# ESCOMP/POP2-CESM

Hardware: AMD Instinct MI355X
Metric: simulated_years_per_day (higher is better)
Workload: dtype f64; 1 GPU; tx0.1v3; nt=2, steps_per_day=300, step_calls_per_day=319, distribution=equal-block-counts, blocks_local=1, hmix=del4, hmix_tracer=del4, vmix=kpp, partial_bottom_cells=False, ns_boundary=closed, grid_input=False, tadvect=centered, solver=pcg, preconditioner=diagonal, transport=none, kpp_surface_buoyancy=on-demand down to the boundary-layer depth

## Files before the change

include/pop_amd.h:

```cpp
#ifndef POP_AMD_H
#define POP_AMD_H

#ifdef __cplusplus
extern "C" {
#endif

#define POP_CONFIG_VERSION 7
typedef struct pop_config {
  int struct_version;
  int nx_global, ny_global, km, nt;
  int block_size_x, block_size_y;
  int ew_boundary;
  int ns_boundary;
  int hmix_momentum;
  int hmix_tracer;
  int lvariable_hmix;
  int vmix_choice;
  int tadvect;
  int solver_choice;
  int max_iterations;
  int convergence_check_freq;
  int tmix_opt;
  int time_mix_freq;
  int steps_per_day;
// ... 33 lines not shown
  double kappa_depth_1, kappa_depth_2, kappa_depth_scale;
  int aniso_alignment;
  int lvariable_hmix_aniso;
  int lsmag_aniso;
  int vconst_5;
  double visc_para, visc_perp;
  double c_para, c_perp;
  double u_para, u_perp;
  double vconst_1;
  double vconst_2;
  double vconst_3;
  double vconst_4;
  double vconst_6;
  double vconst_7;
  double smag_lat;
  double smag_lat_fact;
  double smag_lat_gauss;
  int lsubmesoscale_mixing;
  int luse_const_horiz_len_scale;
  int submeso_diag;
  double efficiency_factor;
  double time_scale_constant;
  double hor_length_scale;
} pop_config;

typedef struct pop_ctx pop_ctx;

#define POP_CREATE_HOST_ONLY 1
#define POP_CREATE_PLAN_ONLY 2

#define POP_TUNING_UNSET (-2147483647 - 1)
typedef struct pop_tuning {
  int struct_bytes;
  int land_skip;
  int land_full_steps;
  int xcd_remap;
  int red_band;
  int lds_order;
  int momentum_lds;
  int tracer_lds;
  int generic_thomas;
  int reg_thomas_t;
  int thomas_pair;
  int tracer_fwd;
  int vdc_shared;
  int side_stream;
  int del4_side;
  int del4_tile;
  int d2t_fuse, d2u_fuse;
  int vmixu_defer;
  int vmixu_inline;
  int btrop_inline;
  int kpp_ahead;
  int kpp_col;
  int kpp_lazy;
  int kpp_ushear_hint;
  int kpp_ushear_margin;
  int kpp_side_stream;
  int kpp_interior_generic;
  int kpp_src_full;
  int solver_unfused;
  int solver_nograph;
  int solver_presum;
  int solver_distributed;
  int solver_overlap_off;
  int fpcg_b2;
  int pcsi_step2;
  int halo_separate;
  int halo_overlap_off;
  int rccl_overlap;
  int evp_wave;
  int fpcg_a_pair;
  int kpp_sparse;
  int pbc_generic_thomas;
  int pbc_generic_kpp;
  int gm_sf_stored;
  int state3d_levels;
  int pcg_persist;
  int gm_flux_tile;
  int pcsi_two_step;
  int block_sums_relay;
  int aniso_side;
  int submeso_all_levels;
} pop_tuning;
void pop_tuning_init(pop_tuning *t);
int pop_get_tuning(const pop_ctx *ctx, pop_tuning *resolved);

int pop_create(const pop_config *cfg, int rank, int nranks, int flags, pop_ctx **out);
typedef struct pop_grid_input {
  const double *ULAT, *ULON, *HTN, *HTE, *HUS, *HUW, *ANGLE;
  const int *KMT;
  const double *DZBC;
} pop_grid_input;
int pop_create_with_grid(const pop_config *cfg, const pop_grid_input *grid, int rank, int nranks, int flags, pop_ctx **out);
int pop_create_tuned(const pop_config *cfg, const pop_grid_input *grid, const pop_tuning *tuning, int rank, int nranks, int flags, pop_ctx **out);
int pop_read_grid_files(const char *horiz_grid_file, const char *topography_file, int nx_global, int ny_global,
                        double *seven_records , int *kmt );
int pop_destroy(pop_ctx *ctx);
const char *pop_last_error(const pop_ctx *ctx);

#define POP_MAX_TIDAL_MIN_REGIONS 9
typedef struct pop_tidal_nml {
  int struct_bytes;
  int ltidal_mixing;
  int tidal_mixing_method;
  int ltidal_max;
  int ltidal_stabc;
  int lccsm_control_compatible;
  int ltidal_min_regions;
  int num_tidal_min_regions;
  int tidal_diag;
  double tidal_local_mixing_fraction;
  double tidal_mixing_efficiency;
  double vertical_decay_scale;
  double tidal_mix_max;
  double tidal_min_values[POP_MAX_TIDAL_MIN_REGIONS];
  double tidal_TLATmin_regions[POP_MAX_TIDAL_MIN_REGIONS];
  double tidal_TLATmax_regions[POP_MAX_TIDAL_MIN_REGIONS];
  double tidal_TLONmin_regions[POP_MAX_TIDAL_MIN_REGIONS];
  double tidal_TLONmax_regions[POP_MAX_TIDAL_MIN_REGIONS];
  int tidal_min_regions_klevels[POP_MAX_TIDAL_MIN_REGIONS];
} pop_tidal_nml;
void pop_tidal_nml_init(pop_tidal_nml *nml);
int pop_init_tidal_mixing(pop_ctx *ctx, const pop_tidal_nml *nml, const double *energy_flux, long long count);

typedef struct pop_kpp_bckgrnd_nml {
  int struct_bytes;
  int lhoriz_varying_bckgrnd;
  int larctic_bckgrnd_vdc;
  double bckgrnd_vdc_eq;
  double bckgrnd_vdc_psim;
  double bckgrnd_vdc_ban;
} pop_kpp_bckgrnd_nml;
void pop_kpp_bckgrnd_nml_init(pop_kpp_bckgrnd_nml *nml);
int pop_init_kpp_bckgrnd(pop_ctx *ctx, const pop_kpp_bckgrnd_nml *nml);

int pop_init_iage(pop_ctx *ctx, int n);

typedef struct pop_ice_nml {
  int struct_bytes;
  int ice_freq_opt;
  int licecesm2;
  int kmxice;
  int lactive_ice;
  int lfw_as_salt_flx;
  int tfreeze_option;
  double sea_ice_salinity;
  double ocn_ref_salinity;
  double latent_heat_fusion;
  double cp_sw;
  double rho_sw;
  double rho_fw;
} pop_ice_nml;
void pop_ice_nml_init(pop_ice_nml *nml);
int pop_init_ice(pop_ctx *ctx, const pop_ice_nml *nml);
int pop_ice_formation(pop_ctx *ctx, int tl);
int pop_ice_flx_to_coupler(pop_ctx *ctx);
int pop_ice_export_reset(pop_ctx *ctx);
int pop_tfreez_host(pop_ctx *ctx, const double *S, double *TFRZ, long long count);

int pop_get_dim(const pop_ctx *ctx, const char *name);
double pop_get_scalar(const pop_ctx *ctx, const char *name);
int pop_get_block(const pop_ctx *ctx, int block_id, int *out8, int *i_glob, int *j_glob);
int pop_local_block_ids(const pop_ctx *ctx, int *ids );

int pop_get_field(pop_ctx *ctx, const char *name, int tl, int n, double *host, long long count);
// ... 134 lines not shown
```

pop2-cesm_amd/csrc/forms.hpp:

```cpp
#pragma once
#include <algorithm>
#include "pop_internal.hpp"

namespace pop {

enum { VMIXU_INLINE = 0, VMIXU_SIDE = 1, VMIXU_DEFERRED = 2 };
enum { KPP_BUOY_MARCH = 0, KPP_BUOY_FUSED_LDS, KPP_BUOY_LDS, KPP_BUOY_PLAIN };
enum { KPP_INTERIOR_FUSED = 0, KPP_INTERIOR_REG, KPP_INTERIOR_GENERIC };
#define POP_FORMS(X)                                                                                                                 \
                                                                   \
  X(int, xcd_remap) X(int, red_band) X(int, lds_order)                                                                              \
     \
  X(bool, land_skip) X(int, land_full_steps)                                                                                        \
     \
  X(int, momentum_lds_rows) X(int, tracer_lds_rows) X(bool, gm_lds) X(bool, kpp_src_full) X(bool, tracer_fwd)                       \
                                                                                               \
  X(bool, reg_thomas_u) X(bool, reg_thomas_t) X(bool, thomas_pair) X(int, impvmixu_waves)                                           \
                                                                                                     \
  X(bool, vdc_shared) X(bool, side_stream) X(bool, del4_side) X(bool, mom_side) X(bool, aniso_side)                                 \
                                                                                                             \
  X(int, del4_tile_rows) X(bool, d2t_fuse) X(bool, d2u_fuse)                                                                        \
             \
  X(int, vmixu) X(bool, btrop_inline)                                                                                               \
                                                                            \
  X(bool, kpp_ahead) X(int, kpp_col) X(bool, kpp_lazy) X(bool, kpp_lazy20) X(bool, kpp_march) X(bool, kpp_pbc_generic)              \
  X(bool, kpp_shear_col) X(int, kpp_buoy) X(int, kpp_buoy_kr) X(bool, kpp_buoy_sfc) X(bool, kpp_depth_lazy) X(int, kpp_depth_kr)    \
  X(int, kpp_interior) X(bool, kpp_sparse) X(bool, kpp_side) X(bool, kpp_wuk) X(int, kpp_wuk_margin)                                \
                                                                                                            \
  X(int, state3d_levels) X(bool, gm_sf_stored) X(bool, submeso_all_levels)                                                          \
          \
  X(int, path) X(bool, fused_ok) X(bool, evp_fused_ok) X(bool, replicated) X(int, evp_wave) X(bool, graph) X(bool, overlap)         \
  X(bool, presum_forced) X(bool, fpcg_b2) X(bool, fpcg_a_pair) X(int, block_sums_relay) X(int, persist)                             \
                       \
  X(bool, pcsi_two_cell) X(bool, pcsi_two_step) X(bool, pcsi_two_step_dist)                                                         \
                                                                                           \
  X(bool, halo_separate) X(bool, halo_overlap) X(int, rccl_overlap)
struct Forms {
#define X(type, name) type name = 0;
  POP_FORMS(X)
#undef X
};
inline int forms_get(const Forms &f, const std::string &name) {
#define X(type, member) if (name == #member) return (int)f.member;
  POP_FORMS(X)
#undef X
  return -1;
}

constexpr double KPP_EPSSFC = 0.1;
inline std::vector<int> kpp_kref(const HostModel &h) {
  std::vector<int> kref(h.km + 3, 1);
  for (int k = 1; k <= h.km; ++k) {
    const double surfthick = KPP_EPSSFC * h.zt[k];
    kref[k] = k;
    for (int kt = 1; kt <= k; ++kt) if (h.zw[kt] >= surfthick) { kref[k] = kt; break; }
  }
  return kref;
}
inline int max_blocks_per_rank(const HostModel &h) {
  std::vector<int> per(h.nranks, 0);
  for (int o : h.block_owner) if (o >= 0 && o < h.nranks) per[o]++;
  return per.empty() ? 0 : *std::max_element(per.begin(), per.end());
}
inline std::vector<int> local_srcmap(const HostModel &h) {
  std::vector<int> sm(h.n2 * h.nblocks);
  for (size_t p = 0; p < sm.size(); ++p) sm[p] = (int)p;
  for (size_t i = 0; i < h.halo.copy_dst.size(); ++i) sm[h.halo.copy_dst[i]] = h.halo.copy_src[i];
  for (int d : h.halo.fill_dst) sm[d] = -1;
  if (h.c.ns_boundary == 2) {
    const TripolePlan &T = h.halo.tripole[0];
    for (size_t e = 0; e < T.dst.size(); ++e) sm[T.dst[e]] = T.a[e];
  }
  return sm;
}
inline bool pcsi_fold_local(const HostModel &h, const std::vector<int> &srcmap, std::vector<int> &jfold) {
  bool local = true;
  jfold.assign(h.nblocks, h.nyb);
  if (h.c.ns_boundary != 2) return true;
  for (int lb = 0; lb < h.nblocks; ++lb) {
    const BlockInfo &B = h.all_blocks[h.local_ids[lb] - 1];
    if (!(B.j_glob[B.je] < 0)) continue;
    jfold[lb] = B.je;
    for (int j = B.je; j < h.nyb; ++j) for (int i = 0; i < h.nxb; ++i) {
      const int cell = lb * (int)h.n2 + j * h.nxb + i;
      if (srcmap[cell] == cell) local = false;
    }
  }
  return local;
}
inline int chunks_per_block(long long n2, int red_band) {
  const int nc = (int)((n2 + 255) / 256);
  return red_band ? 8 * ((nc + 7) / 8) : nc;
}
inline bool presum_by_size(long long nchunk, long long nblocks) { return nchunk * nblocks > 2048; }
inline bool two_cell_shape(int nxb, bool presummed) { return presummed && (nxb & 1) == 0; }

inline bool bandwidth_bound(const HostModel &h) { return (long long)h.n2 * h.nblocks > (1LL << 19); }
inline bool register_levels(const HostModel &h) { return h.km == 60 || h.km == 62; }

inline int resolve_forms(const HostModel &h, Forms &f, std::string &err) {
  const pop_config &c = h.c;
  const pop_tuning &t = h.tun;
  const bool big = bandwidth_bound(h), reg_km = register_levels(h), evp = use_evp(c), tripole = c.ns_boundary == 2;
  const bool single = h.halo.peers.empty();
  auto rule_or = [](int v, bool rule) { return (tun_set(v) && v >= 0) ? v != 0 : rule; };
  if (tun_set(t.xcd_remap) && t.xcd_remap != 0 && t.xcd_remap != 1) { err = "pop_create: pop_tuning.xcd_remap is " + std::to_string(t.xcd_remap) + ": 0 linear or 1 XCD bands"; return 1; }
  if (tun_set(t.evp_wave) && t.evp_wave != 0 && t.evp_wave != 3) { err = "pop_create: pop_tuning.evp_wave is " + std::to_string(t.evp_wave) + ": 0 one thread per sub-block or 3 wavefronts"; return 1; }

  f.xcd_remap = tun_or(t.xcd_remap, big ? 0 : 1);
  f.red_band = tun_or(t.red_band, 1);
  f.lds_order = tun_or(t.lds_order, 1);
  f.land_skip = !tun_off(t.land_skip);
  f.land_full_steps = tun_or(t.land_full_steps, 4);

  f.momentum_lds_rows = tun_or(t.momentum_lds, 4);
  f.tracer_lds_rows = tun_or(t.tracer_lds, 4);
  f.gm_lds = !tun_off(t.gm_flux_tile);
  f.kpp_src_full = tun_on(t.kpp_src_full);

  const bool pbc_generic = c.partial_bottom_cells && tun_on(t.pbc_generic_thomas);
  const bool want_u = !tun_on(t.generic_thomas) && !pbc_generic;
  const bool want_t = (tun_set(t.reg_thomas_t) ? t.reg_thomas_t != 0 : !tun_on(t.generic_thomas)) && !pbc_generic;
  f.reg_thomas_u = want_u && reg_km;
  f.reg_thomas_t = want_t && reg_km;
  f.thomas_pair = f.reg_thomas_t && rule_or(t.thomas_pair, big);
  f.impvmixu_waves = (!c.partial_bottom_cells && !big) ? 2 : 1;
  f.tracer_fwd = c.tadvect == 1 && c.hmix_tracer != 3 && (f.tracer_lds_rows == 4 || f.tracer_lds_rows == 8) && c.lpressure_avg &&
                 (tun_set(t.tracer_fwd) ? t.tracer_fwd != 0 : !want_t);

  f.vdc_shared = c.vmix_choice == 3 && !c.ldbl_diff && !tun_off(t.vdc_shared);
  f.side_stream = !tun_off(t.side_stream);
  f.del4_side = f.side_stream && (c.hmix_tracer == 4 || c.hmix_momentum == 4) && !tun_off(t.del4_side);
  f.aniso_side = f.side_stream && c.hmix_momentum == 3 && !tun_off(t.aniso_side);
  f.mom_side = c.hmix_momentum == 3 ? f.aniso_side : f.del4_side;

  f.del4_tile_rows = big ? 4 : 0;
  if (tun_set(t.del4_tile)) f.del4_tile_rows = (t.del4_tile == 2 || t.del4_tile == 4 || t.del4_tile == 8 || t.del4_tile == 16) ? t.del4_tile : 0;
  const bool fuse = f.del4_side && !tripole && rule_or(t.d2t_fuse, big);
  f.d2t_fuse = fuse && c.hmix_tracer == 4 && c.tadvect == 1;
  f.d2u_fuse = fuse && c.hmix_momentum == 4 && !tun_off(t.d2u_fuse);

  f.btrop_inline = !f.side_stream || tripole || tun_on(t.btrop_inline);
  const bool off_stream = f.side_stream && f.reg_thomas_u && !tun_on(t.vmixu_inline);
  f.vmixu = (off_stream && !f.btrop_inline && rule_or(t.vmixu_defer, big)) ? VMIXU_DEFERRED : off_stream ? VMIXU_SIDE : VMIXU_INLINE;

  f.evp_wave = tun_or(t.evp_wave, 3);
  f.graph = !tun_on(t.solver_nograph);
  f.overlap = !tun_on(t.solver_overlap_off);
  f.presum_forced = tun_on(t.solver_presum);
  f.fpcg_b2 = !tun_off(t.fpcg_b2);
  f.fpcg_a_pair = !tun_off(t.fpcg_a_pair);
  f.block_sums_relay = tun_or(t.block_sums_relay, 1);
  f.persist = !tun_set(t.pcg_persist) ? 1 : (t.pcg_persist == 0 || t.pcg_persist == 2 || t.pcg_persist == 4 || t.pcg_persist == 8) ? t.pcg_persist : 1;
  const bool unfused = tun_on(t.solver_unfused);
  f.fused_ok = single && h.nblocks <= 8 && !unfused;
  if (evp) {
    f.evp_fused_ok = f.fused_ok && c.solver_choice == 3;
    f.fused_ok = false;
  }
  f.replicated = !single && c.solver_choice == 1 && !evp && h.nblocks_tot <= 8 && (long long)h.n2 * h.nblocks_tot <= (4LL << 20) &&
                 !tun_on(t.solver_distributed);
  const bool spread = h.nranks > 1 && !unfused, few = max_blocks_per_rank(h) <= 16;
  if (c.solver_choice == 2) f.path = (f.fused_ok && !evp) ? 2 : (spread && few && !evp) ? 3 : 1;
  else if (c.solver_choice == 3) f.path = evp ? (f.evp_fused_ok ? 2 : 1) : f.fused_ok ? 2 : spread ? 3 : 1;
  else f.path = evp ? 1 : f.replicated ? 4 : f.fused_ok ? 2 : (spread && few) ? 3 : 1;
  const int nchunk = chunks_per_block((long long)h.n2, f.red_band);
  const bool two_cell_rule = two_cell_shape(h.nxb, presum_by_size(nchunk, h.nblocks));
  f.pcsi_two_cell = tun_set(t.pcsi_step2) ? two_cell_shape(h.nxb, t.pcsi_step2 != 0) : two_cell_rule;
  if (!evp && (tun_set(t.pcsi_two_step) ? t.pcsi_two_step != 0 : two_cell_rule)) {
    std::vector<int> jfold;
    const bool fold_ok = !tripole || pcsi_fold_local(h, local_srcmap(h), jfold);
    f.pcsi_two_step = fold_ok && single;
    f.pcsi_two_step_dist = fold_ok && !single;
  }

  if (c.vmix_choice == 3) {
    const bool resident_solve = (c.solver_choice == 1 || c.solver_choice == 3) && !evp && f.persist != 0 && h.nranks == 1 && h.nblocks <= 8 &&
                                h.n2 * h.nblocks <= 250u * 8u * 256u;
    f.kpp_ahead = f.side_stream && (tun_set(t.kpp_ahead) ? t.kpp_ahead != 0 : (big || resident_solve));
    const std::vector<int> kref = kpp_kref(h);
    const int max_kref = *std::max_element(kref.begin(), kref.end());
    f.kpp_col = (max_kref <= 24) ? tun_or(t.kpp_col, big ? 31 : 1) : 0;
    const bool fused_bi = (f.kpp_col & 8) && max_kref <= 20 && h.km <= 64, lds = (f.kpp_col & 4) && max_kref <= 28;
    f.kpp_lazy = (fused_bi || !lds) && max_kref <= 28 && !c.lcheckekmo && c.kpp_ml_diagnostics != 1 && !tun_off(t.kpp_lazy);
    f.kpp_lazy20 = f.kpp_lazy && max_kref <= 20;
    f.kpp_march = f.kpp_lazy && fused_bi && (f.kpp_col & 16) && c.num_v_smooth_Ri == 1 && !c.ldbl_diff && h.km >= 3;
    f.kpp_pbc_generic = c.partial_bottom_cells && !(f.kpp_march && f.kpp_lazy20 && (f.kpp_col & 1) && !tun_on(t.pbc_generic_kpp));
    const bool gen = f.kpp_pbc_generic;
    f.kpp_shear_col = !gen && (f.kpp_col & 1);
    f.kpp_buoy = gen ? KPP_BUOY_PLAIN : f.kpp_march ? KPP_BUOY_MARCH : fused_bi ? KPP_BUOY_FUSED_LDS : lds ? KPP_BUOY_LDS : KPP_BUOY_PLAIN;
    f.kpp_buoy_kr = max_kref <= 20 ? 20 : 28;
    f.kpp_buoy_sfc = gen || !f.kpp_lazy;
    f.kpp_depth_lazy = !gen && f.kpp_lazy;
    f.kpp_depth_kr = (f.kpp_depth_lazy && !f.kpp_lazy20) ? 28 : 20;
    f.kpp_interior = gen ? KPP_INTERIOR_GENERIC : fused_bi ? KPP_INTERIOR_FUSED : (!tun_on(t.kpp_interior_generic) && reg_km) ? KPP_INTERIOR_REG : KPP_INTERIOR_GENERIC;
    f.kpp_sparse = !gen && f.kpp_march && h.km <= 64 && !tun_off(t.kpp_sparse);
    f.kpp_side = !tun_off(t.kpp_side_stream) && !gen;
    f.kpp_wuk = f.kpp_depth_lazy && (f.kpp_col & 1) && !tun_off(t.kpp_ushear_hint);
    f.kpp_wuk_margin = tun_or(t.kpp_ushear_margin, 3);
  }

  f.state3d_levels = tun_or(t.state3d_levels, 4);
  f.gm_sf_stored = !tun_off(t.gm_sf_stored);
  f.submeso_all_levels = tun_on(t.submeso_all_levels);

  f.halo_separate = tun_on(t.halo_separate);
  f.halo_overlap = !tun_on(t.halo_overlap_off);
  f.rccl_overlap = tun_or(t.rccl_overlap, 1);
  return 0;
}

}
```

pop2-cesm_amd/csrc/kernels_bckgrnd.hpp:

```cpp
#pragma once

namespace pop {

struct BckDev {
  const double *VDC = nullptr, *VVC = nullptr, *VVC_PR = nullptr;
};

struct BckRaw { double visc, vd1, vd2; };
__global__ void __launch_bounds__(POP_COL_THREADS)
k_kpp_bckgrnd(DevGrid g, BckDev bd, int vdc_same, double *__restrict__ VISC, double *__restrict__ VDC1, double *__restrict__ VDC2) {
  Col c;
  if (!col_setup(g, c, false)) return;
  const int km = g.km;
  const long long n2 = g.n2;
  const int kmt = g.KMT[c.q2];
  if (kmt < 2) return;
  const double bvdc = bd.VDC[c.q2], bvvc = bd.VVC[c.q2];
  const long long vb = ((long long)c.b * (km + 2)) * n2 + c.p2;
  auto load = [&](int k) {
    BckRaw r;
    r.visc = VISC[c.base3 + (long long)(k - 1) * n2]; r.vd1 = VDC1[vb + (long long)k * n2];
    r.vd2 = vdc_same ? 0.0 : VDC2[vb + (long long)k * n2];
    return r;
  };
  BckRaw cu = load(1);
#pragma unroll 1
  for (int k = 1; k < kmt; ++k) {
    const BckRaw nx = load(k + 1 < kmt ? k + 1 : k);
    VISC[c.base3 + (long long)(k - 1) * n2] = cu.visc + bvvc;
    VDC1[vb + (long long)k * n2] = cu.vd1 + bvdc;
    if (!vdc_same) VDC2[vb + (long long)k * n2] = cu.vd2 + bvdc;
    cu = nx;
  }
}

}
```

pop2-cesm_amd/csrc/kernels_common.hpp:

```cpp
#pragma once
#include "device_types.hpp"
#include "forms.hpp"
#include <type_traits>

namespace pop {

template <class F> inline void with_flags(F &&f) { f(); }
template <class F, class... Bs> inline void with_flags(F &&f, bool b, Bs... bs) {
  if (b) with_flags([&](auto... c) { f(std::true_type{}, c...); }, bs...);
  else with_flags([&](auto... c) { f(std::false_type{}, c...); }, bs...);
}
template <int... Vs, class F> inline bool with_value(int v, F &&f) {
  return ((v == Vs ? (f(std::integral_constant<int, Vs>{}), true) : false) || ...);
}

#define POP_COL_THREADS 64
#ifndef POP_TRC_WAVES
#define POP_TRC_WAVES 2
#endif
#ifndef POP_MOM_WAVES
#define POP_MOM_WAVES 2
#endif

__device__ __forceinline__ double pbc_dz(const DevGrid &g, int k, int kbot, double dzbot) {
  return (k < 1 || k > g.km) ? 0.0 : ((k == kbot) ? dzbot : g.dz[k]);
}

__device__ __forceinline__ int blk_ie(const DevGrid &g, int b) { return g.ieb ? g.ieb[b] : g.ie; }
__device__ __forceinline__ int blk_je(const DevGrid &g, int b) { return g.jeb ? g.jeb[b] : g.je; }

struct Col {
  int i, j, b, p2;
  long long q2;
  long long base3;
};
__host__ __device__ inline int lds_grid_x(int lds_order, int ntx, int nty) {
  const int nt = ntx * nty;
  return lds_order ? 256 * ((nt + 255) / 256) : nt;
}
__host__ __device__ inline int lds_slot_of(int a) {
  const int r = a >> 5, t = a & 31;
  return (((r >> 3) << 5) + t) * 8 + (r & 7);
}
__host__ __device__ inline bool lds_tile_from_gi(int gi, int ntx, int nty, int &ti, int &tj);
__host__ __device__ inline bool lds_tile_of(int lds_order, int bx, int ntx, int nty, int &ti, int &tj) {
  if (!lds_order) { ti = bx % ntx; tj = bx / ntx; return tj < nty; }
  const int e = bx & 7, s = bx >> 3;
  const int gi = ((s >> 5) * 8 + e) * 32 + (s & 31);
  return lds_tile_from_gi(gi, ntx, nty, ti, tj);
}
__host__ __device__ inline bool lds_tile_from_gi(int gi, int ntx, int nty, int &ti, int &tj) {
  constexpr int PW = 4, PH = 8;
  if (gi >= ntx * nty) return false;
  const int row_tiles = PH * ntx, full_rows = nty / PH;
  int Pj, r, h;
  if (gi >= full_rows * row_tiles) { Pj = full_rows; r = gi - full_rows * row_tiles; h = nty - full_rows * PH; }
  else { Pj = gi / row_tiles; r = gi % row_tiles; h = PH; }
  const int patch_tiles = h * PW, nfullp = ntx / PW;
  int Pi, w, rr;
  if (r < nfullp * patch_tiles) { Pi = r / patch_tiles; w = PW; rr = r % patch_tiles; }
  else { Pi = nfullp; w = ntx - nfullp * PW; rr = r - nfullp * patch_tiles; }
  ti = Pi * PW + rr % w; tj = Pj * PH + rr / w;
  return true;
}
__device__ __forceinline__ bool lds_tile(int lds_order, int ntx, int nty, int &ti, int &tj) {
  return lds_tile_of(lds_order, (int)blockIdx.x, ntx, nty, ti, tj);
}
template <int R>
__device__ __forceinline__ bool lds_tile_active(const DevGrid &g, int b, int ntx, int nty, int &ti, int &tj, bool &listed) {
  const int *L = (R == 8) ? g.lds_act8 : g.lds_act4;
  const int nL = (R == 8) ? g.lds_n8 : g.lds_n4;
  listed = g.skip && L != nullptr;
  if (!listed) return lds_tile(g.lds_order, ntx, nty, ti, tj);
  const int e = L[(long long)b * nL + blockIdx.x];
  if (e < 0) return false;
  ti = e & 0xffff; tj = e >> 16;
  return true;
}
template <int R>
__host__ inline int lds_launch_x(const DevGrid &g, int ntx, int nty) {
  const int *L = (R == 8) ? g.lds_act8 : g.lds_act4;
  if (g.skip && L) return (R == 8) ? g.lds_n8 : g.lds_n4;
  return lds_grid_x(g.lds_order, ntx, nty);
}
__device__ __forceinline__ int ocean_cells(const DevGrid &g, int b, int p0, int p1) {
  const int *S = g.opre + (long long)b * (g.n2 + 1);
  return S[p1] - S[p0];
}
__device__ __forceinline__ bool land_tile(const DevGrid &g, int b, int i0, int w, int j0, int h) {
  if (!g.skip) return false;
  int i1 = i0 + w, j1 = j0 + h;
  if (i0 < 0) i0 = 0;
  if (j0 < 0) j0 = 0;
  if (i1 > g.nxb) i1 = g.nxb;
  if (j1 > g.nyb) j1 = g.nyb;
  if (i0 >= i1) return false;
  int n = 0;
  for (int j = j0; j < j1; ++j) n += ocean_cells(g, b, j * g.nxb + i0, j * g.nxb + i1);
  return n == 0;
}
__device__ __forceinline__ bool land_run(const DevGrid &g, int b, long long p0, int n) {
  if (!g.skip || p0 >= g.n2) return false;
  const int p1 = (p0 + n < g.n2) ? (int)(p0 + n) : g.n2;
  return ocean_cells(g, b, (int)p0, p1) == 0;
}
__host__ __device__ inline int col_grid_x(int n2, int threads) { const int nt = (n2 + threads - 1) / threads; return 8 * ((nt + 7) / 8); }
__host__ inline int col_grid(const DevGrid &g, int threads) { return col_grid_x(g.n2, threads); }
__device__ __forceinline__ bool col_setup(const DevGrid &g, Col &c, bool interior_only) {
  c.b = blockIdx.y;
  const int tile = g.xcd_remap ? (blockIdx.x & 7) * (gridDim.x >> 3) + (blockIdx.x >> 3) : blockIdx.x;
  c.p2 = tile * blockDim.x + threadIdx.x;
  if (c.p2 >= g.n2) return false;
  if (land_run(g, c.b, (long long)tile * blockDim.x, blockDim.x)) return false;
  c.i = c.p2 % g.nxb;
  c.j = c.p2 / g.nxb;
  if (interior_only && (c.i + 1 < g.ib || c.i + 1 > blk_ie(g, c.b) || c.j + 1 < g.jb || c.j + 1 > blk_je(g, c.b))) return false;
  c.q2 = (long long)c.b * g.n2 + c.p2;
  c.base3 = (long long)c.b * g.n3 + c.p2;
  return true;
}
__device__ __forceinline__ bool patch_cell(const DevGrid &g, int tile, int b, int &p2) {
  if (!tile) {
    p2 = blockIdx.x * blockDim.x + threadIdx.x;
    if (p2 >= g.n2) return false;
    return !land_run(g, b, (long long)blockIdx.x * blockDim.x, blockDim.x);
  }
  const int tiles_i = (g.nxb + 63) / 64;
  const int ti = blockIdx.x % tiles_i, tj = blockIdx.x / tiles_i;
  const int i = ti * 64 + (threadIdx.x & 63), j = tj * tile + (threadIdx.x >> 6);
  if (land_tile(g, b, ti * 64, 64, tj * tile, tile)) return false;
  if (i >= g.nxb || j >= g.nyb) return false;
  p2 = j * g.nxb + i;
  return true;
}
__host__ inline unsigned patch_grid_x(const DevGrid &g, int tile) {
  return tile ? (unsigned)(((g.nxb + 63) / 64) * ((g.nyb + tile - 1) / tile)) : (unsigned)((g.n2 + 255) / 256);
}
__host__ inline int red_grid_x(const DevGrid &g) {
  return g.red_act ? g.red_nact : chunks_per_block(g.n2, g.red_band);
}
__device__ __forceinline__ int red_chunk(const DevGrid &g) {
  if (g.red_act) return g.red_act[(long long)blockIdx.y * g.red_nact + blockIdx.x];
  return g.red_band ? (blockIdx.x & 7) * (gridDim.x >> 3) + (blockIdx.x >> 3) : blockIdx.x;
}
__device__ __forceinline__ int red_cell(const DevGrid &g) {
  const long long p2 = (long long)red_chunk(g) * blockDim.x + threadIdx.x;
  return p2 < g.n2 ? (int)p2 : g.n2;
}

__device__ __forceinline__ bool red_land(const DevGrid &g, bool deep = false) {
  if (!g.skip || (blockIdx.x == 0 && blockIdx.y == 0)) return false;
  if (g.red_act)
    return (int)((blockIdx.x & 7) * (g.red_nact >> 3) + (blockIdx.x >> 3)) >= g.red_cnt[blockIdx.y];
  const long long p0 = (long long)red_chunk(g) * 256;
  if (!land_run(g, blockIdx.y, p0, 256)) return false;
  const long long p1 = (p0 + 255 < g.n2) ? p0 + 255 : g.n2 - 1;
  const int j0 = (int)(p0 / g.nxb), j1 = (int)(p1 / g.nxb);
  const int i0 = (j0 == j1) ? (int)(p0 % g.nxb) : 0, i1 = (j0 == j1) ? (int)(p1 % g.nxb) : g.nxb - 1;
  if (deep && !(i0 >= g.ib - 1 + NGHOST && i1 <= blk_ie(g, blockIdx.y) - 1 - NGHOST && j0 >= g.jb - 1 + NGHOST && j1 <= blk_je(g, blockIdx.y) - 1 - NGHOST)) return false;
  return true;
}
template <int NF>
__device__ __forceinline__ bool red_land_out(const DevGrid &g, double *__restrict__ partial, int nchunk, bool deep = false) {
  if (!red_land(g, deep)) return false;
  if (threadIdx.x == 0) {
    const long long slot = (long long)blockIdx.y * nchunk + red_chunk(g);
#pragma unroll
    for (int f = 0; f < NF; ++f) partial[NF * slot + f] = 0.0;
  }
  return true;
}

struct MwjfP {
  double n0, n2, ns1t0, d0, d1, d3;
};
__device__ __forceinline__ MwjfP mwjf_level(double pbar) {
  const double p = 10.0 * pbar;
  MwjfP c;
  c.n0 = (9.99843699e+2 * 0.001) + p * ((1.04004591e-2 * 0.001) + p * (-3.24041825e-8 * 0.001));
  c.n2 = (-5.45928211e-2 * 0.001) + p * ((1.03970529e-7 * 0.001) + p * (-1.23869360e-11 * 0.001));
  c.ns1t0 = (2.96938239e+0 * 0.001) + p * (5.18761880e-6 * 0.001);
  c.d0 = 1.0e+0 + p * 5.30848875e-6;
  c.d1 = 7.28606739e-3 + (p * p * p) * -1.27934137e-17;
  c.d3 = 3.68390573e-7 + (p * p) * -3.03175128e-16;
  return c;
}
struct MwjfTS { double TQ, SQ, SQR; };
__device__ __forceinline__ MwjfTS mwjf_prep(double TK, double SK) {
  MwjfTS r;
  r.TQ = fmin(TK, 999.0); r.TQ = fmax(r.TQ, -2.0);
  double SQ = fmin(SK, 0.999); SQ = fmax(SQ, 0.0);
  r.SQ = 1000.0 * SQ;
  r.SQR = sqrt(r.SQ);
  return r;
}
__device__ __forceinline__ double mwjf_eval(const MwjfP &c, const MwjfTS &x) {
  const double n1 = 7.35212840e+0 * 0.001, n3 = 3.98476704e-4 * 0.001;
  const double ns1t1 = -7.23268813e-3 * 0.001, ns2t0 = 2.12382341e-3 * 0.001;
  const double d2 = -4.60835542e-5, d4 = 1.80809186e-10, ds1t0 = 2.14691708e-3, ds1t1 = -9.27062484e-6;
  const double ds1t3 = -1.78343643e-10, dsqt0 = 4.76534122e-6, dsqt2 = 1.63410736e-9;
  const double TQ = x.TQ, SQ = x.SQ, SQR = x.SQR;
  const double W1 = c.n0 + TQ * (n1 + TQ * (c.n2 + n3 * TQ)) + SQ * (c.ns1t0 + ns1t1 * TQ + ns2t0 * SQ);
  const double W2 = c.d0 + TQ * (c.d1 + TQ * (d2 + TQ * (c.d3 + d4 * TQ))) +
                    SQ * (ds1t0 + TQ * (ds1t1 + TQ * TQ * ds1t3) + SQR * (dsqt0 + TQ * TQ * dsqt2));
  const double DEN = 1.0 / W2;
  return W1 * DEN;
}
struct MwjfTS2 { double TQ, SQ, A2; };
__device__ __forceinline__ MwjfTS2 mwjf_prep2(double TK, double SK) {
  const double ds1t0 = 2.14691708e-3, ds1t1 = -9.27062484e-6, ds1t3 = -1.78343643e-10, dsqt0 = 4.76534122e-6, dsqt2 = 1.63410736e-9;
  MwjfTS2 r;
  r.TQ = fmin(TK, 999.0); r.TQ = fmax(r.TQ, -2.0);
  double SQ = fmin(SK, 0.999); SQ = fmax(SQ, 0.0);
  r.SQ = 1000.0 * SQ;
  const double SQR = sqrt(r.SQ), TQ = r.TQ;
  r.A2 = r.SQ * (ds1t0 + TQ * (ds1t1 + TQ * TQ * ds1t3) + SQR * (dsqt0 + TQ * TQ * dsqt2));
  return r;
}
// ... 37 lines not shown
```

pop2-cesm_amd/csrc/kernels_kpp.hpp:

```cpp
#pragma once

namespace pop {

struct KppDev {
  CArr zgrid, hwide, bckgrnd_vdc, bckgrnd_vvc;
  CArrI kref;
  CArr eosP;
  unsigned long long *CONVB;
  int src_clear_all;
  double *HBLT0, *USTAR, *BFSFC;
  int *KBL0, *KBL;
  double Vtc, cg, rich_mix;
  int lrich, ldbl_diff, nsmooth;
  int *WUK;
  int wu_margin;
  int vdc_same;

  int lshort_wave, sw_type, jerlov, lcheckekmo;
  const double *FCORT, *SHF_QSW;
  const double *Tr, *ztr;
  const int *CHLI;
  int ksol;
  double *BO, *BOSOL;
  double *SRCX = nullptr;
// ... 229 lines not shown
  double (*dst)[POP_COL_THREADS] = shtop;
  for (int pass = 0; pass + 1 < kp.nsmooth; ++pass) {
#pragma unroll 1
    for (int k = 1 + gy; k <= km; k += NG) {
      const double cur = src ? src[k - 1][tx] : w0(k);
      double v = cur;
      if (kmt >= 3) {
        const double w1 = 0.25 * ((k > 1) ? (src ? src[k - 2][tx] : w0(k - 1)) : cur);
        const double nxt = (k < km) ? (src ? src[k][tx] : w0(k + 1)) : cur;
        v = w1 + 0.5 * cur + 0.25 * nxt;
      }
      dst[k - 1][tx] = v;
    }
    __syncthreads();
    src = dst; dst = (dst == shtop) ? shri : shtop;
  }
  if (!live) return;
  const long long vb = ((long long)b * (km + 2)) * n2 + p2;
#pragma unroll 1
  for (int k = 1 + gy; k <= km; k += NG) {
    const long long o = base3 + (long long)(k - 1) * n2;
    const double cur = src ? src[k - 1][tx] : w0(k);
    double riw = cur;
    if (kp.nsmooth >= 1 && kmt >= 3) {
      const double w1 = 0.25 * ((k > 1) ? (src ? src[k - 2][tx] : w0(k - 1)) : cur);
      const double nxt = (k < km) ? (src ? src[k][tx] : w0(k + 1)) : cur;
      riw = w1 + 0.5 * cur + 0.25 * nxt;
    }
    double fri = fmax(riw, 0.0) / KPP_RIINFTY;
    fri = fmin(fri, 1.0);
    double visc, vd1 = 0.0, vd2 = 0.0;
    if (kp.lrich) {
      const double f = 1.0 - fri * fri;
      const double f3 = (f * f) * f;
      visc = kp.bckgrnd_vvc[k] + kp.rich_mix * f3;
      if (k < km) { vd2 = kp.bckgrnd_vdc[k] + kp.rich_mix * f3; vd1 = vd2; }
    } else {
      visc = kp.bckgrnd_vvc[k];
      if (k < km) { vd2 = kp.bckgrnd_vdc[k]; vd1 = vd2; }
    }
    if (k >= kmt) { visc = 0.0; vd1 = 0.0; vd2 = 0.0; }
    if (kp.ldbl_diff) {
      const double t_k = T[o], s_k = S[o];
      double ta_u = 0.0, sb_u = 0.0;
      { const MwjfP Pk = mwjf_level(g.pressz[k]); (void)mwjf_rho<true>(Pk, tmask(t_k), s_k, &ta_u, &sb_u); }
      double alphadt = 0.0, betads = 0.0, ta_n = 0.0, sb_n = 0.0, t_n = 0.0, s_n = 0.0;
      if (k < km) {
        t_n = T[o + n2]; s_n = S[o + n2];
        const MwjfP Pn = mwjf_level(g.pressz[k + 1]);
        (void)mwjf_rho<true>(Pn, tmask(t_n), s_n, &ta_n, &sb_n);
        alphadt = -0.5 * (ta_u + ta_n) * (t_k - t_n);
        betads = 0.5 * (sb_u + sb_n) * (s_k - s_n);
      }
      if (alphadt > betads && betads > 0.0) {
        const double rrho = fmin(alphadt / betads, KPP_RRHO0);
        const double f = 1.0 - (rrho - 1.0) / (KPP_RRHO0 - 1.0);
        const double diffdd = KPP_DSFMAX * ((f * f) * f);
        vd1 = vd1 + 0.7 * diffdd; vd2 = vd2 + diffdd;
      }
      double rrho = 0.0, diffdd = 0.0, prandtl = 0.0;
      if (alphadt < 0.0 && betads < 0.0 && alphadt > betads) {
        rrho = alphadt / betads;
        diffdd = 1.5e-2 * 0.909 * exp(4.6 * exp(-0.54 * (1.0 / rrho - 1.0)));
        prandtl = 0.15 * rrho;
      }
      if (rrho > 0.5) prandtl = (1.85 - 0.85 / rrho) * rrho;
      vd1 = vd1 + diffdd; vd2 = vd2 + prandtl * diffdd;
    }
    VISC[o] = visc;
    VDC1[vb + (long long)k * n2] = vd1;
    if (!kp.vdc_same) VDC2[vb + (long long)k * n2] = vd2;
  }
}

__global__ void k_kpp_level_table(DevGrid g, double *__restrict__ tab) {
  const int k = threadIdx.x;
  if (k < 1 || k > g.km) return;
  const MwjfP P = mwjf_level(g.pressz[k]);
  double *t = tab + 6 * k;
  t[0] = P.n0; t[1] = P.n2; t[2] = P.ns1t0; t[3] = P.d0; t[4] = P.d1; t[5] = P.d3;
}
struct KppRaw { double t, s, u[4], v[4]; };
template <bool PBC = false>
__global__ void __launch_bounds__(POP_COL_THREADS)
k_kpp_buoy_interior_march(DevGrid g, KppDev kp, const double *__restrict__ T, const double *__restrict__ S,
                          const double *__restrict__ U, const double *__restrict__ V, double *__restrict__ DBLOC,
                          double *__restrict__ VISC, double *__restrict__ VDC1, double *__restrict__ VDC2) {
  Col c;
  if (!col_setup(g, c, false)) return;
  const int km = g.km, nxb = g.nxb;
  const long long n2 = g.n2;
  const int kmt = g.KMT[c.q2];
  const bool edge = (c.i == 0 || c.j == 0);
  const long long off4[4] = {0, edge ? 0 : -(long long)nxb, edge ? 0 : -1, edge ? 0 : -1 - (long long)nxb};
  const long long vb = ((long long)c.b * (km + 2)) * n2 + c.p2;
  int kmu4[4] = {0, 0, 0, 0}; double dzub4[4] = {0.0, 0.0, 0.0, 0.0}; const double dzbc = PBC ? g.DZBC[c.q2] : 0.0;
  if (PBC) {
#pragma unroll
    for (int t = 0; t < 4; ++t) { kmu4[t] = g.KMU[c.q2 + off4[t]]; dzub4[t] = g.DZUB[c.q2 + off4[t]]; }
  }
  auto dzq = [&](int k, int kbot, double dzbot) { return (k < 1 || k > km) ? 0.0 : ((k == kbot) ? dzbot : g.dz.u(k)); };
  auto load = [&](int k) {
    KppRaw r;
    const long long o = c.base3 + (long long)(k - 1) * n2;
    r.t = T[o]; r.s = S[o];
#pragma unroll
    for (int t = 0; t < 4; ++t) { r.u[t] = U[o + off4[t]]; r.v[t] = V[o + off4[t]]; }
    return r;
  };
  auto emit = [&](int k, double wprev, double cur, double wnext) {
    double riw = cur;
    if (kmt >= 3) {
      const double w1 = 0.25 * ((k > 1) ? wprev : cur);
      const double nxt = (k < km) ? wnext : cur;
      riw = w1 + 0.5 * cur + 0.25 * nxt;
    }
    double fri = fmax(riw, 0.0) / KPP_RIINFTY;
    fri = fmin(fri, 1.0);
    double visc, vd1 = 0.0, vd2 = 0.0;
    if (kp.lrich) {
      const double f = 1.0 - fri * fri;
      const double f3 = (f * f) * f;
      visc = kp.bckgrnd_vvc[k] + kp.rich_mix * f3;
      if (k < km) { vd2 = kp.bckgrnd_vdc[k] + kp.rich_mix * f3; vd1 = vd2; }
    } else {
      visc = kp.bckgrnd_vvc[k];
      if (k < km) { vd2 = kp.bckgrnd_vdc[k]; vd1 = vd2; }
    }
    if (k >= kmt) { visc = 0.0; vd1 = 0.0; vd2 = 0.0; }
    VISC[c.base3 + (long long)(k - 1) * n2] = visc;
    VDC1[vb + (long long)k * n2] = vd1;
    if (!kp.vdc_same) VDC2[vb + (long long)k * n2] = vd2;
  };
  KppRaw up = load(1), A = load(2 <= km ? 2 : km), B;
  MwjfTS2 xkm = mwjf_prep2(tmask(up.t), up.s);
  double wpp = 0.0, wp = 0.0, carry = 0.0;
  unsigned long long convb = 0ull;
  auto level = [&](int k, const KppRaw &cu, KppRaw &nx) {
    nx = load(k + 1 <= km ? k + 1 : km);
    const MwjfTS2 xk = mwjf_prep2(tmask(cu.t), cu.s);
    MwjfP P;
    { const int e = 6 * k; P.n0 = kp.eosP[e]; P.n2 = kp.eosP[e + 1]; P.ns1t0 = kp.eosP[e + 2]; P.d0 = kp.eosP[e + 3]; P.d1 = kp.eosP[e + 4]; P.d3 = kp.eosP[e + 5]; }
    const double rhokm = mwjf_eval2(P, xkm);
    const double rhok = mwjf_eval2(P, xk);
    double dbl = 0.0;
    if (rhok != 0.0) dbl = GRAV * (1.0 - rhokm / rhok);
    if (k - 1 >= kmt) dbl = 0.0;
    DBLOC[c.base3 + (long long)(k - 2) * n2] = dbl;
    if (!(dbl > 0.0)) convb |= 1ull << (k - 2);
    double sh4[4];
#pragma unroll
    for (int t = 0; t < 4; ++t) {
      const double du = up.u[t] - cu.u[t], dv = up.v[t] - cu.v[t];
      sh4[t] = du * du + dv * dv;
      if (PBC) { const double h = 0.5 * (dzq(k - 1, kmu4[t], dzub4[t]) + dzq(k, kmu4[t], dzub4[t])); sh4[t] = sh4[t] / (h * h); }
    }
    double vsh = 0.25 * sh4[0] + 0.25 * sh4[1] + 0.25 * sh4[2] + 0.25 * sh4[3];
    if (edge) vsh = 0.0;
    double ri = dbl * (kp.zgrid[k - 1] - kp.zgrid[k]) / (vsh + KPP_EPS);
    if (PBC) { const double h = 0.5 * (dzq(k - 1, kmt, dzbc) + dzq(k, kmt, dzbc)); ri = dbl / (vsh + KPP_EPS / (h * h)) / h; }
    const int m = k - 1;
    const double w = (m <= kmt) ? ri : carry;
    if (m == kmt) carry = ri;
    if (m >= 2) emit(m - 1, wpp, wp, w);
    wpp = wp; wp = w;
#pragma unroll
    for (int t = 0; t < 4; ++t) { up.u[t] = cu.u[t]; up.v[t] = cu.v[t]; }
    xkm = xk;
  };
  int k = 2;
#pragma unroll 1
  for (; k + 1 <= km; k += 2) { level(k, A, B); level(k + 1, B, A); }
  if (k <= km) level(k, A, B);
  DBLOC[c.base3 + (long long)(km - 1) * n2] = 0.0;
  if (kp.CONVB) kp.CONVB[c.q2] = convb;
  {
    double ri = 0.0 * (kp.zgrid[km] - kp.zgrid[km + 1]) / (0.0 + KPP_EPS);
    if (PBC) { const double h = 0.5 * dzq(km, kmt, dzbc); ri = 0.0 / (0.0 + KPP_EPS / (h * h)) / h; }
    const double w = (km <= kmt) ? ri : carry;
    emit(km - 1, wpp, wp, w);
    emit(km, wp, w, w);
  }
}

template <int KR, bool PBC = false>
__global__ void __launch_bounds__(POP_COL_THREADS)
k_kpp_ushear_col(DevGrid g, KppDev kp, const double *__restrict__ U, const double *__restrict__ V, double *__restrict__ WU) {
  static_assert(POP_COL_THREADS == 64, "k_kpp_ushear_col: one wavefront per workgroup");
  __shared__ int s_cap;
  if (kp.WUK && threadIdx.x == 0) s_cap = 0;
  Col c;
  if (!col_setup(g, c, false)) return;
  const int km = g.km;
  const long long n2 = g.n2;
  int kcap = km, krcap = KR;
  if (kp.WUK) {
    int h = kp.KBL[c.q2];
    if (c.i + 1 < g.nxb) h = max(h, kp.KBL[c.q2 + 1]);
    if (c.j + 1 < g.nyb) { h = max(h, kp.KBL[c.q2 + g.nxb]); if (c.i + 1 < g.nxb) h = max(h, kp.KBL[c.q2 + g.nxb + 1]); }
    __syncthreads();
    atomicMax(&s_cap, h);
    __syncthreads();
    kcap = min(km, max(2, s_cap + kp.wu_margin));
    kp.WUK[c.q2] = kcap;
    krcap = kp.kref[kcap];
  }
  const int kmu_c = PBC ? g.KMU[c.q2] : 0; const double dzub_c = PBC ? g.DZUB[c.q2] : 0.0;
  double ur[KR + 1], vr[KR + 1];
#pragma unroll
  for (int t = 1; t <= KR; ++t) {
    ur[t] = 0.0; vr[t] = 0.0;
    if (t <= krcap) {
      const int kk = (t <= km) ? t : km;
      const long long o = c.base3 + (long long)(kk - 1) * n2;
      ur[t] = U[o]; vr[t] = V[o];
    }
  }
  for (int kl = 2; kl <= kcap; ++kl) {
    const long long o = c.base3 + (long long)(kl - 1) * n2;
    const double ukl = U[o], vkl = V[o];
    const double surfthick = KPP_EPSSFC * g.zt[kl];
    const int kref = kp.kref[kl];
    double uref, vref;
    if (kref > 1) {
      double uk = ur[1], vk = vr[1];
#pragma unroll
      for (int t = 2; t <= KR; ++t) if (t == kref) { uk = ur[t]; vk = vr[t]; }
      uref = uk * (surfthick - g.zw[kref - 1]);
      vref = vk * (surfthick - g.zw[kref - 1]);
#pragma unroll
      for (int kt = 1; kt <= KR - 1; ++kt)
        if (kt <= kref - 1) { uref = uref + g.dz[kt] * ur[kt]; vref = vref + g.dz[kt] * vr[kt]; }
      uref = uref / surfthick; vref = vref / surfthick;
    } else { uref = ur[1]; vref = vr[1]; }
    const double du = uref - ukl, dv = vref - vkl;
    if (PBC) {
      const double h = -kp.zgrid[kl - 1] + 0.5 * (pbc_dz(g, kl, kmu_c, dzub_c) + pbc_dz(g, kl - 1, kmu_c, dzub_c) - pbc_dz(g, 1, kmu_c, dzub_c));
      WU[o] = (du * du + dv * dv) / (h * h);
    } else WU[o] = du * du + dv * dv;
  }
}

template <bool PBC = false>
__global__ void __launch_bounds__(POP_COL_THREADS)
k_kpp_interior(DevGrid g, KppDev kp, const double *__restrict__ T, const double *__restrict__ S,
               const double *__restrict__ U, const double *__restrict__ V, const double *__restrict__ DBLOC,
               double *__restrict__ RIW, double *__restrict__ VISC, double *__restrict__ VDC1, double *__restrict__ VDC2) {
  Col c;
  if (!col_setup(g, c, false)) return;
  const int km = g.km, nxb = g.nxb;
  const long long n2 = g.n2;
  const int kmt = g.KMT[c.q2];
  const bool edge = (c.i == 0 || c.j == 0);
  int kmu4[4] = {0, 0, 0, 0}; double dzub4[4] = {0, 0, 0, 0}; const double dzbc = PBC ? g.DZBC[c.q2] : 0.0;
  if (PBC && !edge) {
    const long long off[4] = {0, -nxb, -1, -1 - nxb};
#pragma unroll
    for (int t = 0; t < 4; ++t) { kmu4[t] = g.KMU[c.q2 + off[t]]; dzub4[t] = g.DZUB[c.q2 + off[t]]; }
  }
  double prev = 0.0;
  for (int k = 1; k <= km; ++k) {
    const long long o = c.base3 + (long long)(k - 1) * n2;
    double vsh = 0.0;
    if (k < km && !edge) {
      auto sh = [&](long long q, int t) {
        const double du = U[q] - U[q + n2], dv = V[q] - V[q + n2];
        if (PBC) { const double h = 0.5 * (pbc_dz(g, k, kmu4[t], dzub4[t]) + pbc_dz(g, k + 1, kmu4[t], dzub4[t])); return (du * du + dv * dv) / (h * h); }
        return du * du + dv * dv;
      };
      vsh = 0.25 * sh(o, 0) + 0.25 * sh(o - nxb, 1) + 0.25 * sh(o - 1, 2) + 0.25 * sh(o - 1 - nxb, 3);
    }
    double ri = DBLOC[o] * (kp.zgrid[k] - kp.zgrid[k + 1]) / (vsh + KPP_EPS);
    if (PBC) {
      const double h = (k < km) ? 0.5 * (pbc_dz(g, k, kmt, dzbc) + pbc_dz(g, k + 1, kmt, dzbc)) : 0.5 * pbc_dz(g, k, kmt, dzbc);
      ri = DBLOC[o] / (vsh + KPP_EPS / (h * h)) / h;
    }
    const double w0 = (k <= kmt) ? ri : prev;
    RIW[o] = w0;
    prev = w0;
  }
  for (int n = 0; n < kp.nsmooth; ++n) {
    double w1 = 0.25 * RIW[c.base3];
    if (kmt >= 3) {
      double cur = RIW[c.base3];
      for (int k = 1; k <= km; ++k) {
        const long long o = c.base3 + (long long)(k - 1) * n2;
        const double nxt = (k < km) ? RIW[o + n2] : cur;
        RIW[o] = w1 + 0.5 * cur + 0.25 * nxt;
        w1 = 0.25 * cur;
        cur = nxt;
      }
    }
  }
  const long long vb = ((long long)c.b * (km + 2)) * n2 + c.p2;
  double ta_u = 0.0, sb_u = 0.0, t_k = T[c.base3], s_k = S[c.base3];
  if (kp.ldbl_diff) { const MwjfP P = mwjf_level(g.pressz[1]); (void)mwjf_rho<true>(P, tmask(t_k), s_k, &ta_u, &sb_u); }
  for (int k = 1; k <= km; ++k) {
    const long long o = c.base3 + (long long)(k - 1) * n2;
    double fri = fmax(RIW[o], 0.0) / KPP_RIINFTY;
    fri = fmin(fri, 1.0);
    double visc, vd1 = 0.0, vd2 = 0.0;
    if (kp.lrich) {
      const double f = 1.0 - fri * fri;
      const double f3 = (f * f) * f;
      visc = kp.bckgrnd_vvc[k] + kp.rich_mix * f3;
      if (k < km) { vd2 = kp.bckgrnd_vdc[k] + kp.rich_mix * f3; vd1 = vd2; }
    } else {
      visc = kp.bckgrnd_vvc[k];
      if (k < km) { vd2 = kp.bckgrnd_vdc[k]; vd1 = vd2; }
    }
    if (k >= kmt) { visc = 0.0; vd1 = 0.0; vd2 = 0.0; }
    if (kp.ldbl_diff) {
      double alphadt = 0.0, betads = 0.0, ta_n = 0.0, sb_n = 0.0, t_n = 0.0, s_n = 0.0;
      if (k < km) {
        t_n = T[o + n2]; s_n = S[o + n2];
        const MwjfP P = mwjf_level(g.pressz[k + 1]);
        (void)mwjf_rho<true>(P, tmask(t_n), s_n, &ta_n, &sb_n);
        alphadt = -0.5 * (ta_u + ta_n) * (t_k - t_n);
        betads = 0.5 * (sb_u + sb_n) * (s_k - s_n);
      }
      if (alphadt > betads && betads > 0.0) {
        const double rrho = fmin(alphadt / betads, KPP_RRHO0);
        const double f = 1.0 - (rrho - 1.0) / (KPP_RRHO0 - 1.0);
// ... 117 lines not shown
    VISC[o] = visc;
    VDC1[vb + (long long)k * n2] = vd1;
    if (!kp.vdc_same) VDC2[vb + (long long)k * n2] = vd2;
  }
}

template <bool PBC = false>
__global__ void __launch_bounds__(256)
k_kpp_ushear(DevGrid g, KppDev kp, const double *__restrict__ U, const double *__restrict__ V, double *__restrict__ WU) {
  const int p2 = blockIdx.x * blockDim.x + threadIdx.x;
  const int kl = blockIdx.y + 1, b = blockIdx.z;
  if (p2 >= g.n2 || kl < 2) return;
  const long long n2 = g.n2;
  const long long base3 = (long long)b * g.n3 + p2;
  const long long o = base3 + (long long)(kl - 1) * n2;
  const double surfthick = KPP_EPSSFC * g.zt[kl];
  const int kref = kp.kref[kl];
  double uref, vref;
  if (kref > 1) {
    const long long orf = base3 + (long long)(kref - 1) * n2;
    uref = U[orf] * (surfthick - g.zw[kref - 1]);
    vref = V[orf] * (surfthick - g.zw[kref - 1]);
    int kt = 1;
    for (; kt + 7 <= kref - 1; kt += 8) {
      double uu[8], vv[8];
#pragma unroll
      for (int t = 0; t < 8; ++t) { const long long ot = base3 + (long long)(kt + t - 1) * n2; uu[t] = U[ot]; vv[t] = V[ot]; }
#pragma unroll
      for (int t = 0; t < 8; ++t) { uref = uref + g.dz[kt + t] * uu[t]; vref = vref + g.dz[kt + t] * vv[t]; }
    }
    for (; kt <= kref - 1; ++kt) {
      const long long ot = base3 + (long long)(kt - 1) * n2;
      uref = uref + g.dz[kt] * U[ot];
      vref = vref + g.dz[kt] * V[ot];
    }
    uref = uref / surfthick; vref = vref / surfthick;
  } else { uref = U[base3]; vref = V[base3]; }
  const double du = uref - U[o], dv = vref - V[o];
  if (PBC) {
    const long long q2 = (long long)b * n2 + p2;
    const int kmu = g.KMU[q2]; const double dzub = g.DZUB[q2];
    const double h = -kp.zgrid[kl - 1] + 0.5 * (pbc_dz(g, kl, kmu, dzub) + pbc_dz(g, kl - 1, kmu, dzub) - pbc_dz(g, 1, kmu, dzub));
    WU[o] = (du * du + dv * dv) / (h * h);
  } else
  WU[o] = du * du + dv * dv;
}

template <bool PBC = false>
__device__ __forceinline__ double kpp_ushear_point(const DevGrid &g, const KppDev &kp, const double *__restrict__ U, const double *__restrict__ V,
                                                   long long base3, int kl, long long q2 = 0) {
  const long long n2 = g.n2;
  const long long o = base3 + (long long)(kl - 1) * n2;
  const double surfthick = KPP_EPSSFC * g.zt[kl];
  const int kref = kp.kref[kl];
  double uref, vref;
  if (kref > 1) {
    const long long orf = base3 + (long long)(kref - 1) * n2;
    uref = U[orf] * (surfthick - g.zw[kref - 1]);
    vref = V[orf] * (surfthick - g.zw[kref - 1]);
#pragma unroll 1
    for (int kt = 1; kt <= kref - 1; ++kt) {
      const long long ot = base3 + (long long)(kt - 1) * n2;
      uref = uref + g.dz[kt] * U[ot];
      vref = vref + g.dz[kt] * V[ot];
    }
    uref = uref / surfthick; vref = vref / surfthick;
  } else { uref = U[base3]; vref = V[base3]; }
  const double du = uref - U[o], dv = vref - V[o];
  if (PBC) {
    const int kmu = g.KMU[q2]; const double dzub = g.DZUB[q2];
    const double h = -kp.zgrid[kl - 1] + 0.5 * (pbc_dz(g, kl, kmu, dzub) + pbc_dz(g, kl - 1, kmu, dzub) - pbc_dz(g, 1, kmu, dzub));
    return (du * du + dv * dv) / (h * h);
  }
  return du * du + dv * dv;
}

template <bool LAZY, int KR, bool PBC = false>
__global__ void __launch_bounds__(POP_COL_THREADS)
k_kpp_bldepth(DevGrid g, KppDev kp, const double *__restrict__ T, const double *__restrict__ S,
              const double *__restrict__ STF1, const double *__restrict__ STF2, const double *__restrict__ DBLOC,
              const double *__restrict__ DBSFC, const double *__restrict__ WU, const double *__restrict__ UU, const double *__restrict__ VV) {
  static_assert(POP_COL_THREADS == 64, "the lazy march votes over one 64-lane wave");
  __shared__ double shtop[LAZY ? 3 * KR : 1][POP_COL_THREADS];
  int nprep = 0;
  Col c;
  if (!col_setup(g, c, false)) return;
  const int km = g.km, nxb = g.nxb;
  const long long n2 = g.n2;
  const int kmt = g.KMT[c.q2];
  const bool edge = (c.i == 0 || c.j == 0);
  int wuk[4] = {km, km, km, km};
  if (LAZY && kp.WUK && !edge) { wuk[0] = kp.WUK[c.q2]; wuk[1] = kp.WUK[c.q2 - 1]; wuk[2] = kp.WUK[c.q2 - nxb]; wuk[3] = kp.WUK[c.q2 - 1 - nxb]; }
  const double s1 = g.SMFT1[c.q2], s2 = g.SMFT2[c.q2];
  double ustar = sqrt(sqrt(s1 * s1 + s2 * s2));
  ustar = fmax(ustar, KPP_EPS);
  double talpha, sbeta;
  const MwjfP P1 = mwjf_level(g.pressz[1]);
  const double rho1 = mwjf_rho<true>(P1, tmask(T[c.base3]), S[c.base3], &talpha, &sbeta);
  double bo = 0.0, bosol = 0.0;
  const int chli = (kp.lshort_wave && kp.sw_type == 2) ? kp.CHLI[c.q2] : 0;
  if (rho1 != 0.0) {
    bo = GRAV * (-talpha * STF1[c.q2] - sbeta * STF2[c.q2]) / rho1;
    if (kp.lshort_wave) bosol = -GRAV * talpha * kp.SHF_QSW[c.q2] / rho1;
  }
  int kbl = (kmt > 1) ? kmt : 1;
  double hblt = -kp.zgrid[kbl];
  const double dzbc = PBC ? g.DZBC[c.q2] : 0.0, dzub = PBC ? g.DZUB[c.q2] : 0.0;
  const int kmu_c = PBC ? g.KMU[c.q2] : 0;
  auto zkl_of = [&](int kl) { return (PBC && kl > 1) ? -kp.zgrid[kl - 1] + 0.5 * (pbc_dz(g, kl, kmt, dzbc) + pbc_dz(g, kl - 1, kmt, dzbc)) : -kp.zgrid[kl]; };
  if (PBC) hblt = zkl_of(kbl);
  double rib_upper = 0.0, rib_up = 0.0, z_upper = 0.0, z_up = kp.zgrid[1];
  double bfsfc = bo;
  double hekman = 0.0, hlimit = 0.0, hmon_up = 0.0;
  if (kp.lcheckekmo) {
    hekman = -kp.zgrid[km] + KPP_EPS; hlimit = -kp.zgrid[km] + KPP_EPS;
    double bf = kpp_bfsfc(kp, bo, bosol, -z_up, 1, chli);
    const double st = (bf >= 0.0) ? 1.0 : 0.0;
    bf = bf + st * KPP_EPS;
    const double w = st * KPP_CMONOB * ustar * ustar * ustar / KPP_VONKAR / bf + (st - 1.0) * kp.zgrid[km];
    hmon_up = (w <= -z_up) ? -z_up + KPP_EPS : w;
  }
  for (int kl = 2; kl <= km; ++kl) {
    if (LAZY && __builtin_amdgcn_ballot_w64(kbl == kmt && kl <= kmt) == 0) break;
    const long long o = c.base3 + (long long)(kl - 1) * n2;
    const double surfthick = KPP_EPSSFC * g.zt[kl];
    const double zkl = zkl_of(kl);
    double dbsfc;
    if (LAZY) {
      const int kref = kp.kref[kl];
      for (; nprep < kref; ++nprep) {
        const int kk = (nprep + 1 <= km) ? nprep + 1 : km;
        const long long ot = c.base3 + (long long)(kk - 1) * n2;
        const MwjfTS2 x = mwjf_prep2(tmask(T[ot]), S[ot]);
        shtop[nprep][threadIdx.x] = x.TQ; shtop[KR + nprep][threadIdx.x] = x.SQ; shtop[2 * KR + nprep][threadIdx.x] = x.A2;
      }
      auto top_at = [&](int t) { MwjfTS2 x; x.TQ = shtop[t - 1][threadIdx.x]; x.SQ = shtop[KR + t - 1][threadIdx.x]; x.A2 = shtop[2 * KR + t - 1][threadIdx.x]; return x; };
      const MwjfTS2 xk = mwjf_prep2(tmask(T[o]), S[o]);
      const MwjfP P = mwjf_level(g.pressz[kl]);
      const double rhok = mwjf_eval2(P, xk);
      double rhoavg = mwjf_eval2(P, top_at(kref));
      if (kref != 1) {
        rhoavg = rhoavg * (surfthick - g.zw[kref - 1]);
#pragma unroll 1
        for (int kt = 1; kt <= kref - 1; ++kt) rhoavg = rhoavg + g.dz[kt] * mwjf_eval2(P, top_at(kt));
        rhoavg = rhoavg / surfthick;
      }
      dbsfc = 0.0;
      if (rhok != 0.0) dbsfc = GRAV * (1.0 - rhoavg / rhok);
    } else dbsfc = DBSFC[o];
    double vshear = 0.0;
    if (!edge) {
      if (LAZY && kp.WUK) {
        const double w00 = (kl <= wuk[0]) ? WU[o] : kpp_ushear_point<PBC>(g, kp, UU, VV, c.base3, kl, c.q2);
        const double w10 = (kl <= wuk[1]) ? WU[o - 1] : kpp_ushear_point<PBC>(g, kp, UU, VV, c.base3 - 1, kl, c.q2 - 1);
        const double w01 = (kl <= wuk[2]) ? WU[o - nxb] : kpp_ushear_point<PBC>(g, kp, UU, VV, c.base3 - nxb, kl, c.q2 - nxb);
        const double w11 = (kl <= wuk[3]) ? WU[o - 1 - nxb] : kpp_ushear_point<PBC>(g, kp, UU, VV, c.base3 - 1 - nxb, kl, c.q2 - 1 - nxb);
        vshear = fmax(fmax(w00, w10), fmax(w01, w11));
      } else vshear = fmax(fmax(WU[o], WU[o - 1]), fmax(WU[o - nxb], WU[o - 1 - nxb]));
    }
    bfsfc = kpp_bfsfc(kp, bo, bosol, zkl, 2 * kl - 1, chli);
    const double stable = (bfsfc >= 0.0) ? 1.0 : 0.0;
    bfsfc = bfsfc + stable * KPP_EPS;
    if (kp.lcheckekmo) {
      if (stable > 0.5 && hekman >= -kp.zgrid[km]) hekman = fmax(zkl, KPP_CEKMAN * ustar / (fabs(kp.FCORT[c.q2]) + KPP_EPS));
      const double hmon_dn = stable * KPP_CMONOB * ustar * ustar * ustar / KPP_VONKAR / bfsfc + (stable - 1.0) * kp.zgrid[km];
      if (hmon_dn <= zkl && hmon_up > -z_up) {
        const double w = (hmon_dn - hmon_up) / (z_up + zkl);
        hlimit = (hmon_dn - w * zkl) / (1.0 - w);
      }
      hmon_up = hmon_dn;
    }
    double wm_unused = 0.0, ws;
    kpp_wscale<false>(KPP_EPSSFC, zkl, ustar, bfsfc, wm_unused, ws);
    const double db = DBLOC[o];
    double bfr = sqrt(0.5 * (db + fabs(db) + KPP_EPS2) / (kp.zgrid[kl] - kp.zgrid[kl + 1]));
    if (PBC) bfr = (kl < km) ? sqrt(0.5 * (db + fabs(db) + KPP_EPS2) / (0.5 * (pbc_dz(g, kl, kmt, dzbc) + pbc_dz(g, kl + 1, kmt, dzbc))))
                             : sqrt(0.5 * (db + fabs(db) + KPP_EPS2) / pbc_dz(g, kl, kmt, dzbc));
    const double zref = -surfthick / 2.0;
    double wmm = zkl * ws * bfr * ((kp.Vtc / KPP_RICR) * fmax(2.1 - 200.0 * bfr, KPP_CONCV));
    double wk = (kmt >= kl) ? (zref - kp.zgrid[kl]) * dbsfc : 0.0;
    double rib_dn;
    if (PBC) {
      const double ht = -kp.zgrid[kl - 1] + 0.5 * (pbc_dz(g, kl - 1, kmt, dzbc) + pbc_dz(g, kl, kmt, dzbc) - pbc_dz(g, 1, kmt, dzbc));
      const double hu = -kp.zgrid[kl - 1] + 0.5 * (pbc_dz(g, kl, kmu_c, dzub) + pbc_dz(g, kl - 1, kmu_c, dzub) - pbc_dz(g, 1, kmu_c, dzub));
      wk = (kmt >= kl) ? dbsfc / ht : 0.0;
      wmm = wmm / (ht * ht);
      rib_dn = wk / (vshear + wmm + KPP_EPS / (hu * hu));
    } else rib_dn = wk / (vshear + wmm + KPP_EPS);
    if (kbl == kmt && rib_dn > KPP_RICR) {
      const double slope_up = (rib_upper - rib_up) / (z_up - z_upper);
      const double d = z_up + zkl;
      const double a_co = (rib_dn - rib_up - slope_up * (zkl + z_up)) / (d * d);
      const double b_co = slope_up + 2.0 * a_co * z_up;
      const double c_co = rib_up + z_up * (a_co * z_up + slope_up) - KPP_RICR;
      const double sqrt_arg = b_co * b_co - 4.0 * a_co * c_co;
      if ((fabs(b_co) > KPP_EPS && fabs(a_co) / fabs(b_co) <= KPP_EPS) || sqrt_arg <= 0.0)
        hblt = -z_up + (z_up + zkl) * (KPP_RICR - rib_up) / (rib_dn - rib_up);
      else hblt = (-b_co + sqrt(sqrt_arg)) / (2.0 * a_co);
      kbl = kl;
    }
    rib_upper = rib_up; rib_up = rib_dn;
    z_upper = z_up; z_up = kp.zgrid[kl];
  }
  if (kp.lcheckekmo) {
    if (hekman < hlimit) hlimit = hekman;
    for (int kl = 2; kl <= km; ++kl)
      if (hlimit < hblt && hlimit > -kp.zgrid[kl - 1] && hlimit <= zkl_of(km)) { hblt = hlimit; kbl = kl; }
  }
  if (LAZY && km >= 2) {
    bfsfc = kpp_bfsfc(kp, bo, bosol, -kp.zgrid[km], 2 * km - 1, chli);
    bfsfc = bfsfc + ((bfsfc >= 0.0) ? 1.0 : 0.0) * KPP_EPS;
  }
  kp.HBLT0[c.q2] = hblt;
  kp.KBL0[c.q2] = kbl;
  kp.USTAR[c.q2] = ustar;
  kp.BFSFC[c.q2] = bfsfc;
  if (kp.lshort_wave) { kp.BO[c.q2] = bo; kp.BOSOL[c.q2] = bosol; }
}

struct KppBlRaw { double visc, vd1, vd2, db; };
template <bool PBC = false, bool SAME = false, bool SPARSE = false, bool XS = false>
__global__ void __launch_bounds__(POP_COL_THREADS)
k_kpp_blmix(DevGrid g, StepParams sp, KppDev kp, const double *__restrict__ DBLOC, const double *__restrict__ STF1,
            const double *__restrict__ STF2, double *__restrict__ VISC, double *__restrict__ VDC1, double *__restrict__ VDC2,
            double *__restrict__ SRC1, double *__restrict__ SRC2, double *__restrict__ HBLT_OUT) {
  Col c;
  if (!col_setup(g, c, false)) return;
  const int km = g.km, nxb = g.nxb;
  const long long n2 = g.n2;
  const int kmt = g.KMT[c.q2];
  const CArr zgrid = kp.zgrid, hwide = kp.hwide;
  double w2 = kp.HBLT0[c.q2];
  int kbl = kp.KBL0[c.q2];
  const bool inner = (c.i >= 1 && c.i <= g.nxb - 2 && c.j >= 1 && c.j <= g.nyb - 2);
  if (inner && kmt != 0) {
    double cw = 0.125, ce = 0.125, cn = 0.125, cs = 0.125, cc = 0.5;
    if (g.KMT[c.q2 - 1] == 0) { cc = cc + cw; cw = 0.0; }
    if (g.KMT[c.q2 + 1] == 0) { cc = cc + ce; ce = 0.0; }
    if (g.KMT[c.q2 - nxb] == 0) { cc = cc + cs; cs = 0.0; }
    if (g.KMT[c.q2 + nxb] == 0) { cc = cc + cn; cn = 0.0; }
    w2 = cw * kp.HBLT0[c.q2 - 1] + ce * kp.HBLT0[c.q2 + 1] + cs * kp.HBLT0[c.q2 - nxb] + cn * kp.HBLT0[c.q2 + nxb] + cc * kp.HBLT0[c.q2];
  }
  const double dzbc = PBC ? g.DZBC[c.q2] : 0.0;
  auto dzt_at = [&](int k) { return pbc_dz(g, k, kmt, dzbc); };
  auto ztmp = [&](int k) { return PBC ? -zgrid[k - 1] + 0.5 * (dzt_at(k - 1) + dzt_at(k)) : -zgrid[k]; };
  if (inner && kmt >= 1 && w2 > ztmp(kmt)) w2 = ztmp(kmt);
  const double hblt = fmax(w2, -zgrid[1]);
  if (inner && kmt != 0)
    for (int k = 1; k <= km; ++k)
      if (hblt > -zgrid[k - 1] && hblt <= ztmp(k)) kbl = max(k, 2);
  HBLT_OUT[c.q2] = hblt;
  const int kbl_prev = SPARSE ? kp.KBL[c.q2] : 0;
  kp.KBL[c.q2] = kbl;
  const double ustar = kp.USTAR[c.q2];
  double bfsfc = kp.BFSFC[c.q2];
  if (kp.lshort_wave) bfsfc = kpp_bfsfc(kp, kp.BO[c.q2], kp.BOSOL[c.q2], hblt, 0, kp.sw_type == 2 ? kp.CHLI[c.q2] : 0);
  const double stable = (bfsfc >= 0.0) ? 1.0 : 0.0;
  bfsfc = bfsfc + stable * KPP_EPS;
  double wm, ws;
  kpp_wscale<true>(KPP_EPSSFC, hblt, ustar, bfsfc, wm, ws);
  double casea_x = -zgrid[kbl] - 0.5 * hwide[kbl] - hblt;
  if (PBC) casea_x = (kbl == 1) ? -zgrid[0] - hblt : -zgrid[kbl - 1] + 0.5 * dzt_at(kbl - 1) - hblt;
  const double casea = 0.5 + (casea_x >= 0.0 ? 0.5 : -0.5);
  const int nc = (casea > 0.5) ? 1 : 0;
  const int kn = nc * (kbl - 1) + (1 - nc) * kbl;
  const double u2 = ustar * ustar;
  const double f1 = stable * 5.0 * bfsfc / (u2 * u2 + KPP_EPS);
  const long long vb = ((long long)c.b * (km + 2)) * n2 + c.p2;
  auto visc_at = [&](int k) { return (k >= 1 && k <= km) ? VISC[c.base3 + (long long)(k - 1) * n2] : 0.0; };
  double gat1[3] = {0.0, 0.0, 0.0}, dat1[3] = {0.0, 0.0, 0.0};
  if (kn >= 1 && kn <= km) {
    const int k = kn;
    double dh = 0.5 * hwide[k] - zgrid[k] - hblt;
    double R = 1.0 - dh / hwide[k];
    double hup = hwide[k], hdn = hwide[k + 1];
    if (PBC) {
      const double w1 = (k == 1) ? 0.0 : dzt_at(k - 1);
      hdn = (k == km) ? KPP_EPS : dzt_at(k + 1);
      hup = dzt_at(k);
      dh = -zgrid[k - 1] + dzt_at(k) + 0.5 * w1 - hblt;
      R = 1.0 - dh / dzt_at(k);
    }
    double fm[3], f0[3], fp[3];
    fm[0] = visc_at(k - 1); f0[0] = visc_at(k); fp[0] = visc_at(k + 1);
    fm[2] = VDC1[vb + (long long)(k - 1) * n2]; f0[2] = VDC1[vb + (long long)k * n2]; fp[2] = VDC1[vb + (long long)(k + 1) * n2];
    if (!SAME) { fm[1] = VDC2[vb + (long long)(k - 1) * n2]; f0[1] = VDC2[vb + (long long)k * n2]; fp[1] = VDC2[vb + (long long)(k + 1) * n2]; }
    else { fm[1] = fm[2]; f0[1] = f0[2]; fp[1] = fp[2]; }
#pragma unroll
    for (int q = 0; q < 3; ++q) {
      const double up = (fm[q] - f0[q]) / hup, dn = (f0[q] - fp[q]) / hdn;
      const double Pq = 0.5 * ((1.0 - R) * (up + fabs(up)) + R * (dn + fabs(dn)));
      const double Hq = f0[q] + Pq * dh;
      const double wv = (q == 0) ? wm : ws;
      gat1[q] = Hq / hblt / (wv + KPP_EPS);
      dat1[q] = fmin(-Pq / (wv + KPP_EPS) + f1 * Hq, 0.0);
    }
  }
  auto shape = [&](double sig, double wv, int q) {
    return hblt * wv * sig * (1.0 + sig * ((sig - 2.0) + (3.0 - 2.0 * sig) * gat1[q] + (sig - 1.0) * dat1[q]));
  };
  double dkm1[3];
  {
    const int k = kbl - 1;
    const double sig = -zgrid[k] / hblt;
    double wm1, ws1;
    kpp_wscale<true>(fmin(sig, KPP_EPSSFC), hblt, ustar, bfsfc, wm1, ws1);
    dkm1[0] = shape(sig, wm1, 0); dkm1[1] = shape(sig, ws1, 1); dkm1[2] = shape(sig, ws1, 2);
  }
  const double stf1 = STF1[c.q2], stf2 = STF2[c.q2];
  const int kb1 = (kbl - 1 >= 1) ? kbl - 1 : 1;
// ... 19 lines not shown
        const double dzk = (PBC && k > 1) ? dzt_at(k) : g.dz.u(k);
        SRC1[o] = stf1 / dzk * (0.0 - 0.0); SRC2[o] = stf2 / dzk * (0.0 - 0.0);
        if (XS) kp.SRCX[o] = 0.0 - 0.0;
      }
    }
  } else {
  auto load = [&](int k) {
    KppBlRaw r;
    const long long o = c.base3 + (long long)(k - 1) * n2;
    r.visc = VISC[o]; r.vd1 = VDC1[vb + (long long)k * n2]; r.vd2 = SAME ? 0.0 : VDC2[vb + (long long)k * n2]; r.db = DBLOC[o];
    return r;
  };
  auto level = [&](int k, const KppBlRaw &cu, KppBlRaw &nx) {
    nx = load(k + 1 <= km ? k + 1 : km);
    const long long o = c.base3 + (long long)(k - 1) * n2;
    const double zk = zgrid.u(k), zk1 = zgrid.u(k + 1), dz_k = g.dz.u(k);
    double visc = cu.visc, vd1 = cu.vd1, vd2 = SAME ? cu.vd1 : cu.vd2;
    if (k <= km - 1) {
      const double N2 = PBC ? cu.db / (0.5 * (dzt_at(k) + dzt_at(k + 1))) : cu.db / (zk - zk1);
      const double fcon = (N2 > 0.0) ? 0.0 : 1.0;
      double cvv = 0.0, cvd = 0.0;
      if (k >= kbl) { cvv = sp.convect_visc * fcon; cvd = sp.convect_diff * fcon; }
      if (k < kmt) { visc = visc + cvv; vd1 = vd1 + cvd; vd2 = vd2 + cvd; }
      else { visc = 0.0; vd1 = 0.0; vd2 = 0.0; }
    } else { vd1 = 0.0; vd2 = 0.0; }
    VISC[o] = visc;
    VDC1[vb + (long long)k * n2] = vd1;
    if (!SAME) VDC2[vb + (long long)k * n2] = vd2;
    const double fl1 = vd1 * 0.0, fl2 = vd2 * 0.0;
    const double dzk = (PBC && k > 1) ? dzt_at(k) : dz_k;
    const double p1 = (k == 1) ? -fl1 : 0.0 - fl1, p2 = (k == 1) ? -fl2 : 0.0 - fl2;
    SRC1[o] = stf1 / dzk * p1; SRC2[o] = stf2 / dzk * p2;
    if (XS) kp.SRCX[o] = p2;
  };
  {
    KppBlRaw A = load(1), B;
    int k = 1;
#pragma unroll 1
    for (; k + 1 <= km; k += 2) { level(k, A, B); level(k + 1, B, A); }
    if (k <= km) level(k, A, B);
  }
  }
  double flux1_prev = 0.0, flux2_prev = 0.0;
#pragma unroll 1
  for (int k = 1; k <= kbl && k <= km; ++k) {
    const long long o = c.base3 + (long long)(k - 1) * n2;
    const double dzk = (PBC && k > 1) ? dzt_at(k) : g.dz[k];
    if (k == kbl) {
      if (k > 1) { SRC1[o] = stf1 / dzk * (flux1_prev - 0.0); SRC2[o] = stf2 / dzk * (flux2_prev - 0.0); if (XS) kp.SRCX[o] = flux2_prev - 0.0; }
      else if (SPARSE) { SRC1[o] = stf1 / dzk * (-(0.0)); SRC2[o] = stf2 / dzk * (-(0.0)); if (XS) kp.SRCX[o] = -(0.0); }
      break;
    }
    double sig = (-zgrid[k] + 0.5 * hwide[k]) / hblt;
    if (PBC && k > 1) sig = (-zgrid[k - 1] + 0.5 * dzt_at(k - 1) + dzt_at(k)) / hblt;
    double wmk, wsk;
    kpp_wscale<true>(fmin(sig, KPP_EPSSFC), hblt, ustar, bfsfc, wmk, wsk);
    double b0 = shape(sig, wmk, 0), b1 = shape(sig, wsk, 1), b2 = shape(sig, wsk, 2);
    double ghat = (1.0 - stable) * kp.cg / (wsk * hblt + KPP_EPS);
    if (k == kbl - 1 && k <= km - 1) {
      double dh = (hblt + zgrid[k]) / (zgrid[k] - zgrid[k + 1]);
      if (PBC) {
        const double w1 = (k == 1) ? -0.5 * dzt_at(k) : zgrid[k - 1] - 0.5 * (dzt_at(k - 1) + dzt_at(k));
        dh = (hblt + w1) / (0.5 * (dzt_at(k) + dzt_at(k + 1)));
      }
      const double omd = 1.0 - dh;
      b0 = omd * visc_b + dh * ((omd * omd) * dkm1[0] + (dh * dh) * (casea * visc_b + (1.0 - casea) * b0));
      b1 = omd * vd2_b + dh * ((omd * omd) * dkm1[1] + (dh * dh) * (casea * vd2_b + (1.0 - casea) * b1));
      b2 = omd * vd1_b + dh * ((omd * omd) * dkm1[2] + (dh * dh) * (casea * vd1_b + (1.0 - casea) * b2));
      ghat = (1.0 - casea) * ghat;
    }
    double visc = b0, vd2 = b1, vd1 = b2;
    if (k <= km - 1) {
      if (k < kmt) { visc = visc + 0.0; vd1 = vd1 + 0.0; vd2 = vd2 + 0.0; }
      else { visc = 0.0; vd1 = 0.0; vd2 = 0.0; }
    } else { vd1 = 0.0; vd2 = 0.0; }
    VISC[o] = visc;
    VDC1[vb + (long long)k * n2] = vd1;
    if (!SAME) VDC2[vb + (long long)k * n2] = vd2;
    const double fl1 = vd1 * ghat, fl2 = vd2 * ghat;
    if (k == 1) { SRC1[o] = stf1 / dzk * (-fl1); SRC2[o] = stf2 / dzk * (-fl2); if (XS) kp.SRCX[o] = -fl2; }
    else { SRC1[o] = stf1 / dzk * (flux1_prev - fl1); SRC2[o] = stf2 / dzk * (flux2_prev - fl2); if (XS) kp.SRCX[o] = flux2_prev - fl2; }
    flux1_prev = fl1; flux2_prev = fl2;
  }
}

#define POP_VVC_KC 8
__global__ void __launch_bounds__(POP_COL_THREADS)
k_kpp_hmxl(DevGrid g, KppDev kp, const double *__restrict__ T, const double *__restrict__ S, const double *__restrict__ DBSFC,
           double *__restrict__ HMXL, double *__restrict__ HMXL_DR) {
  Col c;
  if (!col_setup(g, c, false)) return;
  const int km = g.km, kmt = g.KMT[c.q2];
  const long long n2 = g.n2;
  const bool pbc = g.pbc != 0;
  const double dzb = pbc ? g.DZBC[c.q2] : 0.0;
  auto dzt = [&](int k) { return pbc_dz(g, k, kmt, dzb); };
  double ustar = 0.0, hmxl = (kmt == 1) ? g.zt[1] : 0.0;
  for (int k = 2; k <= km && k <= kmt; ++k) {
    const double zk = pbc ? g.zt[k - 1] + 0.5 * (dzt(k - 1) + dzt(k)) : g.zt[k];
    const double q = DBSFC[c.base3 + (long long)(k - 1) * n2] / zk;
    ustar = (q > ustar) ? q : ustar;
    hmxl = zk;
  }
  double gm1 = 0.0, dbm1 = DBSFC[c.base3];
  for (int k = 2; k <= km; ++k) {
    const double db = DBSFC[c.base3 + (long long)(k - 1) * n2];
    const double dzk = pbc ? 0.5 * (dzt(k) + dzt(k - 1)) : (g.zt[k] - g.zt[k - 1]);
    const double v = (ustar > 0.0) ? (db - dbm1) / dzk : 0.0;
    if (v >= ustar && (v - gm1) != 0.0 && ustar > 0.0) {
      const double bf = (v - ustar) / (v - gm1);
      hmxl = pbc ? (g.zt[k - 1] + 0.25 * (dzt(k - 1) + dzt(k))) * (1.0 - bf) + (g.zt[k - 1] - 0.25 * (dzt(k - 2) + dzt(k - 1))) * bf
                 : -0.5 * (kp.zgrid[k] + kp.zgrid[k - 1]) * (1.0 - bf) - 0.5 * (kp.zgrid[k - 1] + kp.zgrid[k - 2]) * bf;
      ustar = 0.0;
    }
    gm1 = v; dbm1 = db;
  }
  HMXL[c.q2] = hmxl;
  const MwjfP P1 = mwjf_level(g.pressz[1]);
  const double rho1 = mwjf_rho<false>(P1, tmask(T[c.base3]), S[c.base3], nullptr, nullptr);
  const double target = rho1 + 3.0e-05;
  double rhok = rho1, hdr = (kmt == 1) ? g.zt[1] : 0.0;
  bool found = (kmt == 1);
  for (int k = 1; k <= km - 1; ++k) {
    const long long o = c.base3 + (long long)k * n2;
    const double rkp1 = mwjf_rho<false>(P1, tmask(T[o]), S[o], nullptr, nullptr);
    if (target > rhok && target <= rkp1 && !found) {
      hdr = g.zt[k] + (target - rhok) * (g.zt[k + 1] - g.zt[k]) / (rkp1 - rhok + KPP_EPS);
      found = true;
    }
    rhok = rkp1;
  }
  HMXL_DR[c.q2] = hdr;
}

__global__ void k_kpp_vvc(DevGrid g, const double *__restrict__ VISC, double *__restrict__ VVC, int patch) {
  int p2;
  const int k0 = blockIdx.y * POP_VVC_KC + 1, b = blockIdx.z;
  if (!patch_cell(g, patch, b, p2)) return;
  const int i = p2 % g.nxb, j = p2 / g.nxb, nxb = g.nxb;
  const long long q2 = (long long)b * g.n2 + p2;
  const bool in = i < g.nxb - 1 && j < g.nyb - 1;
  const int kmu = g.KMU[q2];
  const double au0 = g.AU0[q2], aun = g.AUN[q2], aue = g.AUE[q2], aune = g.AUNE[q2];
  const int k1 = min(k0 + POP_VVC_KC - 1, g.km);
  for (int k = k0; k <= k1; ++k) {
    const long long o = (long long)b * g.n3 + (long long)(k - 1) * g.n2 + p2;
    double v = 0.0;
    if (k <= g.km - 1 && k < kmu && in)
      v = au0 * VISC[o] + aun * VISC[o + nxb] + aue * VISC[o + 1] + aune * VISC[o + nxb + 1];
    VVC[o] = v;
  }
}

inline void launch_kpp_vvc(const DevGrid &g, int vp, hipStream_t st, const double *VISC, double *VVC) {
  hipLaunchKernelGGL(k_kpp_vvc, dim3(patch_grid_x(g, vp), (g.km + POP_VVC_KC - 1) / POP_VVC_KC, g.nblocks), dim3(vp ? 64 * vp : 256), 0, st, g, VISC, VVC, vp);
}

struct KppHost {
  TidalDev tidal;
  bool tidal_on = false;
  BckDev bck;
  bool bck_on = false;
  const double *zero_bck = nullptr;
  KppDev dev;
  int *wuk = nullptr;
  unsigned long long *convb = nullptr;
  hipStream_t side = nullptr;
  hipEvent_t ev_fork = nullptr, ev_join = nullptr, ev_bd = nullptr;
};
inline void kpp_destroy(MixDev &m) {
  KppHost *k = (KppHost *)m.kpp;
  if (k) {
    if (k->ev_fork) hipEventDestroy(k->ev_fork);
    if (k->ev_join) hipEventDestroy(k->ev_join);
    if (k->ev_bd) hipEventDestroy(k->ev_bd);
    if (k->side) hipStreamDestroy(k->side);
  }
  delete k; m.kpp = nullptr;
}

inline int sw_chl_index(const SwTab &T, double chl) {
  chl = std::max(chl, T.chlmin); chl = std::min(chl, T.chlmax);
  int idx = (int)(std::log10(chl / T.chlmin) / T.dlogchl);
  return std::min(std::max(idx, 0), 400);
}
inline int sw_tables_create(HostModel &h, std::vector<void *> &allocs, std::string &err) {
  if (h.sw.swabs) return 0;
  const pop_config &c = h.c;
  const int km = h.km, type = c.sw_absorption_type, jt = c.jerlov_water_type ? c.jerlov_water_type : 3;
  const size_t a2 = h.n2 * h.nblocks;
  void *p;
  auto up = [&](const void *src, size_t bytes, void **dst) -> int {
    if (hipMalloc(dst, bytes) != hipSuccess) return 1;
    allocs.push_back(*dst);
    return hipMemcpy(*dst, src, bytes, hipMemcpyHostToDevice) != hipSuccess ? 1 : 0;
  };
  {
    std::vector<double> sa(km + 1, 0.0);
    sa[0] = 1.0;
    if (type == 1) {
      const double rfac[5] = {0.58, 0.62, 0.67, 0.77, 0.78}, depth1[5] = {0.35, 0.60, 1.00, 1.50, 1.40}, depth2[5] = {23.0, 20.0, 17.0, 14.0, 7.90};
      for (int kk = 1; kk <= km - 1; ++kk) {
        const double dm = -h.zw[kk] * 0.01;
        sa[kk] = (dm < -200.0) ? 0.0 : rfac[jt - 1] * std::exp(dm / depth1[jt - 1]) + (1.0 - rfac[jt - 1]) * std::exp(dm / depth2[jt - 1]);
      }
    }
    if (up(sa.data(), sa.size() * 8, &p)) { err = "sw alloc"; return 1; } h.sw.swabs = (double *)p;
  }
  if (type == 2) {
    static const double cnc[31] = {.001, .005, .01, .02, .03, .05, .10, .15, .20, .25, .30, .35, .40, .45, .50, .60, .70, .80, .90, 1.00, 1.50,
      2.00, 2.50, 3.00, 4.00, 5.00, 6.00, 7.00, 8.00, 9.00, 10.00};
    static const double A1t[31] = {0.4421, 0.4451, 0.4488, 0.4563, 0.4622, 0.4715, 0.4877, 0.4993, 0.5084, 0.5159, 0.5223, 0.5278, 0.5326, 0.5369,
      0.5408, 0.5474, 0.5529, 0.5576, 0.5615, 0.5649, 0.5757, 0.5802, 0.5808, 0.5788, 0.56965, 0.55638, 0.54091, 0.52442, 0.50766, 0.49110, 0.47505};
    static const double A2t[31] = {0.2981, 0.2963, 0.2940, 0.2894, 0.2858, 0.2800, 0.2703, 0.2628, 0.2571, 0.2523, 0.2481, 0.2444, 0.2411, 0.2382,
      0.2356, 0.2309, 0.2269, 0.2235, 0.2206, 0.2181, 0.2106, 0.2089, 0.2113, 0.2167, 0.23357, 0.25504, 0.27829, 0.30274, 0.32698, 0.35056, 0.37303};
    static const double B1t[31] = {0.0287, 0.0301, 0.0319, 0.0355, 0.0384, 0.0434, 0.0532, 0.0612, 0.0681, 0.0743, 0.0800, 0.0853, 0.0902, 0.0949,
      0.0993, 0.1077, 0.1154, 0.1227, 0.1294, 0.1359, 0.1640, 0.1876, 0.2082, 0.2264, 0.25808, 0.28498, 0.30844, 0.32932, 0.34817, 0.36540, 0.38132};
    static const double B2t[31] = {0.3192, 0.3243, 0.3306, 0.3433, 0.3537, 0.3705, 0.4031, 0.4262, 0.4456, 0.4621, 0.4763, 0.4889, 0.4999, 0.5100,
      0.5191, 0.5347, 0.5477, 0.5588, 0.5682, 0.5764, 0.6042, 0.6206, 0.6324, 0.6425, 0.66172, 0.68144, 0.70086, 0.72144, 0.74178, 0.76190, 0.78155};
    const int ksol = 2 * km, nsub = 400;
    std::vector<double> ztr(ksol + 1, 0.0), Tr((size_t)(ksol + 1) * (nsub + 1));
    for (int kk = 1; kk <= km; ++kk) { ztr[2 * kk - 1] = h.zt[kk]; ztr[2 * kk] = h.zw[kk]; }
    h.sw.chlmin = cnc[0]; h.sw.chlmax = cnc[30];
    h.sw.dlogchl = (std::log10(h.sw.chlmax) - std::log10(h.sw.chlmin)) / (double)nsub;
    double logchl = std::log10(h.sw.chlmin) - h.sw.dlogchl;
    for (int n = 0; n <= nsub; ++n) {
      logchl = logchl + h.sw.dlogchl;
      const double amount = std::pow(10.0, logchl);
      int mc = -1;
      for (int q = 0; q < 30; ++q) if (cnc[q] <= amount && amount <= cnc[q + 1]) { mc = q; break; }
      if (mc < 0) mc = (amount < cnc[0]) ? 0 : 29;
      const double w2 = (amount - cnc[mc]) / (cnc[mc + 1] - cnc[mc]), w1 = 1.0 - w2;
      const double A1 = A1t[mc] * w1 + A1t[mc + 1] * w2, A2 = A2t[mc] * w1 + A2t[mc + 1] * w2;
      const double B1 = B1t[mc] * w1 + B1t[mc + 1] * w2, B2 = B2t[mc] * w1 + B2t[mc + 1] * w2;
      double *Trn = Tr.data() + (size_t)n * (ksol + 1);
      Trn[0] = 1.0;
      for (int kk = 1; kk <= ksol; ++kk) {
        double arg = std::min(B1 * ztr[kk] * 0.01, 35.0);
// ... 1 lines not shown
        arg = std::min(B2 * ztr[kk] * 0.01, 35.0);
        Trn[kk] = Trn[kk] + A2 * std::exp(-arg);
      }
    }
    if (up(ztr.data(), ztr.size() * 8, &p)) { err = "sw alloc"; return 1; } h.sw.ztr = (double *)p;
    if (up(Tr.data(), Tr.size() * 8, &p)) { err = "sw alloc"; return 1; } h.sw.Tr = (double *)p;
    h.sw.ksol = ksol;
    std::vector<int> ci(a2, sw_chl_index(h.sw, 0.25));
    if (up(ci.data(), a2 * 4, &p)) { err = "sw alloc"; return 1; } h.sw.CHLI = (int *)p;
  }
  return 0;
}
inline int kpp_create(HostModel &h, const Forms &f, const DevGrid &g, MixDev &m, std::vector<void *> &allocs, std::string &err) {
  const pop_config &c = h.c;
  if (c.lshort_wave && (c.sw_absorption_type < 0 || c.sw_absorption_type > 2)) { err = "KPP: sw_absorption_type: 0 top-layer, 1 jerlov, 2 chlorophyll"; return 1; }
  if (c.jerlov_water_type < 0 || c.jerlov_water_type > 5) { err = "KPP: jerlov_water_type: 1..5 (0 = 3)"; return 1; }
  if (c.num_v_smooth_Ri < 1) { err = "KPP: num_v_smooth_Ri must be >= 1 (the reference leaves FRI unset otherwise)"; return 1; }
  const int km = h.km;
  std::vector<double> zgrid(km + 3, 0.0), hwide(km + 3, 0.0), bvdc(km + 3, 0.0), bvvc(km + 3, 0.0);
  const std::vector<int> kref = kpp_kref(h);
  zgrid[0] = KPP_EPS; hwide[0] = KPP_EPS;
  for (int k = 1; k <= km; ++k) { zgrid[k] = -h.zt[k]; hwide[k] = h.dz[k]; }
  zgrid[km + 1] = -h.zw[km]; hwide[km + 1] = KPP_EPS;
  for (int k = 1; k <= km; ++k) {
    bvdc[k] = c.bckgrnd_vdc1 + c.bckgrnd_vdc2 * std::atan(c.bckgrnd_vdc_linv * (h.zw[k] - c.bckgrnd_vdc_dpth));
    bvvc[k] = c.Prandtl * bvdc[k];
  }
  auto up = [&](const void *src, size_t bytes, void **dst) -> int {
    if (hipMalloc(dst, bytes) != hipSuccess) return 1;
    allocs.push_back(*dst);
    return hipMemcpy(*dst, src, bytes, hipMemcpyHostToDevice) != hipSuccess ? 1 : 0;
  };
  KppHost *K = new KppHost();
  m.kpp = K;
  if (f.kpp_side) {
    if (hipStreamCreateWithFlags(&K->side, hipStreamNonBlocking) != hipSuccess ||
        hipEventCreateWithFlags(&K->ev_fork, hipEventDisableTiming) != hipSuccess ||
        hipEventCreateWithFlags(&K->ev_join, hipEventDisableTiming) != hipSuccess ||
        hipEventCreateWithFlags(&K->ev_bd, hipEventDisableTiming) != hipSuccess) { err = "kpp: side stream"; return 1; }
  }
  KppDev &k = K->dev;
  void *p;
  if (up(zgrid.data(), zgrid.size() * 8, &p)) { err = "kpp alloc"; return 1; } k.zgrid = (double *)p;
  if (up(hwide.data(), hwide.size() * 8, &p)) { err = "kpp alloc"; return 1; } k.hwide = (double *)p;
  if (up(bvdc.data(), bvdc.size() * 8, &p)) { err = "kpp alloc"; return 1; } k.bckgrnd_vdc = (double *)p;
  if (up(bvvc.data(), bvvc.size() * 8, &p)) { err = "kpp alloc"; return 1; } k.bckgrnd_vvc = (double *)p;
  if (up(kref.data(), kref.size() * 4, &p)) { err = "kpp alloc"; return 1; } k.kref = (int *)p;
  {
    std::vector<double> z6(6 * (km + 3), 0.0);
    if (up(z6.data(), z6.size() * 8, &p)) { err = "kpp alloc"; return 1; }
    if (km + 1 <= 1024) hipLaunchKernelGGL(k_kpp_level_table, dim3(1), dim3(km + 1), 0, 0, g, (double *)p);
    if (hipDeviceSynchronize() != hipSuccess) { err = "kpp: level table"; return 1; }
    k.eosP = (double *)p;
  }
  const size_t a2 = h.n2 * h.nblocks;
  std::vector<double> z(a2, 0.0);
  if (up(z.data(), a2 * 8, &p)) { err = "kpp alloc"; return 1; } k.HBLT0 = (double *)p;
  if (up(z.data(), a2 * 8, &p)) { err = "kpp alloc"; return 1; } k.USTAR = (double *)p;
  if (up(z.data(), a2 * 8, &p)) { err = "kpp alloc"; return 1; } k.BFSFC = (double *)p;
  std::vector<int> zi(a2, 0);
  if (up(zi.data(), a2 * 4, &p)) { err = "kpp alloc"; return 1; } k.KBL0 = (int *)p;
  if (up(zi.data(), a2 * 4, &p)) { err = "kpp alloc"; return 1; } k.KBL = (int *)p;
  if (up(zi.data(), a2 * 4, &p)) { err = "kpp alloc"; return 1; } K->wuk = (int *)p;
  { std::vector<unsigned long long> zb(a2, 0ull); if (up(zb.data(), a2 * 8, &p)) { err = "kpp alloc"; return 1; } K->convb = (unsigned long long *)p; }
  k.CONVB = nullptr; k.src_clear_all = 0;
  k.WUK = nullptr; k.wu_margin = 3;
  k.Vtc = std::sqrt(0.2 / KPP_C_S / KPP_EPSSFC) / (KPP_VONKAR * KPP_VONKAR);
  k.cg = KPP_CSTAR * KPP_VONKAR * std::pow(KPP_C_S * KPP_VONKAR * KPP_EPSSFC, 1.0 / 3.0);
  k.rich_mix = c.kpp_rich_mix; k.lrich = c.lrich; k.ldbl_diff = c.ldbl_diff; k.nsmooth = c.num_v_smooth_Ri;
  k.lshort_wave = c.lshort_wave ? 1 : 0; k.sw_type = c.sw_absorption_type; k.jerlov = c.jerlov_water_type ? c.jerlov_water_type : 3; k.lcheckekmo = c.lcheckekmo ? 1 : 0;
  if (k.lshort_wave) {
    if (up(z.data(), a2 * 8, &p)) { err = "kpp alloc"; return 1; } k.BO = (double *)p;
    if (up(z.data(), a2 * 8, &p)) { err = "kpp alloc"; return 1; } k.BOSOL = (double *)p;
  }
  if (k.lshort_wave && k.sw_type == 2) {
    if (sw_tables_create(h, allocs, err)) return 1;
    k.ztr = h.sw.ztr; k.Tr = h.sw.Tr; k.ksol = h.sw.ksol; k.CHLI = h.sw.CHLI;
  }
  return 0;
}

inline const int *mix_kpp_kbl(const MixDev &m) { return m.kpp ? ((const KppHost *)m.kpp)->dev.KBL : nullptr; }

inline int kpp_vmix_coeffs(const HostModel &h, const Forms &f, const DevGrid &g, const StepParams &sp, const MixDev &m, const MixState &s,
                           hipStream_t st, std::string &err) {
  const KppHost &KH = *(const KppHost *)m.kpp;
  KppDev g_kpp = KH.dev;
  g_kpp.SHF_QSW = s.SHF_QSW; g_kpp.FCORT = g.FCORT;
  if (s.KBL) g_kpp.KBL = s.KBL;
  g_kpp.vdc_same = (s.VDC[0] == s.VDC[1]) ? 1 : 0;
  if (KH.tidal_on || KH.bck_on) { g_kpp.bckgrnd_vdc = KH.zero_bck; g_kpp.bckgrnd_vvc = KH.zero_bck; }
  const dim3 GC(col_grid(g, POP_COL_THREADS), g.nblocks), BC(POP_COL_THREADS);
  const dim3 G3((g.n2 + 255) / 256, g.km, g.nblocks);
  double *DBLOC = s.S3a, *DBSFC = s.S3b, *WU = s.S3c, *VISC = s.S3d, *RIW = s.E3;
  const dim3 GL(col_grid_x(g.n2, POP_COL_THREADS), g.nblocks), BL(POP_COL_THREADS, 4);

  struct Sel {
    bool shear_col;
    int buoy;
    int buoy_kr; bool buoy_sfc;
    bool depth_lazy; int depth_kr;
    int interior;
    bool same, sparse;
    bool side, wuk, convb;
  } sel{f.kpp_shear_col, f.kpp_buoy, f.kpp_buoy_kr, f.kpp_buoy_sfc, f.kpp_depth_lazy, f.kpp_depth_kr, f.kpp_interior,
        g_kpp.vdc_same != 0, f.kpp_sparse, f.kpp_side, f.kpp_wuk, f.kpp_sparse};
  g_kpp.WUK = sel.wuk ? KH.wuk : nullptr;
  g_kpp.wu_margin = f.kpp_wuk_margin;
  g_kpp.CONVB = sel.convb ? KH.convb : nullptr;
  g_kpp.src_clear_all = s.src_clear_all;
  g_kpp.SRCX = s.KPP_SRCX;

  const hipStream_t side = sel.side ? KH.side : nullptr, su = side ? side : st;
  if (side) { hipEventRecord(KH.ev_fork, st); hipStreamWaitEvent(side, KH.ev_fork, 0); }
  with_flags([&](auto COL, auto PBC) {
    if constexpr (COL.value) hipLaunchKernelGGL((k_kpp_ushear_col<24, PBC.value>), GC, BC, 0, su, g, g_kpp, s.UMIX, s.VMIX, WU);
    else hipLaunchKernelGGL(k_kpp_ushear<PBC.value>, G3, dim3(256), 0, su, g, g_kpp, s.UMIX, s.VMIX, WU);
  }, sel.shear_col, g.pbc);
  const auto T0 = s.TMIX[0], T1 = s.TMIX[1];
  if (sel.buoy == KPP_BUOY_MARCH) with_flags([&](auto PBC) { hipLaunchKernelGGL(k_kpp_buoy_interior_march<PBC.value>, GC, BC, 0, st, g, g_kpp, T0, T1, s.UMIX, s.VMIX, DBLOC, VISC, s.VDC[0], s.VDC[1]); }, g.pbc);
  else if (sel.buoy == KPP_BUOY_FUSED_LDS) with_flags([&](auto SFC) { hipLaunchKernelGGL((k_kpp_buoy_interior_lds<20, 8, SFC.value>), GL, dim3(POP_COL_THREADS, 8), 0, st, g, g_kpp, T0, T1, s.UMIX, s.VMIX, DBLOC, DBSFC, VISC, s.VDC[0], s.VDC[1]); }, sel.buoy_sfc);
  else if (sel.buoy == KPP_BUOY_LDS) with_value<20, 28>(sel.buoy_kr, [&](auto KR) { hipLaunchKernelGGL((k_kpp_buoydiff_lds<KR.value, 4>), GL, BL, 0, st, g, g_kpp, T0, T1, DBLOC, DBSFC); });
  else with_flags([&](auto SFC) { hipLaunchKernelGGL(k_kpp_buoydiff<SFC.value>, G3, dim3(256), 0, st, g, g_kpp, T0, T1, DBLOC, DBSFC); }, sel.buoy_sfc);
  auto depth = [&](hipStream_t sd) {
    with_flags([&](auto LAZY, auto KR28, auto PBC) {
      if constexpr (!KR28.value || (LAZY.value && !PBC.value))
        hipLaunchKernelGGL((k_kpp_bldepth<LAZY.value, KR28.value ? 28 : 20, PBC.value>), GC, BC, 0, sd, g, g_kpp, T0, T1, s.STF[0], s.STF[1], (const double *)DBLOC, (const double *)DBSFC, (const double *)WU, s.UMIX, s.VMIX);
    }, sel.depth_lazy, sel.depth_kr == 28, g.pbc);
  };
  if (side) {
    hipEventRecord(KH.ev_bd, st); hipStreamWaitEvent(side, KH.ev_bd, 0);
    depth(side);
    hipEventRecord(KH.ev_join, side);
  }
  if (sel.interior == KPP_INTERIOR_REG) with_value<60, 62>(g.km, [&](auto KM) { hipLaunchKernelGGL(k_kpp_interior_reg<KM.value>, GC, BC, 0, st, g, g_kpp, T0, T1, s.UMIX, s.VMIX, (const double *)DBLOC, VISC, s.VDC[0], s.VDC[1]); });
  else if (sel.interior == KPP_INTERIOR_GENERIC) with_flags([&](auto PBC) { hipLaunchKernelGGL(k_kpp_interior<PBC.value>, GC, BC, 0, st, g, g_kpp, T0, T1, s.UMIX, s.VMIX, (const double *)DBLOC, RIW, VISC, s.VDC[0], s.VDC[1]); }, g.pbc);
  if (KH.tidal_on) {
    TidalDev td = KH.tidal;
    if (KH.bck_on) { td.B2 = KH.bck.VDC; td.BPR2 = KH.bck.VVC_PR; }
    with_flags([&](auto PBC, auto HV) { hipLaunchKernelGGL((k_kpp_tidal<PBC.value, HV.value>), GC, BC, 0, st, g, td, (int)g_kpp.vdc_same, (const double *)DBLOC, VISC, s.VDC[0], s.VDC[1]); }, g.pbc, KH.bck_on);
  } else if (KH.bck_on) hipLaunchKernelGGL(k_kpp_bckgrnd, GC, BC, 0, st, g, KH.bck, (int)g_kpp.vdc_same, VISC, s.VDC[0], s.VDC[1]);
  if (side) hipStreamWaitEvent(st, KH.ev_join, 0);
  else depth(st);
  with_flags([&](auto PBC, auto SAME, auto SPARSE, auto XS) {
    hipLaunchKernelGGL((k_kpp_blmix<PBC.value, SAME.value, SPARSE.value, XS.value>), GC, BC, 0, st, g, sp, g_kpp, (const double *)DBLOC, s.STF[0], s.STF[1], VISC, s.VDC[0], s.VDC[1], s.KPP_SRC[0], s.KPP_SRC[1], s.HBLT);
  }, g.pbc, sel.same, sel.sparse, g_kpp.SRCX != nullptr);
  launch_kpp_vvc(g, f.del4_tile_rows, st, (const double *)VISC, s.VVC);
  if (h.c.kpp_ml_diagnostics == 1 && s.HMXL && s.HMXL_DR)
    hipLaunchKernelGGL(k_kpp_hmxl, GC, BC, 0, st, g, g_kpp, T0, T1, (const double *)DBSFC, s.HMXL, s.HMXL_DR);
  if (hipGetLastError() != hipSuccess) { err = "KPP kernel launch failed"; return 1; }
  return 0;
}

}
```

pop2-cesm_amd/csrc/kernels_mix.hpp:

```cpp
#pragma once
#include "kernels_common.hpp"

namespace pop {

struct MixDev {
  const double *bckgrnd_vdc = nullptr, *bckgrnd_vvc = nullptr, *zgrid = nullptr, *hwide = nullptr, *Ricr = nullptr;
  const double *D4AMF = nullptr, *D4AHF = nullptr;
  const double *d4DTN = nullptr, *d4DTS = nullptr, *d4DTE = nullptr, *d4DTW = nullptr;
  const double *d4DUC = nullptr, *d4DUN = nullptr, *d4DUS = nullptr, *d4DUE = nullptr, *d4DUW = nullptr;
  const double *d4DMC = nullptr, *d4DMN = nullptr, *d4DMS = nullptr, *d4DME = nullptr, *d4DMW = nullptr, *d4DUM = nullptr;
  void *kpp = nullptr;
};
struct MixState {
  const double *TMIX[2], *UMIX, *VMIX, *UCUR, *VCUR, *RHOMIX, *STF[2], *SHF_QSW;
  double *VDC[2], *VVC, *KPP_SRC[2], *HBLT, *HMXL, *HMXL_DR;
  int *KBL = nullptr;
  int src_clear_all = 0;
  double *S3a, *S3b, *S3c, *S3d, *E3, *F3;
  double *KPP_SRCX = nullptr;
};

template <bool PBC>
__global__ void k_rich_t(DevGrid g, StepParams sp, MixState s, double *__restrict__ RICH) {
  const int p2 = blockIdx.x * blockDim.x + threadIdx.x;
// ... 16 lines not shown
      auto shear = [&](const double *A, long long d) {
        const int kmu = g.KMU[q2 + d];
        const double dzub = g.DZUB[q2 + d];
        return (A[ok + d] - A[okp + d]) / (0.5 * (pbc_dz(g, k, kmu, dzub) + pbc_dz(g, kp1, kmu, dzub)));
      };
      double ut = 0.0, vt = 0.0;
      if (i >= 1 && j >= 1) {
        ut = 0.25 * shear(s.UMIX, 0) + 0.25 * shear(s.UMIX, -nxb) + 0.25 * shear(s.UMIX, -1) + 0.25 * shear(s.UMIX, -1 - nxb);
        vt = 0.25 * shear(s.VMIX, 0) + 0.25 * shear(s.VMIX, -nxb) + 0.25 * shear(s.VMIX, -1) + 0.25 * shear(s.VMIX, -1 - nxb);
      }
      const double dzb = g.DZBC[q2];
      const double h = 0.5 * (pbc_dz(g, k, kmt, dzb) + pbc_dz(g, kp1, kmt, dzb));
      rich = -sp.grav * (rhok - s.RHOMIX[okp]) / h / (ut * ut + vt * vt + 1.0e-10 / (h * h));
    } else {
      const double du = u2t(s.UMIX, ok) - u2t(s.UMIX, okp), dv = u2t(s.VMIX, ok) - u2t(s.VMIX, okp);
      rich = -sp.grav * g.dzw[k] * (rhok - s.RHOMIX[okp]) / (du * du + dv * dv + 1.0e-10);
    }
    const double f = 1.0 + 5.0 * rich;
    vdc = fmin(critnu, sp.rich_bckgrnd_vdc + (sp.rich_bckgrnd_vvc + sp.rich_mix / (f * f)) / f);
  }
  if (rich < 0.0) vdc = critnu;
  RICH[ok] = rich;
  s.VDC[0][((long long)b * (g.km + 2) + k) * g.n2 + p2] = vdc;
}
__global__ void k_rich_u(DevGrid g, StepParams sp, MixState s, const double *__restrict__ RICH) {
  const int p2 = blockIdx.x * blockDim.x + threadIdx.x;
  const int k = blockIdx.y + 1, b = blockIdx.z;
  if (p2 >= g.n2) return;
  const int i = p2 % g.nxb, j = p2 / g.nxb, nxb = g.nxb;
  const long long q2 = (long long)b * g.n2 + p2, ok = (long long)b * g.n3 + (long long)(k - 1) * g.n2 + p2;
  double richu = 0.0;
  if (i < g.nxb - 1 && j < g.nyb - 1)
    richu = g.AU0[q2] * RICH[ok] + g.AUN[q2] * RICH[ok + nxb] + g.AUE[q2] * RICH[ok + 1] + g.AUNE[q2] * RICH[ok + nxb + 1];
  const double critnu = sp.convect_visc;
  double vvc;
  if (k < g.KMU[q2]) { const double f = 1.0 + 5.0 * richu; vvc = fmin(critnu, sp.rich_bckgrnd_vvc + sp.rich_mix / (f * f)); }
  else { richu = 0.0; vvc = 0.0; }
  if (richu < 0.0) vvc = critnu;
  s.VVC[ok] = vvc;
}

__global__ void k_state_points(DevGrid g, int kk, const double *__restrict__ T, const double *__restrict__ S, double *__restrict__ rho,
                               double *__restrict__ drdt, double *__restrict__ drds, long long n) {
  const long long p = (long long)blockIdx.x * blockDim.x + threadIdx.x;
  if (p >= n) return;
  const MwjfP P = mwjf_level(g.pressz[kk]);
  double a, b;
  rho[p] = mwjf_rho<true>(P, T[p], S[p], &a, &b);
  if (drdt) drdt[p] = a;
  if (drds) drds[p] = b;
}
inline int mix_state_host(const HostModel &h, const DevGrid &g, int kk, const double *T, const double *S, double *rho, double *drdt,
                          double *drds, long long n, hipStream_t st, std::string &err) {
  if (kk < 1 || kk > h.km) { err = "state: kk out of range"; return 1; }
  double *d = nullptr;
  if (hipMalloc((void **)&d, sizeof(double) * 5 * n) != hipSuccess) { err = "state: hipMalloc failed"; return 1; }
  hipMemcpyAsync(d, T, sizeof(double) * n, hipMemcpyHostToDevice, st);
  hipMemcpyAsync(d + n, S, sizeof(double) * n, hipMemcpyHostToDevice, st);
  hipLaunchKernelGGL(k_state_points, dim3((unsigned)((n + 255) / 256)), dim3(256), 0, st, g, kk, d, d + n, d + 2 * n, d + 3 * n, d + 4 * n, n);
  hipMemcpyAsync(rho, d + 2 * n, sizeof(double) * n, hipMemcpyDeviceToHost, st);
  if (drdt) hipMemcpyAsync(drdt, d + 3 * n, sizeof(double) * n, hipMemcpyDeviceToHost, st);
  if (drds) hipMemcpyAsync(drds, d + 4 * n, sizeof(double) * n, hipMemcpyDeviceToHost, st);
  const hipError_t e = hipStreamSynchronize(st);
  hipFree(d);
  if (e != hipSuccess) { err = std::string("state: ") + hipGetErrorString(e); return 1; }
  return 0;
}

}

#include "kernels_del4.hpp"
#include "kernels_tidal.hpp"
#include "kernels_bckgrnd.hpp"
#include "kernels_kpp.hpp"

namespace pop {

inline int mix_create(HostModel &h, const Forms &f, const DevGrid &g, MixDev &m, std::vector<void *> &allocs, std::string &err) {
  if ((h.c.hmix_momentum == 4 || h.c.hmix_tracer == 4) && del4_create(h, g, m, allocs, err)) return 1;
  if (h.c.vmix_choice == 3 && kpp_create(h, f, g, m, allocs, err)) return 1;
  return 0;
}
inline int mix_vmix_coeffs(const HostModel &h, const Forms &f, const DevGrid &g, const StepParams &sp, const MixDev &m, const MixState &s,
                           hipStream_t st, std::string &err) {
  const dim3 G3((g.n2 + 255) / 256, g.km, g.nblocks);
  if (h.c.vmix_choice == 2) {
    with_flags([&](auto PBC) { hipLaunchKernelGGL(k_rich_t<PBC.value>, G3, dim3(256), 0, st, g, sp, s, s.S3c); }, g.pbc);
    hipLaunchKernelGGL(k_rich_u, G3, dim3(256), 0, st, g, sp, s, (const double *)s.S3c);
    return 0;
  }
  if (h.c.vmix_choice == 3) return kpp_vmix_coeffs(h, f, g, sp, m, s, st, err);
  err = "unknown vmix_choice";
  return 1;
}

}
```

pop2-cesm_amd/csrc/kernels_passive.hpp:

```cpp
#pragma once
#include "kernels_common.hpp"

namespace pop {

struct KppSrcPassiveArgs { const double *STF[2]; double *SRC[2]; };
template <bool PBC = false>
__global__ void __launch_bounds__(256)
k_kpp_src_passive(DevGrid g, const double *__restrict__ X, KppSrcPassiveArgs a, int np) {
  const int p2 = blockIdx.x * blockDim.x + threadIdx.x;
  const int k = blockIdx.y + 1, b = blockIdx.z / np, n = blockIdx.z % np;
  if (p2 >= g.n2) return;
  const long long q2 = (long long)b * g.n2 + p2, o = (long long)b * g.n3 + (long long)(k - 1) * g.n2 + p2;
  const double dzk = (PBC && k > 1) ? pbc_dz(g, k, g.KMT[q2], g.DZBC[q2]) : g.dz[k];
  a.SRC[n][o] = a.STF[n][q2] / dzk * X[o];
}

struct AvgPassiveArgs { double *TO[2], *TC[2]; const double *TN[2]; const double *PO, *PC, *PN; double dz1, grav; };
__global__ void __launch_bounds__(256)
k_avg_passive(DevGrid g, AvgPassiveArgs a, int np) {
  const int p2 = blockIdx.x * blockDim.x + threadIdx.x;
  const int k = blockIdx.y + 1, b = blockIdx.z / np, n = blockIdx.z % np;
  if (p2 >= g.n2) return;
  const long long q = (long long)b * g.n2 + p2, o = (long long)b * g.n3 + (long long)(k - 1) * g.n2 + p2;
  const double to = a.TO[n][o], tc = a.TC[n][o], tn = a.TN[n][o];
  if (k >= 2) {
    a.TO[n][o] = 0.5 * (to + tc);
    a.TC[n][o] = 0.5 * (tc + tn);
    return;
  }
  const double po = a.PO[q], pc = a.PC[q], pn = a.PN[q];
  const double pfo = 0.5 * (po + pc), pfc = 0.5 * (pc + pn);
  double t = 0.5 * ((a.dz1 + po / a.grav) * to + (a.dz1 + pc / a.grav) * tc);
  t = t / (a.dz1 + pfo / a.grav);
  const double mn = fmin(to, tc), mx = fmax(to, tc);
  if (t < mn) t = mn;
  if (t > mx) t = mx;
  a.TO[n][o] = t;
  double t2 = 0.5 * ((a.dz1 + pc / a.grav) * tc + (a.dz1 + pn / a.grav) * tn);
  t2 = t2 / (a.dz1 + pfc / a.grav);
  const double mn2 = fmin(tc, tn), mx2 = fmax(tc, tn);
  if (t2 < mn2) t2 = mn2;
  if (t2 > mx2) t2 = mx2;
  a.TC[n][o] = t2;
}

__global__ void k_rf_surface_div(DevGrid g, RfParams p, const double *__restrict__ PC, const double *__restrict__ PN,
                                 double *__restrict__ TC, double *__restrict__ TN) {
  const long long q2 = (long long)blockIdx.x * blockDim.x + threadIdx.x;
  if (q2 >= (long long)g.n2 * g.nblocks) return;
  const long long b = q2 / g.n2, q = b * g.n3 + (q2 - b * g.n2);
  if (p.nonzero_new) TN[q] = TN[q] / (p.dz1 + PN[q2] / p.grav);
  TC[q] = TC[q] / (p.dz1 + PC[q2] / p.grav);
}

}
```

pop2-cesm_amd/csrc/kernels_tidal.hpp:

```cpp
#pragma once

namespace pop {

struct TidalDev {
  const double *COEF = nullptr;
  const int *BOX = nullptr;
  CArr zgrid, bvdc, bvvc_pr;
  const double *B2 = nullptr, *BPR2 = nullptr;
  CArr minval;
  CArrI klev;
  double mix_max = 0.0, prandtl = 0.0;
  int lmax = 0, stabc = 0;
  double *DIFF = nullptr, *N2 = nullptr, *KV = nullptr, *KVM = nullptr;
};

struct TidalRaw { double db, co, visc, vd1, vd2; };
template <bool PBC = false, bool HV = false>
__global__ void __launch_bounds__(POP_COL_THREADS)
k_kpp_tidal(DevGrid g, TidalDev td, int vdc_same, const double *__restrict__ DBLOC, double *__restrict__ VISC,
            double *__restrict__ VDC1, double *__restrict__ VDC2) {
  Col c;
  if (!col_setup(g, c, false)) return;
  const int km = g.km;
  const long long n2 = g.n2;
  const int kmt = g.KMT[c.q2];
  if (kmt < 2) return;
  const long long vb = ((long long)c.b * (km + 2)) * n2 + c.p2;
  const double dzbc = PBC ? g.DZBC[c.q2] : 0.0;
  double hb = 0.0, hbpr = 0.0;
  if constexpr (HV) { hb = td.B2[c.q2]; hbpr = td.BPR2[c.q2]; }
  double rmin = 0.0; int klo = km + 1;
  if (td.BOX) {
    const int r = td.BOX[c.q2];
    if (r > 0) {
      rmin = td.minval[r];
      const int kl = td.klev[r];
      if (kl == 2) klo = max(3, kmt - 2);
      else if (kl == 6) klo = max(7, kmt - 6);
    }
  }
  auto load = [&](int k) {
    TidalRaw r;
    const long long o = c.base3 + (long long)(k - 1) * n2;
    r.db = DBLOC[o]; r.co = td.COEF[o]; r.visc = VISC[o]; r.vd1 = VDC1[vb + (long long)k * n2];
    r.vd2 = vdc_same ? 0.0 : VDC2[vb + (long long)k * n2];
    return r;
  };
  TidalRaw cu = load(1);
  double prev = 0.0;
#pragma unroll 1
  for (int k = 1; k < kmt; ++k) {
    const TidalRaw nx = load(k + 1 < kmt ? k + 1 : k);
    const long long o = c.base3 + (long long)(k - 1) * n2;
    const double h = PBC ? 0.5 * (pbc_dz(g, k, kmt, dzbc) + pbc_dz(g, k + 1, kmt, dzbc)) : td.zgrid[k] - td.zgrid[k + 1];
    const double N2 = cu.db / h;
    double t = (N2 > 0.0) ? cu.co / N2 : 0.0;
    if (td.lmax) t = fmin(t, td.mix_max);
    if (td.stabc && k > 2 && k >= kmt - 2) t = fmax(t, prev);
    if (k >= klo) t = fmax(t, rmin);
    prev = t;
    const double kv = fmin((HV ? hb : td.bvdc[k]) + t, td.mix_max);
    const double kvm = td.prandtl * fmin((HV ? hbpr : td.bvvc_pr[k]) + t, td.mix_max);
    VISC[o] = cu.visc + kvm;
    VDC1[vb + (long long)k * n2] = cu.vd1 + kv;
    if (!vdc_same) VDC2[vb + (long long)k * n2] = cu.vd2 + kv;
    if (td.DIFF) { td.DIFF[o] = t; td.N2[o] = N2; td.KV[o] = kv; td.KVM[o] = kvm; }
    cu = nx;
  }
}

}
```

pop2-cesm_amd/csrc/pop_amd.hip:

```cpp
#include <hip/hip_runtime.h>
#include <algorithm>
#include <chrono>
#include <unordered_map>
#include "kernels_baroclinic.hpp"
#include "kernels_barotropic.hpp"
#include "kernels_mix.hpp"
#include "kernels_thomas_reg.hpp"
#include "kernels_momentum_lds.hpp"
#include "kernels_aniso.hpp"
#include "kernels_submeso.hpp"
#include "kernels_tracer_lds.hpp"
#include "kernels_rf.hpp"
#include "kernels_pcsi.hpp"
#include "kernels_evp.hpp"
#include "kernels_lwlim.hpp"
#include "kernels_gm.hpp"
#include "kernels_passive.hpp"
#include "kernels_ice.hpp"
#include "kernels_pcg_persist.hpp"
#include "kernels_tavg.hpp"
#include "kernels_diag.hpp"
#include "kernels_moc.hpp"
#include "rccl_transport.hpp"

// ... 72 lines not shown
    if (name == "TIDAL_N2") return ok(td.N2, a3);
    if (name == "KVMIX") return ok(td.KV, a3);
    if (name == "KVMIX_M") return ok(td.KVM, a3);
  }
  if (name == "GM_GTK") return (n == 0 || n == 1) ? ok(c->gm.GTK[n], a3) : (n >= 2 && n < c->h.nt && c->h.c.hmix_tracer == 3) ? ok(c->PW[n], a3) : 1;
  if (name == "HDU") return ok(c->HDU, a3);
  if (name == "HDV") return ok(c->HDV, a3);
  if (name == "F_PARA") return ok(c->FPARA, a3);
  if (name == "F_PERP") return ok(c->FPERP, a3);
  if (name == "QICE") return ok(c->ice.QICE, a2);
  if (name == "AQICE") return ok(c->ice.AQICE, a2);
  if (name == "QFLUX") return ok(c->ice.QFLUX, a2);
  if (name == "FW_FREEZE") return ok(c->ice.FWF, a2);
  if (name == "SMF") return ok(c->d2[n == 0 ? "SMF1" : "SMF2"], a2);
  if (name == "SMFT") return ok(c->d2[n == 0 ? "SMFT1" : "SMFT2"], a2);
  auto it = c->d2.find(name);
  if (it != c->d2.end()) return ok(it->second, a2);
  return 1;
}

int unknown(pop_ctx *c, const char *what, const char *name) { c->err = std::string(what) + name; return 1; }
int field_arg(pop_ctx *c, const char *name, int tl, int n, double **ptr, long long *count) {
  if (!resolve(c, name, tl, n, ptr, count)) return 0;
  for (const char *f : {"TRACER", "STF", "TFW", "KPP_SRC", "GM_GTK", "SUBM_ADV_TEND"})
    if (!strcmp(name, f) && (n < 0 || n >= c->h.nt)) { c->err = std::string(name) + ": tracer index " + std::to_string(n) + " is outside 0 .. nt-1 = " + std::to_string(c->h.nt - 1); return 1; }
  return unknown(c, "unknown field ", name);
}
int mask_arg(pop_ctx *c, const char *name, double **ptr) {
  long long cnt;
  *ptr = nullptr;
  return name && resolve(c, name, 0, 0, ptr, &cnt) ? unknown(c, "unknown mask ", name) : 0;
}
int count_is(pop_ctx *c, long long have, long long want, const char *name) {
  if (have == want) return 0;
  c->err = name ? std::string("count mismatch for ") + name : std::string("count mismatch");
  return 1;
}
template <class V, class T>
int copy_out(pop_ctx *c, const V &v, T *host, long long count, const char *name) {
  if (count_is(c, (long long)v.size(), count, name)) return 1;
  std::copy(v.begin(), v.end(), host);
  return 0;
}
void mark_written(pop_ctx *c, const char *name, int tl) {
  const std::string nm(name);
  if (nm == "KPP_SRC") { c->kpp_src_user = true; c->src_dirty = true; c->src_dirty_alt = true; }
  if (nm == "TRACER") c->tr_ghosts_ok[time_index(c, tl)] = false;
  if (nm == "UVEL" || nm == "VVEL") c->uv_ghosts_ok[time_index(c, tl)] = false;
  for (const char *f : {"TRACER", "UVEL", "VVEL", "RHO", "PSURF", "GRADPX", "GRADPY", "UBTROP", "VBTROP", "PGUESS", "FW_OLD"})
    if (nm == f) c->full_left = c->f.land_full_steps;
}
int loc_kind_ok(pop_ctx *c, int loc, int kind, const char *text) {
  if (loc >= 0 && loc <= 3 && kind >= 0 && kind <= 2) return 0;
  c->err = text;
  return 1;
}
int single_rank_only(pop_ctx *c) {
  if (c->h.nranks == 1) return 0;
  c->err = "host halo update needs all blocks on one rank";
  return 1;
}

}

extern "C" {

int pop_create(const pop_config *cfg, int rank, int nranks, int flags, pop_ctx **out) { return pop_create_tuned(cfg, nullptr, nullptr, rank, nranks, flags, out); }
int pop_create_with_grid(const pop_config *cfg, const pop_grid_input *grid, int rank, int nranks, int flags, pop_ctx **out) {
  return pop_create_tuned(cfg, grid, nullptr, rank, nranks, flags, out);
}

#define POP_TUNING_FIELDS(X)                                                                                                            \
  X(land_skip, "POP_LAND_SKIP") X(land_full_steps, "POP_LAND_FULL_STEPS") X(xcd_remap, "POP_XCD_REMAP")   \
  X(red_band, "POP_RED_BAND") X(lds_order, "POP_LDS_ORDER") X(momentum_lds, "POP_MOMENTUM_LDS") X(tracer_lds, "POP_TRACER_LDS")         \
  X(generic_thomas, "POP_GENERIC_THOMAS") X(reg_thomas_t, "POP_REG_THOMAS_T") X(thomas_pair, "POP_THOMAS_PAIR")                         \
  X(tracer_fwd, "POP_TRACER_FWD") X(vdc_shared, "POP_VDC_SHARED") X(side_stream, "POP_SIDE_STREAM") X(del4_side, "POP_DEL4_SIDE")       \
  X(del4_tile, "POP_DEL4_TILE") X(d2t_fuse, "POP_D2T_FUSE") X(d2u_fuse, "POP_D2U_FUSE") X(vmixu_defer, "POP_VMIXU_DEFER")               \
  X(vmixu_inline, "POP_VMIXU_INLINE") X(btrop_inline, "POP_BTROP_INLINE") X(kpp_ahead, "POP_KPP_AHEAD") X(kpp_col, "POP_KPP_COL")       \
  X(kpp_lazy, "POP_KPP_LAZY") X(kpp_ushear_hint, "POP_KPP_USHEAR_HINT") X(kpp_ushear_margin, "POP_KPP_USHEAR_MARGIN")                   \
  X(kpp_side_stream, "POP_KPP_SIDE_STREAM") X(kpp_interior_generic, "POP_KPP_INTERIOR_GENERIC") \
  X(kpp_src_full, "POP_KPP_SRC_FULL") X(solver_unfused, "POP_SOLVER_UNFUSED") X(solver_nograph, "POP_SOLVER_NOGRAPH")                   \
  X(solver_presum, "POP_SOLVER_PRESUM") X(solver_distributed, "POP_SOLVER_DISTRIBUTED") X(solver_overlap_off, "POP_SOLVER_OVERLAP_OFF") \
  X(fpcg_b2, "POP_FPCG_B2") X(pcsi_step2, "POP_PCSI_STEP2") X(halo_separate, "POP_HALO_SEPARATE")                                       \
  X(halo_overlap_off, "POP_HALO_OVERLAP_OFF") X(rccl_overlap, "POP_RCCL_OVERLAP") X(evp_wave, "POP_EVP_WAVE") X(fpcg_a_pair, "POP_FPCG_A_PAIR") X(kpp_sparse, "POP_KPP_SPARSE") X(pbc_generic_thomas, "POP_PBC_GENERIC_THOMAS") X(pbc_generic_kpp, "POP_PBC_GENERIC_KPP") X(state3d_levels, "POP_STATE3D_LEVELS") X(gm_sf_stored, "POP_GM_SF_STORED") X(pcg_persist, "POP_PCG_PERSIST") X(gm_flux_tile, "POP_GM_FLUX_TILE") X(pcsi_two_step, "POP_PCSI_TWO_STEP") X(block_sums_relay, "POP_BLOCK_SUMS_RELAY") X(aniso_side, "POP_ANISO_SIDE") X(submeso_all_levels, "POP_SUBMESO_ALL_LEVELS")
void pop_tuning_init(pop_tuning *t) {
  if (!t) return;
  t->struct_bytes = (int)sizeof(pop_tuning);
#define X(f, e) t->f = POP_TUNING_UNSET;
  POP_TUNING_FIELDS(X)
#undef X
}
static void tuning_resolve(pop_tuning &t, const pop_tuning *user) {
  pop_tuning_init(&t);
  if (user && user->struct_bytes == (int)sizeof(pop_tuning)) t = *user;
  auto env = [](const char *name, int &v) {
    const char *e = getenv(name);
    if (!e) return;
    char *end = nullptr;
    const long x = strtol(e, &end, 10);
    v = (end == e) ? 1 : (int)x;
  };
#define X(f, e) env(e, t.f);
  POP_TUNING_FIELDS(X)
#undef X
}
int pop_get_tuning(const pop_ctx *c, pop_tuning *resolved) {
  if (!c || !resolved) return 1;
  *resolved = c->h.tun;
  return 0;
}

int pop_read_grid_files(const char *horiz_grid_file, const char *topography_file, int nx_global, int ny_global, double *seven_records, int *kmt) {
  const size_t n = (size_t)nx_global * ny_global;
  auto slurp = [&](const char *path, void *dst, size_t bytes) {
    FILE *f = fopen(path, "rb");
    if (!f) return 1;
    const size_t got = fread(dst, 1, bytes, f);
    fclose(f);
    return got == bytes ? 0 : 1;
  };
  if (horiz_grid_file && seven_records && slurp(horiz_grid_file, seven_records, 7 * n * sizeof(double))) return 1;
  if (topography_file && kmt && slurp(topography_file, kmt, n * sizeof(int))) return 2;
  return 0;
}

int pop_create_tuned(const pop_config *cfg_in, const pop_grid_input *grid, const pop_tuning *tuning, int rank, int nranks, int flags, pop_ctx **out) {
  if (!cfg_in || !out || nranks < 1 || rank < 0 || rank >= nranks) return 1;
  pop_ctx *c = new pop_ctx();
  *out = c;
  if (cfg_in->struct_version == POP_CONFIG_VERSION) c->h.c = *cfg_in;
  else if (cfg_in->struct_version == 6) memcpy(&c->h.c, cfg_in, offsetof(pop_config, lsubmesoscale_mixing));
  else memcpy(&c->h.c, cfg_in, offsetof(pop_config, aniso_alignment));
  const pop_config *cfg = &c->h.c;
  c->h.rank = rank; c->h.nranks = nranks;
  if (cfg->hmix_tracer == 3 && cfg->gm_transition_layer == 1 && cfg->vmix_choice == 3) c->h.c.kpp_ml_diagnostics = 1;
  if (cfg->lsubmesoscale_mixing == 1 && cfg->vmix_choice == 3) c->h.c.kpp_ml_diagnostics = 1;
  if (tuning && tuning->struct_bytes != (int)sizeof(pop_tuning)) { c->err = "pop_create_tuned: pop_tuning.struct_bytes does not match this library (use pop_tuning_init)"; return 1; }
  tuning_resolve(c->h.tun, tuning);
  c->grid_from_input = grid != nullptr;
  if (grid && !(grid->ULAT && grid->ULON && grid->HTN && grid->HTE && grid->HUS && grid->HUW)) { c->err = "pop_create_with_grid: ULAT, ULON, HTN, HTE, HUS, HUW are required"; return 1; }
  c->h.gin = grid;
  {
    auto bad = [&](const std::string &m) { c->err = "pop_create: " + m; return 1; };
    if (cfg->struct_version != POP_CONFIG_VERSION && cfg->struct_version != 6 && cfg->struct_version != 5) return bad("pop_config.struct_version is " + std::to_string(cfg->struct_version) + ", this library reads 5, 6 and " + std::to_string(POP_CONFIG_VERSION) + " (include/pop_amd.h)");
    if (cfg->reserved_i[0] != 0) return bad("pop_config.reserved_i must be 0");
    if (cfg->gm_kappa_bkg_srfbl != 0 && cfg->gm_kappa_bkg_srfbl != 1) return bad("gm_kappa_bkg_srfbl: 0 or 1");
    if (cfg->ah_bkg_bottom < 0.0) return bad("ah_bkg_bottom: >= 0");
    if (cfg->gm_diag_bolus != 0 && cfg->gm_diag_bolus != 1) return bad("gm_diag_bolus: 0 or 1");
    if (cfg->gm_diag_bolus && cfg->hmix_tracer != 3) return bad("gm_diag_bolus needs hmix_tracer = 3");
    if (cfg->gm_transition_layer != 0 && cfg->gm_transition_layer != 1) return bad("gm_transition_layer: 0 or 1");
    if (cfg->gm_transition_layer && cfg->hmix_tracer != 3) return bad("gm_transition_layer needs hmix_tracer = 3");
    if (cfg->hmix_tracer == 3 && cfg->partial_bottom_cells) return bad("hmix_tracer = 3 (Gent-McWilliams) with partial_bottom_cells: the reference refuses the combination (hmix_gm.F90:782-785), so does this library");
    if (cfg->hmix_tracer == 3 && cfg->gm_kappa_type == 2 && cfg->kappa_depth_2 == 0.0) return bad("gm_kappa_type = 2 ('depth') needs kappa_depth_2 /= 0 (hmix_gm.F90:724-730)");
    if (cfg->hmix_tracer == 3 && cfg->gm_kappa_type == 1 && cfg->gm_kappa_freq == 0) return bad("gm_kappa_type = 1 ('bfre') needs gm_kappa_freq = 1 | 2: 'kappa_freq should not be set to never when model fields dependent kappa types are chosen' (hmix_gm.F90:756-780; no N^2 file here)");
    if (cfg->gm_kappa_type < 0 || cfg->gm_kappa_type > 2) return bad("gm_kappa_type: 0 constant, 1 bfre, 2 depth (the other kappa choices of hmix_gm_nml are not built)");
    if (cfg->gm_kappa_freq < 0 || cfg->gm_kappa_freq > 2) return bad("gm_kappa_freq: 0 never, 1 every_time_step, 2 once_a_day");
    if (cfg->gm_kappa_freq == 2 && cfg->tmix_opt == 1) return bad("gm_kappa_freq = once_a_day with time_mix_opt 'avg' (half steps that do not fit the day: the end-of-day test of time_management.F90:3586-3592 on the calendar) is not built: avgfit, robert or none");
    if (cfg->gm_slope_control < 0 || cfg->gm_slope_control > 3) return bad("gm_slope_control: 0 notanh, 1 tanh, 2 clip, 3 Gerd");
    if (cfg->gm_slope_control == 2 && cfg->gm_transition_layer) return bad("gm_slope_control = clip with the transition layer (SLA_SAVE is formed before the slopes are clipped, hmix_gm.F90:1234-1245) is not built");
    if (cfg->ah_bolus < 0.0 || cfg->ah_bkg_srfbl < 0.0 || cfg->slm_r < 0.0 || cfg->slm_b < 0.0) return bad("ah_bolus, ah_bkg_srfbl, slm_r, slm_b: >= 0 (0 = ah, ah, 0.3, 0.3)");
    if (cfg->partial_bottom_cells != 0 && cfg->partial_bottom_cells != 1) return bad("partial_bottom_cells: 0 or 1");
    if (cfg->partial_bottom_cells && grid && grid->DZBC == nullptr && grid->KMT != nullptr) return bad("partial_bottom_cells with a topography record needs pop_grid_input.DZBC (the record of bottom_cell_file)");
    if (cfg->lsw_absorb != 0 && cfg->lsw_absorb != 1) return bad("lsw_absorb: 0 or 1");
    if (cfg->nx_global < 1 || cfg->ny_global < 1 || cfg->km < 2 || cfg->block_size_x < 1 || cfg->block_size_y < 1) return bad("domain / block sizes must be positive (km >= 2)");
    if (cfg->ew_boundary != 0 && cfg->ew_boundary != 1) return bad("ew_boundary: 0 closed, 1 cyclic");
    if (cfg->ns_boundary < 0 || cfg->ns_boundary > 2) return bad("ns_boundary: 0 closed, 1 cyclic, 2 tripole");
    if (cfg->hmix_momentum == 3 && cfg->struct_version < 6) return bad("hmix_momentum = 3 (anis) needs pop_config struct_version 6: the hmix_aniso_nml members (include/pop_amd.h)");
// ... 450 lines not shown
      const size_t nsb = (size_t)E.xnb * E.ynb, S = nsb * h.nblocks;
      constexpr int NC = EVP_LD * EVP_LD, NR = EVP_LE * EVP_LE;
      std::vector<int4> meta(S);
      std::vector<double> cc(S * NC), ne(S * NC), icc(S * NC), ine(S * NC), rinv(S * NR);
      for (int lb = 0; lb < h.nblocks; ++lb) {
        const size_t gb = (size_t)h.local_ids[lb] - 1;
        for (int j = 1; j <= E.ynb; ++j) for (int i = 1; i <= E.xnb; ++i) {
          const size_t sl = lb * nsb + (size_t)(j - 1) * E.xnb + (i - 1), sg = gb * nsb + (size_t)(j - 1) * E.xnb + (i - 1);
          const int is = E.xidx[i], ie = E.xidx[i + 1] + 1, js = E.yidx[j], je = E.yidx[j + 1] + 1;
          int ocean = 0;
          {
            const std::vector<int> &KMT = h.i2.at("KMT");
            for (int cj = js + 1; cj <= je - 1; ++cj) for (int ci = is + 1; ci <= ie - 1; ++ci)
              if (KMT[gb * h.n2 + (size_t)(cj - 1) * h.nxb + (ci - 1)] > 0) ocean = 1;
          }
          meta[sl] = make_int4((int)(lb * h.n2 + (size_t)(js - 1) * h.nxb + (is - 1)), (ie - is + 1) | ((je - js + 1) << 8), E.land[sg], (E.land[sg] && !ocean) ? 1 : 0);
          for (int q = 0; q < NC; ++q) {
            cc[q * S + sl] = E.cc[sg * NC + q]; ne[q * S + sl] = E.ne[sg * NC + q];
            icc[q * S + sl] = E.icc[sg * NC + q]; ine[q * S + sl] = E.ine[sg * NC + q];
          }
          for (int q = 0; q < NR; ++q) rinv[q * S + sl] = E.rinv[sg * NR + q];
        }
      }
      int4 *dm; double *d0, *d1, *d2, *d3, *d4;
      if (dev_upload(c, &dm, meta.data(), S) || dev_upload(c, &d0, cc.data(), cc.size()) || dev_upload(c, &d1, ne.data(), ne.size()) ||
          dev_upload(c, &d2, icc.data(), icc.size()) || dev_upload(c, &d3, ine.data(), ine.size()) || dev_upload(c, &d4, rinv.data(), rinv.size())) return 1;
      c->evp = EvpDev{(long long)S, dm, d0, d1, d2, d3, d4, c->d2["evpC0"], c->d2["btropWgtNE"]};
      c->use_evp = true;
    }
    if (f.pcsi_two_step || f.pcsi_two_step_dist) {
      if (dev_alloc(c, &c->pcsi_raw, a2)) return 1;
      std::vector<int> jfold;
      pcsi_fold_local(h, c->h_srcmap, jfold);
      if (cfg->ns_boundary == 2 && dev_upload(c, &c->pcsi_jfold, jfold.data(), jfold.size())) return 1;
    }
    if (f.replicated) {
      const size_t NG = h.n2 * h.nblocks_tot;
      SolveView &v = c->gv;
      v.g = c->g; v.g.nblocks = h.nblocks_tot;
      double *p;
      if (dev_upload(c, &p, h.f2["btropWgtNE"].data(), NG)) return 1; v.g.WNE = p;
      if (dev_upload(c, &p, h.f2["btropWgtEast"].data(), NG)) return 1; v.g.WEa = p;
      if (dev_upload(c, &p, h.f2["btropWgtNorth"].data(), NG)) return 1; v.g.WNo = p;
      if (dev_upload(c, &p, h.f2["btropXW"].data(), NG)) return 1; v.g.XW = p;
      if (dev_upload(c, &p, h.f2["btropYW"].data(), NG)) return 1; v.g.YW = p;
      if (dev_upload(c, &p, h.f2["centerWgtIndep"].data(), NG)) return 1; v.g.WC0 = p;
      if (dev_upload(c, &p, h.f2["mMask"].data(), NG)) return 1; v.g.mMask = p;
      { std::vector<unsigned char> m8(NG); for (size_t q = 0; q < NG; ++q) m8[q] = h.f2["mMask"][q] != 0.0;
        unsigned char *d8; if (dev_upload(c, &d8, m8.data(), NG)) return 1; v.g.mMask8 = d8; }
      if (dev_upload(c, &c->gTAREA, h.f2["TAREA"].data(), NG)) return 1;
      if (dev_upload(c, &c->gKMT, h.i2["KMT"].data(), NG)) return 1;
      double **vecs[] = {&v.X, &v.R, &v.Z, &v.S0, &v.S1, &v.Q, &v.RHS, &v.C};
      for (auto q : vecs) if (dev_alloc(c, q, NG)) return 1;
      if (dev_alloc(c, &v.partial, (size_t)c->nchunk * h.nblocks_tot * 2 + POP_RELAY_SLACK) || dev_alloc(c, &v.blocksum, (size_t)h.nblocks_tot * 4)) return 1;
      std::vector<int> gsm = global_srcmap(h), gid(h.nblocks_tot);
      for (int b = 0; b < h.nblocks_tot; ++b) gid[b] = b;
      if (dev_upload(c, &v.srcmap, gsm.data(), gsm.size()) || dev_upload(c, &v.gid, gid.data(), gid.size())) return 1;
      v.nchunk = c->nchunk; v.nblocks_tot = h.nblocks_tot;
    }
  }
  if (cfg->vmix_choice == 1) {
    std::vector<double> v((size_t)(h.km + 2) * a2, cfg->const_vdc), w(a3, cfg->const_vvc);
    HIPCHK(c, hipMemcpy(c->VDC[0], v.data(), v.size() * sizeof(double), hipMemcpyHostToDevice));
    HIPCHK(c, hipMemcpy(c->VVC, w.data(), w.size() * sizeof(double), hipMemcpyHostToDevice));
  }
  if (mix_create(c->h, f, c->g, c->mix, c->allocs, c->err)) return 1;
  c->KBL = const_cast<int *>(mix_kpp_kbl(c->mix));
  if (cfg->lsw_absorb != 0 && sw_tables_create(c->h, c->allocs, c->err)) return 1;
  if (c->h.sw.CHLI) {
    std::vector<double> chl((size_t)c->g.n2 * c->g.nblocks, 0.25);
    HIPCHK(c, hipMemcpy(c->CHL, chl.data(), chl.size() * sizeof(double), hipMemcpyHostToDevice));
  }
  if (f.kpp_ahead) {
    for (int n = 0; n < 2; ++n) if (dev_alloc(c, &c->KPPa[n], a3)) return 1;
    if (h.nt > 2 && dev_alloc(c, &c->KPPXa, a3)) return 1;
    if (dev_alloc(c, &c->VDCa[0], (size_t)(h.km + 2) * a2)) return 1;
    if (f.vdc_shared) c->VDCa[1] = c->VDCa[0];
    else if (dev_alloc(c, &c->VDCa[1], (size_t)(h.km + 2) * a2)) return 1;
    if (dev_alloc(c, &c->VVCa, a3) || dev_alloc(c, &c->HBLTa, a2) || dev_alloc(c, &c->KBLa, a2)) return 1;
    if (c->h.c.kpp_ml_diagnostics == 1 && (dev_alloc(c, &c->HMXLa, a2) || dev_alloc(c, &c->HMXL_DRa, a2))) return 1;
    HIPCHK(c, hipStreamCreateWithFlags(&c->ahead, hipStreamNonBlocking));
    HIPCHK(c, hipEventCreateWithFlags(&c->ev_ahead_fork, hipEventDisableTiming));
    HIPCHK(c, hipEventCreateWithFlags(&c->ev_ahead, hipEventDisableTiming));
  }
  c->oldt = 0; c->curt = 1; c->newt = 2; c->mixt = 1;
  for (int t = 0; t < 3; ++t) {
    HIPCHK(c, hipMemcpy(c->TR[0][t], h.f3["TEMP0"].data(), a3 * sizeof(double), hipMemcpyHostToDevice));
    HIPCHK(c, hipMemcpy(c->TR[1][t], h.f3["SALT0"].data(), a3 * sizeof(double), hipMemcpyHostToDevice));
  }
  launch_state3d(c->g, c->TR[0][c->curt], c->TR[1][c->curt], c->RHO[c->curt], c->stream);
  launch_state3d(c->g, c->TR[0][c->oldt], c->TR[1][c->oldt], c->RHO[c->oldt], c->stream);
  HIPCHK(c, hipStreamSynchronize(c->stream));
  h.f3.clear();
  return 0;
}

int pop_destroy(pop_ctx *c) {
  if (c) for (hipEvent_t &e : c->ev_solve) if (e) { hipEventDestroy(e); e = nullptr; }
  if (!c) return 0;
  for (auto &g : c->graphs) hipGraphExecDestroy(g.exec);
  if (c->host_sc) hipHostFree(c->host_sc);
  if (c->host_rr) hipHostFree(c->host_rr);
  if (c->persist_out) hipHostFree(c->persist_out);
  if (c->diag.h_pre || c->diag.h_after || c->diag.h_cfl) {
    if (c->stream) hipStreamSynchronize(c->stream);
    for (double *p : {c->diag.h_pre, c->diag.h_after, c->diag.h_cfl}) if (p) hipHostFree(p);
  }
  if (c->ev_fork) hipEventDestroy(c->ev_fork);
  if (c->ev_d2t) hipEventDestroy(c->ev_d2t);
  if (c->ev_d2u) hipEventDestroy(c->ev_d2u);
  if (c->ev_vmixu) hipEventDestroy(c->ev_vmixu);
  if (c->ahead) { hipStreamSynchronize(c->ahead); hipStreamDestroy(c->ahead); }
  if (c->ev_ahead_fork) hipEventDestroy(c->ev_ahead_fork);
  if (c->ev_ahead) hipEventDestroy(c->ev_ahead);
  if (c->ev_sa) hipEventDestroy(c->ev_sa);
  if (c->ev_sx) hipEventDestroy(c->ev_sx);
  for (auto &e : c->chk_ev) if (e) hipEventDestroy(e);
  if (c->rccl_tr) {
    if (c->stream) hipStreamSynchronize(c->stream);
    if (c->comm_side) hipStreamSynchronize(c->comm_side);
    if (c->rccl_tr->comm2) rccl().CommDestroy(c->rccl_tr->comm2);
    if (c->rccl_tr->comm) rccl().CommDestroy(c->rccl_tr->comm);
    delete c->rccl_tr;
  }
  if (c->comm_side) hipStreamDestroy(c->comm_side);
  if (c->side) { hipStreamSynchronize(c->side); hipStreamDestroy(c->side); }
  kpp_destroy(c->mix);
  for (void *p : c->allocs) hipFree(p);
  if (c->own_stream && c->stream) hipStreamDestroy(c->stream);
  delete c;
  return 0;
}
const char *pop_last_error(const pop_ctx *c) { return c ? c->err.c_str() : "null context"; }

int pop_get_dim(const pop_ctx *c, const char *name) {
  const std::string n(name);
  if (n == "nx_block") return c->h.nxb;
  if (n == "ny_block") return c->h.nyb;
  if (n == "km") return c->h.km;
  if (n == "nt") return c->h.nt;
  if (n == "nblocks") return c->h.nblocks;
  if (n == "nblocks_tot") return c->h.nblocks_tot;
  if (n == "nblocks_x") return c->h.nbx;
  if (n == "nblocks_y") return c->h.nby;
  if (n == "nghost") return NGHOST;
  if (n == "oldtime") return c->oldt;
  if (n == "curtime") return c->curt;
  if (n == "newtime") return c->newt;
  if (n == "leapfrogts") return c->leapfrogts;
  if (n == "land_skip_active") return c->g.skip;
  if (n == "kpp_ahead_used") return c->ahead_swaps;
  if (n == "d2t_fused") return c->f.d2t_fuse;
  if (n == "d2u_fused") return c->f.d2u_fuse;
  if (n == "d2t_last_formed") return c->d2t_last_formed;
  if (n == "d2u_last_formed") return c->d2u_last_formed;
  if (n == "avg_ts") return c->avg_ts;
  if (n == "eod") return c->eod;
  if (n == "eod_last") return c->eod_last;
  if (n == "nsteps_total") return c->nsteps_total;
  if (n == "nsteps_per_interval") return c->h.nsteps_per_interval;
  if (n == "solver_stream_ops") return (int)c->solver_ops;
  if (n == "solver_iterations_enqueued") return (int)c->solver_enq;
  if (n == "rank") return c->h.rank;
  if (n == "nranks") return c->h.nranks;
  if (n == "solver_chunks_per_block") return c->nchunk;
  if (n == "solver_chunks_listed") return c->red_act ? c->red_nact : -1;
  if (n == "solver_chunks_active") return c->red_active_total;
  if (n == "pcg_persist_used") return c->persist_used;
  if (n == "pcg_persist_gave_up") return c->persist_gave_up;
  if (n == "pcsi_two_step") return (c->f.pcsi_two_step || c->f.pcsi_two_step_dist) ? 1 : 0;
  if (n == "pcg_persist_workgroups") return c->persist_nwg;
  if (n == "pcg_persist_chunks_per_workgroup") return c->persist_cp;
  if (n == "solver_path") return c->h.plan_only ? 0 : c->f.path;
  if (n == "thomas_register_tracers") return c->f.reg_thomas_t;
  if (n == "thomas_register_velocity") return c->f.reg_thomas_u;
  if (n == "max_blocks_per_rank") return max_blocks_per_rank(c->h);
  if (n == "ocean_columns_local") return (int)c->h.ocean_cols_local;
  if (n == "ocean_columns_total") return (int)c->h.ocean_cols_total;
  if (n == "lat_aux_region_start") return (c->moc.aux.inited && c->moc.aux.n_reg > 1) ? c->moc.aux.region_start[1] : 0;
  if (n == "moc_stream") return c->moc.requested ? c->moc.stream : 0;
  if (n.compare(0, 5, "form_") == 0 && !c->h.plan_only) return forms_get(c->f, n.substr(5));
  return -1;
}
double pop_get_scalar(const pop_ctx *c, const char *name) {
  const std::string n(name);
  if (n == "dtt") return c->h.dtt;
  if (n == "dtu") return c->h.dtu;
  if (n == "dtp") return c->h.dtp;
  if (n == "residualNorm") return c->h.residualNorm;
  if (n == "convergenceCriterion") return c->h.convergenceCriterion;
  if (n == "rcheck") return c->h.rcheck;
  if (n == "rconst") return c->h.rconst;
  if (n == "uarea_equator") return c->h.uarea_equator;
  if (n == "rmsResidual") return c->rmsResidual;
  if (n == "land_tile_fraction") return c->land_fraction;
  if (n == "PcsiMaxEigs") return c->h.pcsi_max_eig;
  if (n == "PcsiMinEigs") return c->h.pcsi_min_eig;
  if (n == "lanczos_steps") return (double)c->h.pcsi_lanczos_steps;
  if (n == "robert_curtime") return c->h.robert_curtime;
  if (n == "robert_newtime") return c->h.robert_newtime;
  if (n == "rf_volume_2_km") return c->h.rf_volume_2_km;
  if (n == "open_ocean_volume_2_km") return c->h.open_ocean_volume_2_km;
  if (n == "bgtarea_t_1") return c->h.bgtarea_t_1;
  if (n == "persist_iterations") return c->persist_out ? c->persist_out[0] : NAN;
  if (n == "persist_rr") return c->persist_out ? c->persist_out[1] : NAN;
  if (n == "persist_status") return c->persist_out ? c->persist_out[2] : NAN;
  if (n == "persist_checks") return c->persist_out ? c->persist_out[3] : NAN;
  if (n == "tlast_ice") return c->ice.inited ? c->ice.tlast_ice : NAN;
  if (n == "time_weight") return ice_time_weight(c);
  if (n == "cp_over_lhfusion") return c->ice.inited ? c->ice.k.cp_over_lhfusion : NAN;
  if (n == "rf_S1") return c->rf_S[0];
  if (n == "rf_S2") return c->rf_S[1];
  if (n == "rf_S_prev1") return c->rf_S_prev_valid[0] ? c->rf_S_prev[0] : NAN;
  if (n == "rf_S_prev2") return c->rf_S_prev_valid[1] ? c->rf_S_prev[1] : NAN;
  if (n == "solver_ms_total") { solve_collect(const_cast<pop_ctx *>(c)); return c->solver_ms_total; }
  if (n == "solver_iterations_total") { solve_collect(const_cast<pop_ctx *>(c)); return (double)c->solver_iters_total; }
  if (n == "solver_calls_total") { solve_collect(const_cast<pop_ctx *>(c)); return (double)c->solver_calls_total; }
  if (n == "solver_ms_reset") { pop_ctx *m = const_cast<pop_ctx *>(c); solve_collect(m); m->solver_ms_total = 0; m->solver_iters_total = 0; m->solver_calls_total = 0; return 0.0; }
  return NAN;
}
int pop_get_block(const pop_ctx *c, int block_id, int *out8, int *i_glob, int *j_glob) {
  if (block_id < 1 || block_id > c->h.nblocks_tot) return 1;
  const BlockInfo &B = c->h.all_blocks[block_id - 1];
  if (out8) { int v[8] = {B.block_id, B.local_id, B.ib, B.ie, B.jb, B.je, B.iblock, B.jblock}; std::copy(v, v + 8, out8); }
  if (i_glob) std::copy(B.i_glob.begin(), B.i_glob.end(), i_glob);
  if (j_glob) std::copy(B.j_glob.begin(), B.j_glob.end(), j_glob);
  return 0;
}
int pop_local_block_ids(const pop_ctx *c, int *ids) { std::copy(c->h.local_ids.begin(), c->h.local_ids.end(), ids); return 0; }

long long pop_field_count(const pop_ctx *c, const char *name) {
  const std::string n(name);
  const long long a2 = (long long)c->h.n2 * c->h.nblocks, a3 = (long long)c->h.n3 * c->h.nblocks;
  for (const char *s : {"TRACER", "UVEL", "VVEL", "RHO", "KPP_SRC", "VVC", "UISOP", "VISOP", "WISOP", "GM_SF_SLX", "GM_SF_SLY", "HDU", "HDV", "F_PARA", "F_PERP",
// ... 225 lines not shown
  c->eod = (cf.tmix_opt == 2) ? (c->nsteps_this_interval == c->h.nsteps_per_interval) : (c->nsteps_total % cf.steps_per_day == 0);
  if (c->first_step) { c->leapfrogts = 0; c->f_euler_ts = 1; c->first_step = 0; }
  if (cf.tmix_opt == 1 && c->nsteps_total % cf.time_mix_freq == 0) c->avg_ts = 1;
  if (cf.tmix_opt == 2) {
    const int n = c->nsteps_this_interval;
    if (n == 2) c->avg_ts = 1;
    else if (n != 1 && (n + 1) % cf.time_mix_freq != 0 && n % cf.time_mix_freq == 0) c->avg_ts = 1;
  }
  if (c->leapfrogts) { c->mixt = c->oldt; c->beta = 1.0 / 3.0; c->c2dtt = 2.0 * c->h.dt[1]; c->c2dtu = 2.0 * c->h.dtu; c->c2dtp = 2.0 * c->h.dtp; }
  else { c->mixt = c->curt; c->beta = 0.5; c->c2dtt = c->h.dt[1]; c->c2dtu = c->h.dtu; c->c2dtp = c->h.dtp; }
  tavg_set_flag(c);
  c->tavg.in_step = !c->host_only;
  c->diag.run_global = c->diag.arm_global; c->diag.run_cfl = c->diag.arm_cfl;
  c->diag.arm_global = c->diag.arm_cfl = false;
  return 0;
}

int pop_dhdt(pop_ctx *c) {
  if (need_device(c)) return 1;
  ScopedPhase ph(c, "DHDT");
  hipLaunchKernelGGL(k_dhdt, dim3(col_grid(c->g, 256), c->g.nblocks), dim3(256), 0, c->stream, c->g, step_params(c),
                     c->PS[c->curt], c->PS[c->oldt], c->FW_OLD, c->DH, c->DHU);
  HIPCHK(c, hipGetLastError());
  if (c->tavg.active && tavg_site(c, TS_FORCING)) return 1;
  return 0;
}

static MixState kpp_mix_state(pop_ctx *c, int slot, bool into_alt) {
  MixState ms{};
  for (int n = 0; n < 2; ++n) {
    ms.TMIX[n] = c->TR[n][slot]; ms.STF[n] = c->STF[n];
    ms.KPP_SRC[n] = into_alt ? c->KPPa[n] : c->KPP_SRC[n]; ms.VDC[n] = into_alt ? c->VDCa[n] : c->VDC[n];
  }
  ms.UMIX = c->U[slot]; ms.VMIX = c->V[slot]; ms.UCUR = c->U[c->curt]; ms.VCUR = c->V[c->curt]; ms.RHOMIX = c->RHO[slot];
  ms.VVC = into_alt ? c->VVCa : c->VVC; ms.SHF_QSW = c->SHF_QSW; ms.HBLT = into_alt ? c->HBLTa : c->HBLT;
  ms.HMXL = (into_alt && c->HMXLa) ? c->HMXLa : c->HMXL; ms.HMXL_DR = (into_alt && c->HMXL_DRa) ? c->HMXL_DRa : c->HMXL_DR;
  ms.KBL = into_alt ? c->KBLa : c->KBL;
  ms.KPP_SRCX = into_alt ? c->KPPXa : c->KPPX;
  ms.src_clear_all = (into_alt ? c->src_dirty_alt : c->src_dirty) ? 1 : 0;
  (into_alt ? c->src_dirty_alt : c->src_dirty) = false;
  ms.S3a = c->S3a; ms.S3b = c->S3b; ms.S3c = c->S3c; ms.S3d = c->S3d; ms.E3 = c->E3; ms.F3 = c->F3;
  return ms;
}
static int phase_kpp_src_passive(pop_ctx *c) {
  for (int n = 2; n < c->h.nt; n += 2) {
    const int np = std::min(2, c->h.nt - n);
    KppSrcPassiveArgs a{};
    for (int s = 0; s < np; ++s) { a.STF[s] = c->STF[n + s]; a.SRC[s] = c->KPP_SRC[n + s]; }
    const dim3 G((c->g.n2 + 255) / 256, c->g.km, c->g.nblocks * np);
    with_flags([&](auto PBC) { hipLaunchKernelGGL(k_kpp_src_passive<PBC.value>, G, dim3(256), 0, c->stream, c->g, (const double *)c->KPPX, a, np); }, c->g.pbc);
  }
  HIPCHK(c, hipGetLastError());
  return 0;
}
static int phase_vmix(pop_ctx *c) {
  const pop_config &cf = c->h.c;
  const StepParams sp = step_params(c);
  if (cf.vmix_choice == 1)
    hipLaunchKernelGGL(k_vmix_const, grid_3d(c), dim3(256), 0, c->stream, c->g, sp, c->TR[0][c->mixt], c->TR[1][c->mixt], c->VDC[0], c->VVC);
  else {
    if (c->ahead_valid && c->ahead_slot == c->mixt) {
      HIPCHK(c, hipStreamWaitEvent(c->stream, c->ev_ahead, 0));
      c->ahead_valid = false; c->kpp_src_user = false; ++c->ahead_swaps;
      for (int n = 0; n < 2; ++n) { std::swap(c->VDC[n], c->VDCa[n]); std::swap(c->KPP_SRC[n], c->KPPa[n]); }
      std::swap(c->VVC, c->VVCa); std::swap(c->HBLT, c->HBLTa); std::swap(c->KBL, c->KBLa); std::swap(c->src_dirty, c->src_dirty_alt);
      if (c->HMXLa) { std::swap(c->HMXL, c->HMXLa); std::swap(c->HMXL_DR, c->HMXL_DRa); }
      std::swap(c->KPPX, c->KPPXa);
      return c->h.nt > 2 ? phase_kpp_src_passive(c) : 0;
    }
    if (ahead_cancel(c)) return 1;
    const MixState ms = kpp_mix_state(c, c->mixt, false);
    if (mix_vmix_coeffs(c->h, c->f, c->g, sp, c->mix, ms, c->stream, c->err)) return 1;
    c->kpp_src_user = false;
    if (cf.vmix_choice == 3 && c->h.nt > 2) return phase_kpp_src_passive(c);
  }
  return 0;
}
static int kpp_look_ahead(pop_ctx *c) {
  if (!c->f.kpp_ahead || c->avg_ts || c->h.c.tmix_opt == 3 || (c->h.c.kpp_ml_diagnostics == 1 && !c->HMXLa) ||
      (c->tidal.on && c->tidal.nml.tidal_diag)) return 0;
  HIPCHK(c, hipEventRecord(c->ev_ahead_fork, c->stream));
  HIPCHK(c, hipStreamWaitEvent(c->ahead, c->ev_ahead_fork, 0));
  const MixState ms = kpp_mix_state(c, c->curt, true);
  if (mix_vmix_coeffs(c->h, c->f, c->g, step_params(c), c->mix, ms, c->ahead, c->err)) return 1;
  HIPCHK(c, hipEventRecord(c->ev_ahead, c->ahead));
  c->ahead_valid = true; c->ahead_slot = c->curt;
  return 0;
}
static SubmDev submeso_dev(pop_ctx *c) {
  SubmDev W = c->subm;
  W.HMXL = (c->h.c.vmix_choice == 3) ? c->HMXL : nullptr;
  W.grav = step_params(c).grav; W.sqrt_grav = std::sqrt(W.grav);
  return W;
}
static int submeso_flux_launch(pop_ctx *c, const SubmDev &W, const double *X0, const double *X1, bool tz0 = false) {
  if (W.TD[0]) {
    const size_t bytes = (size_t)c->g.n3 * c->g.nblocks * sizeof(double);
    HIPCHK(c, hipMemsetAsync(W.TD[0], 0, bytes, c->stream));
    HIPCHK(c, hipMemsetAsync(W.TD[1], 0, bytes, c->stream));
  }
  const dim3 GT(((c->g.nxb + POP_SUBM_TX - 1) / POP_SUBM_TX) * ((c->g.nyb + POP_SUBM_TY - 1) / POP_SUBM_TY), c->g.nblocks);
  with_flags([&](auto TZ0) { hipLaunchKernelGGL(k_submeso_flux<TZ0.value>, GT, dim3(POP_SUBM_TX, POP_SUBM_TY), 0, c->stream, c->g, W, X0, X1); }, tz0);
  return 0;
}
static int phase_submeso(pop_ctx *c, const double *T, const double *S) {
  const SubmDev W = submeso_dev(c);
  const dim3 G2((c->g.n2 + 255) / 256, c->g.nblocks);
  hipLaunchKernelGGL(k_submeso_column, G2, dim3(256), 0, c->stream, c->g, W, T, S);
  if (submeso_flux_launch(c, W, T, S)) return 1;
  if (W.US) hipLaunchKernelGGL(k_submeso_vel, G2, dim3(256), 0, c->stream, c->g, W);
  HIPCHK(c, hipGetLastError());
  return 0;
}
static void gm_flux_launch(pop_ctx *c, const GmDev &G, const double *X0, const double *X1, bool add) {
  const dim3 G3((c->g.n2 + 255) / 256, c->g.km, c->g.nblocks);
  const StepParams sp = step_params(c);
  double *v1 = (sp.nvdc == 2 && c->VDC[1] != c->VDC[0]) ? c->VDC[1] : nullptr;
  if (c->f.gm_lds && (G.cancellation || G.SF[0])) {
    constexpr int R = 8;
    const dim3 GT(((c->g.nxb + 62) / 63) * ((c->g.nyb + R - 2) / (R - 1)), (c->g.km + POP_GM_KC - 1) / POP_GM_KC, G3.z);
    with_flags([&](auto CANC, auto ADD) {
      hipLaunchKernelGGL((k_gm_flux_tile<R, CANC.value, ADD.value>), GT, dim3(64, R), 0, c->stream, c->g, G, X0, X1, c->VDC[0], v1);
    }, G.cancellation, add);
  } else
  with_flags([&](auto ADD) {
    hipLaunchKernelGGL(k_gm_flux<ADD.value>, dim3(G3.x, (c->g.km + POP_GM_KC - 1) / POP_GM_KC, G3.z), dim3(256), 0, c->stream, c->g, G, X0, X1, c->VDC[0], v1);
  }, add);
}
static GmDev gm_dev(pop_ctx *c) {
  GmDev G = c->gm;
  G.HBLT = (c->h.c.vmix_choice == 3) ? c->HBLT : nullptr;
  if (G.tlt) G.HMXL = (c->h.c.vmix_choice == 3) ? c->HMXL : nullptr;
  return G;
}
static int phase_hmix_gm(pop_ctx *c) {
  const double *T = c->TR[0][c->mixt], *S = c->TR[1][c->mixt];
  const GmDev G = gm_dev(c);
  const dim3 G3((c->g.n2 + 255) / 256, c->g.km, c->g.nblocks);
  const dim3 G2(G3.x, c->g.nblocks);
  const bool kappa_now = G.KV && (c->h.c.gm_kappa_freq == 1 || c->nsteps_total == 1 || (c->h.c.gm_kappa_freq == 2 && c->eod_last));
  if (G.tlt) {
    hipLaunchKernelGGL(k_gm_diabatic_depth, G2, dim3(256), 0, c->stream, c->g, G);
    hipLaunchKernelGGL(k_gm_coeffs<1>, G3, dim3(256), 0, c->stream, c->g, G, T, S);
    hipLaunchKernelGGL(k_gm_transition_layer, G2, dim3(256), 0, c->stream, c->g, G);
    if (kappa_now) hipLaunchKernelGGL(k_gm_kappa_vertical, G2, dim3(256), 0, c->stream, c->g, G, T, S, step_params(c).grav);
    hipLaunchKernelGGL(k_gm_coeffs<2>, G3, dim3(256), 0, c->stream, c->g, G, T, S);
    hipLaunchKernelGGL(k_gm_msf_column, G2, dim3(256), 0, c->stream, c->g, G);
  } else {
    if (kappa_now) hipLaunchKernelGGL(k_gm_kappa_vertical, G2, dim3(256), 0, c->stream, c->g, G, T, S, step_params(c).grav);
    hipLaunchKernelGGL(k_gm_coeffs<0>, G3, dim3(256), 0, c->stream, c->g, G, T, S);
  }
  if (G.SF[0]) hipLaunchKernelGGL(k_gm_sf, G3, dim3(256), 0, c->stream, c->g, G);
  if (G.UISOP) hipLaunchKernelGGL(k_gm_bolus, G2, dim3(256), 0, c->stream, c->g, G);
  gm_flux_launch(c, G, T, S, true);
  HIPCHK(c, hipGetLastError());
  if (c->h.c.lsubmesoscale_mixing) return phase_submeso(c, T, S);
  return 0;
}
static int phase_hmix_tracer(pop_ctx *c, hipStream_t st = nullptr) {
  if (c->h.c.hmix_tracer == 3) return phase_hmix_gm(c);
  if (c->h.c.hmix_tracer != 4) return 0;
  if (c->d2t_next_valid && c->d2t_next_slot == c->mixt) {
    c->d2t_next_valid = false;
    std::swap(c->d2t[0], c->d2t_next[0]); std::swap(c->d2t[1], c->d2t_next[1]);
    return 0;
  }
  c->d2t_next_valid = false;
// ... 1436 lines not shown
```

pop2-cesm_amd/csrc/pop_ctx.hpp:

```cpp
#pragma once

#define HIPCHK(ctx, call)                                                                       \
  do {                                                                                          \
    hipError_t e_ = (call);                                                                     \
    if (e_ != hipSuccess) {                                                                     \
      (ctx)->err = std::string(#call) + ": " + hipGetErrorString(e_);                           \
      return 1;                                                                                 \
    }                                                                                           \
  } while (0)

struct PhaseTimer { double ms = 0; int calls = 0; };

struct DevPeer { int rank; int *send_src = nullptr, *recv_dst = nullptr; int nsend = 0, nrecv = 0; };

enum TavgSite { TS_FORCING = 0, TS_STATE, TS_TRACER, TS_VMIX, TS_HMIX, TS_BTROP, TS_QFLUX, TS_NSITES };
struct TavgEntry {
  std::string name;
  int stream = 0, site = 0, ndims = 2, method = TAVG_AVG;
  int kmax = 1;
  int nlev = 1;
  int expr = TX_X, a = -1, b = -1;
  double cst = 0.0, cst2 = 0.0;
  bool cells = false;
  bool vint = false;
  double *buf = nullptr;
};
struct TavgSiteTab { TavgTable cells{}, cols{}; int sid_cells[TAVG_MAX_SRC] = {}, sid_cols[TAVG_MAX_SRC] = {}; bool vint_psurf = false; };
struct TavgState {
  std::vector<TavgEntry> req;
  bool on[TAVG_MAX_STREAMS + 1] = {};
  bool used[TAVG_MAX_STREAMS + 1] = {};
  bool has_qflux[TAVG_MAX_STREAMS + 1] = {};
  double sum[TAVG_MAX_STREAMS + 1] = {}, sum_qflux[TAVG_MAX_STREAMS + 1] = {};
  double dtavg = 0.0;
  bool active = false;
  bool in_step = false;
  bool dirty = true;
  TavgSiteTab site[TS_NSITES];
  double *scratch = nullptr;
};

struct DiagState {
  bool arm_global = false, arm_cfl = false;
  bool run_global = false, run_cfl = false;
  double *partial = nullptr; size_t partial_n = 0;
  double *vec = nullptr; size_t vec_n = 0;
  double *cfl_val = nullptr; int *cfl_idx = nullptr; size_t cfl_n = 0;
  double *h_pre = nullptr, *h_after = nullptr, *h_cfl = nullptr;
  int step_pre = -1, step_after = -1, step_cfl = -1;
  double c2dtt_pre = 0.0, rms_after = 0.0; int iters_after = 0;
};

struct MocState {
  LatAux aux;
  bool requested = false; int stream = 0;
  bool active = false;
  std::vector<int> loc_list, loc_blist;
  MocList *d_lists = nullptr, *d_blists = nullptr; int *d_cells = nullptr, *d_bcells = nullptr;
  double *ACC = nullptr, *BACC = nullptr, *WE = nullptr, *gather = nullptr;
  std::vector<double> set_sums;
  std::vector<double> snap; bool have_snap = false;
};

struct pop_ctx {
  HostModel h;
  Forms f;
  bool host_only = true;
  std::string err;
  hipStream_t stream = nullptr;
  bool own_stream = false;
  DevGrid g{};
  std::map<std::string, double *> d2;
  std::map<std::string, int *> di2;
  std::vector<void *> allocs;
  double *TR[MAXNT][3] = {}, *U[3] = {}, *V[3] = {}, *RHO[3] = {};
  double *PS[3] = {}, *GX[3] = {}, *GY[3] = {}, *UB[3] = {}, *VB[3] = {};
  double *PGUESS = nullptr, *FW = nullptr, *FW_OLD = nullptr, *SHF_QSW = nullptr, *CHL = nullptr;
  double *STF[MAXNT] = {}, *TFW[MAXNT] = {}, *KPP_SRC[MAXNT] = {}, *VDC[2] = {}, *VVC = nullptr;
  double *DH = nullptr, *DHU = nullptr, *ZX = nullptr, *ZY = nullptr, *UH = nullptr, *VH = nullptr;
  double *W3 = nullptr, *W4 = nullptr, *RHS = nullptr, *centerWgt = nullptr;
  double *E3 = nullptr, *F3 = nullptr, *S3a = nullptr, *S3b = nullptr, *S3c = nullptr, *S3d = nullptr;
  double *d2t[2] = {nullptr, nullptr}, *d2u[2] = {nullptr, nullptr};
  double *HDU = nullptr, *HDV = nullptr, *FPARA = nullptr, *FPERP = nullptr;
  double *d2t_next[2] = {nullptr, nullptr};
  bool d2t_next_valid = false; int d2t_next_slot = -1;
  bool tr_ghosts_ok[3] = {true, true, true};
  double *d2u_next[2] = {nullptr, nullptr};
  bool d2u_next_valid = false; int d2u_next_slot = -1;
  bool uv_ghosts_ok[3] = {true, true, true};
  bool d2t_last_formed = false, d2u_last_formed = false;
  hipStream_t side = nullptr; hipEvent_t ev_fork = nullptr, ev_d2t = nullptr, ev_d2u = nullptr, ev_vmixu = nullptr;
  bool vmixu_pending = false, btrop_added = false, vmixu_deferred = false;
  double *HBLT = nullptr, *HMXL = nullptr, *HMXL_DR = nullptr;
  MixDev mix{};
  bool kpp_src_user = false;
  bool src_dirty = true, src_dirty_alt = true;
  double *VDCa[2] = {nullptr, nullptr}, *VVCa = nullptr, *KPPa[MAXNT] = {}, *HBLTa = nullptr, *HMXLa = nullptr, *HMXL_DRa = nullptr;
  int *KBL = nullptr, *KBLa = nullptr;
  hipStream_t ahead = nullptr; hipEvent_t ev_ahead_fork = nullptr, ev_ahead = nullptr;
  bool ahead_valid = false; int ahead_slot = -1, ahead_swaps = 0;
  double *R = nullptr, *S0 = nullptr, *S1 = nullptr, *Q = nullptr, *Z = nullptr, *AZ = nullptr;
  double *partial = nullptr, *blocksum = nullptr;
  SolverScalars *sc = nullptr;
  int *gid = nullptr, *srcmap = nullptr, *iota = nullptr, *loc_of_gid = nullptr;
  std::vector<int> opre_host;
  int *red_act = nullptr, *red_cnt = nullptr; int red_nact = 0;
  SolverScalars *host_sc = nullptr;
  double *host_rr = nullptr;
  hipEvent_t chk_ev[4] = {};
  struct IntervalGraph { const double *key; int variant; hipGraphExec_t exec; };
  std::vector<IntervalGraph> graphs;
  bool grid_from_input = false;
  int full_left = 4, full_seen = 0; double land_fraction = 0.0;
  struct PersistPlan {
    const void *key = nullptr; bool ok = false; std::string why;
    int CP = 0, nwg = 0, nwin_max = 0, nslots = 0;
    int *own_q = nullptr, *halo_off = nullptr, *halo_q = nullptr; unsigned short *nbr = nullptr;
    PWord *W = nullptr;
    double *X0 = nullptr;
  };
  unsigned long long persist_epoch = 0;
  std::vector<PersistPlan> persist;
  std::vector<int> h_srcmap;
  double *persist_out = nullptr;
  int persist_used = 0;
  int persist_gave_up = 0;
  int red_active_total = 0;
  int persist_nwg = 0, persist_cp = 0;
  double *pcsi_raw = nullptr;
  int *pcsi_jfold = nullptr;
  SolveView gv{};
  double *gTAREA = nullptr; int *gKMT = nullptr;
  int nchunk = 0, numIterations = 0;
  double rmsResidual = 0.0;
  int *copy_dst = nullptr, *copy_src = nullptr, *fill_dst = nullptr;
  int ncopy = 0, nfill = 0;
  std::vector<DevPeer> peers;
  int *sa_src = nullptr, *sa_start = nullptr, *sa_cnt = nullptr, *ra_dst = nullptr, *ra_start = nullptr, *ra_cnt = nullptr;
  int nsend_all = 0, nrecv_all = 0;
  int *sendmap = nullptr, *send_off = nullptr, *send_slot = nullptr, *rmap = nullptr;
  bool halo_ns_only = false;
  pop_exchange_fn xchg_side = nullptr;
  hipStream_t comm_side = nullptr;
  hipEvent_t ev_sa = nullptr, ev_sx = nullptr;
  long long solver_ops = 0, solver_enq = 0;
  int *tp_dst[5] = {}, *tp_a[5] = {}, *tp_b[5] = {}; int tp_n[5] = {}; double *tp_buf = nullptr;
  double *sendbuf = nullptr, *recvbuf = nullptr, *redbuf = nullptr;
  long long comm_doubles = 0, red_doubles = 0;
  pop_exchange_fn xchg = nullptr;
  pop_allreduce_fn allred = nullptr;
  void *comm_user = nullptr;
  EvpDev evp{}; bool use_evp = false;
  double *pcsi_omega = nullptr; int *pcsi_base = nullptr; double pcsi_csy = 0;
  double rf_S[MAXNT] = {}, rf_S_prev[MAXNT] = {}; bool rf_S_prev_valid[MAXNT] = {};
  Upw3Dev upw3{};
  LwDev lw{};
  SubmDev subm{};
  GmDev gm{};
  double *PW[MAXNT] = {}, *PWX = nullptr, *PL[2] = {nullptr, nullptr}, *PTD[MAXNT] = {}, *PTDX = nullptr, *KPPX = nullptr, *KPPXa = nullptr;
  RcclTransport *rccl_tr = nullptr;
  struct Tidal { bool inited = false, on = false; pop_tidal_nml nml{}; TidalFields f; } tidal;
  struct Bckgrnd { bool inited = false, on = false; pop_kpp_bckgrnd_nml nml{}; BckgrndFields f; } bck;
  struct Ice { bool inited = false, liceform = false; pop_ice_nml nml{}; IceConsts k{}; double tlast_ice = 0.0;
               double *QICE = nullptr, *AQICE = nullptr, *QFLUX = nullptr, *FWF = nullptr; } ice;
  std::vector<double> tlon;
  bool ran = false;
  int oldt = 0, curt = 1, newt = 2, mixt = 1;
  int first_step = 1, leapfrogts = 1, f_euler_ts = 0, avg_ts = 0, nsteps_total = 0, nsteps_this_interval = 0;
  int eod = 0, eod_last = 0;
  double c2dtt = 0, c2dtu = 0, c2dtp = 0, beta = 0;
  std::map<std::string, PhaseTimer> timers;
  hipEvent_t ev_solve[2] = {nullptr, nullptr}; bool solve_pending = false; int solve_iters_pending = 0;
  double solver_ms_total = 0.0; long long solver_iters_total = 0, solver_calls_total = 0;
  bool timing = false;
  bool phase_timing = false;
  double *op_scratch = nullptr;
  TavgState tavg;
  DiagState diag;
  MocState moc;
};

namespace {

// ... 70 lines not shown
```

Measured before the change: 10.31 SYPD.

## Add grid-stride capping for KPP ahead-stream kernels and occupancy launch bounds

Converts the KPP column kernels (buoyancy march, shear, blmix, hmxl, tidal, background, vvc, passive source) to grid-stride loops over tiles, so the ahead stream can launch a capped number of workgroups that leave room for main-stream work. The cap is set by new tuning knobs (waves per CU or an absolute workgroup count), both defaulting to off. Independently, it adds minimum-occupancy hints to __launch_bounds__ on several KPP kernels, which may force register spills. With the knobs at default, the main effect is the launch-bounds change plus small loop overhead in each kernel.

```diff
diff --git a/include/pop_amd.h b/include/pop_amd.h
--- a/include/pop_amd.h
+++ b/include/pop_amd.h
@@ -139,6 +139,8 @@
   int block_sums_relay;
   int aniso_side;
   int submeso_all_levels;
+  int kpp_ahead_waves;
+  int kpp_ahead_wgs;
 } pop_tuning;
 void pop_tuning_init(pop_tuning *t);
 int pop_get_tuning(const pop_ctx *ctx, pop_tuning *resolved);
diff --git a/pop2-cesm_amd/csrc/forms.hpp b/pop2-cesm_amd/csrc/forms.hpp
--- a/pop2-cesm_amd/csrc/forms.hpp
+++ b/pop2-cesm_amd/csrc/forms.hpp
@@ -26,6 +26,8 @@
   X(bool, kpp_ahead) X(int, kpp_col) X(bool, kpp_lazy) X(bool, kpp_lazy20) X(bool, kpp_march) X(bool, kpp_pbc_generic)              \
   X(bool, kpp_shear_col) X(int, kpp_buoy) X(int, kpp_buoy_kr) X(bool, kpp_buoy_sfc) X(bool, kpp_depth_lazy) X(int, kpp_depth_kr)    \
   X(int, kpp_interior) X(bool, kpp_sparse) X(bool, kpp_side) X(bool, kpp_wuk) X(int, kpp_wuk_margin)                                \
+                                                    \
+  X(int, kpp_ahead_waves) X(int, kpp_ahead_wgs)                                                                                     \
                                                                                                             \
   X(int, state3d_levels) X(bool, gm_sf_stored) X(bool, submeso_all_levels)                                                          \
           \
@@ -178,6 +180,8 @@
     const bool resident_solve = (c.solver_choice == 1 || c.solver_choice == 3) && !evp && f.persist != 0 && h.nranks == 1 && h.nblocks <= 8 &&
                                 h.n2 * h.nblocks <= 250u * 8u * 256u;
     f.kpp_ahead = f.side_stream && (tun_set(t.kpp_ahead) ? t.kpp_ahead != 0 : (big || resident_solve));
+    f.kpp_ahead_waves = std::max(0, tun_or(t.kpp_ahead_waves, 0));
+    f.kpp_ahead_wgs = std::max(0, tun_or(t.kpp_ahead_wgs, 0));
     const std::vector<int> kref = kpp_kref(h);
     const int max_kref = *std::max_element(kref.begin(), kref.end());
     f.kpp_col = (max_kref <= 24) ? tun_or(t.kpp_col, big ? 31 : 1) : 0;
diff --git a/pop2-cesm_amd/csrc/kernels_bckgrnd.hpp b/pop2-cesm_amd/csrc/kernels_bckgrnd.hpp
--- a/pop2-cesm_amd/csrc/kernels_bckgrnd.hpp
+++ b/pop2-cesm_amd/csrc/kernels_bckgrnd.hpp
@@ -9,8 +9,9 @@
 struct BckRaw { double visc, vd1, vd2; };
 __global__ void __launch_bounds__(POP_COL_THREADS)
 k_kpp_bckgrnd(DevGrid g, BckDev bd, int vdc_same, double *__restrict__ VISC, double *__restrict__ VDC1, double *__restrict__ VDC2) {
+  col_tiles(g, [&](int slot, int nslots) {
   Col c;
-  if (!col_setup(g, c, false)) return;
+  if (!col_setup(g, c, false, slot, nslots)) return;
   const int km = g.km;
   const long long n2 = g.n2;
   const int kmt = g.KMT[c.q2];
@@ -32,6 +33,7 @@
     if (!vdc_same) VDC2[vb + (long long)k * n2] = cu.vd2 + bvdc;
     cu = nx;
   }
+  });
 }
 
 }
diff --git a/pop2-cesm_amd/csrc/kernels_common.hpp b/pop2-cesm_amd/csrc/kernels_common.hpp
--- a/pop2-cesm_amd/csrc/kernels_common.hpp
+++ b/pop2-cesm_amd/csrc/kernels_common.hpp
@@ -106,9 +106,9 @@
 }
 __host__ __device__ inline int col_grid_x(int n2, int threads) { const int nt = (n2 + threads - 1) / threads; return 8 * ((nt + 7) / 8); }
 __host__ inline int col_grid(const DevGrid &g, int threads) { return col_grid_x(g.n2, threads); }
-__device__ __forceinline__ bool col_setup(const DevGrid &g, Col &c, bool interior_only) {
+__device__ __forceinline__ bool col_setup(const DevGrid &g, Col &c, bool interior_only, int slot, int nslots) {
   c.b = blockIdx.y;
-  const int tile = g.xcd_remap ? (blockIdx.x & 7) * (gridDim.x >> 3) + (blockIdx.x >> 3) : blockIdx.x;
+  const int tile = g.xcd_remap ? (slot & 7) * (nslots >> 3) + (slot >> 3) : slot;
   c.p2 = tile * blockDim.x + threadIdx.x;
   if (c.p2 >= g.n2) return false;
   if (land_run(g, c.b, (long long)tile * blockDim.x, blockDim.x)) return false;
@@ -119,21 +119,33 @@
   c.base3 = (long long)c.b * g.n3 + c.p2;
   return true;
 }
-__device__ __forceinline__ bool patch_cell(const DevGrid &g, int tile, int b, int &p2) {
+__device__ __forceinline__ bool col_setup(const DevGrid &g, Col &c, bool interior_only) {
+  return col_setup(g, c, interior_only, (int)blockIdx.x, (int)gridDim.x);
+}
+template <bool LDS = false, class F>
+__device__ __forceinline__ void col_tiles(const DevGrid &g, F &&body) {
+  const int nslots = col_grid_x(g.n2, (int)blockDim.x);
+  for (int slot = (int)blockIdx.x; slot < nslots; slot += (int)gridDim.x) {
+    body(slot, nslots);
+    if (LDS) __syncthreads();
+  }
+}
+__device__ __forceinline__ bool patch_cell(const DevGrid &g, int tile, int b, int &p2, int slot) {
   if (!tile) {
-    p2 = blockIdx.x * blockDim.x + threadIdx.x;
+    p2 = slot * blockDim.x + threadIdx.x;
     if (p2 >= g.n2) return false;
-    return !land_run(g, b, (long long)blockIdx.x * blockDim.x, blockDim.x);
+    return !land_run(g, b, (long long)slot * blockDim.x, blockDim.x);
   }
   const int tiles_i = (g.nxb + 63) / 64;
-  const int ti = blockIdx.x % tiles_i, tj = blockIdx.x / tiles_i;
+  const int ti = slot % tiles_i, tj = slot / tiles_i;
   const int i = ti * 64 + (threadIdx.x & 63), j = tj * tile + (threadIdx.x >> 6);
   if (land_tile(g, b, ti * 64, 64, tj * tile, tile)) return false;
   if (i >= g.nxb || j >= g.nyb) return false;
   p2 = j * g.nxb + i;
   return true;
 }
-__host__ inline unsigned patch_grid_x(const DevGrid &g, int tile) {
+__device__ __forceinline__ bool patch_cell(const DevGrid &g, int tile, int b, int &p2) { return patch_cell(g, tile, b, p2, (int)blockIdx.x); }
+__host__ __device__ inline unsigned patch_grid_x(const DevGrid &g, int tile) {
   return tile ? (unsigned)(((g.nxb + 63) / 64) * ((g.nyb + tile - 1) / tile)) : (unsigned)((g.n2 + 255) / 256);
 }
 __host__ inline int red_grid_x(const DevGrid &g) {
diff --git a/pop2-cesm_amd/csrc/kernels_kpp.hpp b/pop2-cesm_amd/csrc/kernels_kpp.hpp
--- a/pop2-cesm_amd/csrc/kernels_kpp.hpp
+++ b/pop2-cesm_amd/csrc/kernels_kpp.hpp
@@ -335,12 +335,13 @@
 }
 struct KppRaw { double t, s, u[4], v[4]; };
 template <bool PBC = false>
-__global__ void __launch_bounds__(POP_COL_THREADS)
+__global__ void __launch_bounds__(POP_COL_THREADS, PBC ? 2 : 3)
 k_kpp_buoy_interior_march(DevGrid g, KppDev kp, const double *__restrict__ T, const double *__restrict__ S,
                           const double *__restrict__ U, const double *__restrict__ V, double *__restrict__ DBLOC,
                           double *__restrict__ VISC, double *__restrict__ VDC1, double *__restrict__ VDC2) {
+  col_tiles(g, [&](int slot, int nslots) {
   Col c;
-  if (!col_setup(g, c, false)) return;
+  if (!col_setup(g, c, false, slot, nslots)) return;
   const int km = g.km, nxb = g.nxb;
   const long long n2 = g.n2;
   const int kmt = g.KMT[c.q2];
@@ -434,30 +435,38 @@
     emit(km - 1, wpp, wp, w);
     emit(km, wp, w, w);
   }
+  });
 }
 
 template <int KR, bool PBC = false>
-__global__ void __launch_bounds__(POP_COL_THREADS)
+__global__ void __launch_bounds__(POP_COL_THREADS, 4)
 k_kpp_ushear_col(DevGrid g, KppDev kp, const double *__restrict__ U, const double *__restrict__ V, double *__restrict__ WU) {
   static_assert(POP_COL_THREADS == 64, "k_kpp_ushear_col: one wavefront per workgroup");
   __shared__ int s_cap;
+  col_tiles<true>(g, [&](int slot, int nslots) {
   if (kp.WUK && threadIdx.x == 0) s_cap = 0;
   Col c;
-  if (!col_setup(g, c, false)) return;
+  const bool live = col_setup(g, c, false, slot, nslots);
   const int km = g.km;
   const long long n2 = g.n2;
   int kcap = km, krcap = KR;
   if (kp.WUK) {
-    int h = kp.KBL[c.q2];
-    if (c.i + 1 < g.nxb) h = max(h, kp.KBL[c.q2 + 1]);
-    if (c.j + 1 < g.nyb) { h = max(h, kp.KBL[c.q2 + g.nxb]); if (c.i + 1 < g.nxb) h = max(h, kp.KBL[c.q2 + g.nxb + 1]); }
+    int h = 0;
+    if (live) {
+      h = kp.KBL[c.q2];
+      if (c.i + 1 < g.nxb) h = max(h, kp.KBL[c.q2 + 1]);
+      if (c.j + 1 < g.nyb) { h = max(h, kp.KBL[c.q2 + g.nxb]); if (c.i + 1 < g.nxb) h = max(h, kp.KBL[c.q2 + g.nxb + 1]); }
+    }
     __syncthreads();
-    atomicMax(&s_cap, h);
+    if (live) atomicMax(&s_cap, h);
     __syncthreads();
     kcap = min(km, max(2, s_cap + kp.wu_margin));
-    kp.WUK[c.q2] = kcap;
-    krcap = kp.kref[kcap];
-  }
+    if (live) {
+      kp.WUK[c.q2] = kcap;
+      krcap = kp.kref[kcap];
+    }
+  }
+  if (!live) return;
   const int kmu_c = PBC ? g.KMU[c.q2] : 0; const double dzub_c = PBC ? g.DZUB[c.q2] : 0.0;
   double ur[KR + 1], vr[KR + 1];
 #pragma unroll
@@ -492,6 +501,7 @@
       WU[o] = (du * du + dv * dv) / (h * h);
     } else WU[o] = du * du + dv * dv;
   }
+  });
 }
 
 template <bool PBC = false>
@@ -775,9 +785,10 @@
               const double *__restrict__ DBSFC, const double *__restrict__ WU, const double *__restrict__ UU, const double *__restrict__ VV) {
   static_assert(POP_COL_THREADS == 64, "the lazy march votes over one 64-lane wave");
   __shared__ double shtop[LAZY ? 3 * KR : 1][POP_COL_THREADS];
+  col_tiles<LAZY>(g, [&](int slot, int nslots) {
   int nprep = 0;
   Col c;
-  if (!col_setup(g, c, false)) return;
+  if (!col_setup(g, c, false, slot, nslots)) return;
   const int km = g.km, nxb = g.nxb;
   const long long n2 = g.n2;
   const int kmt = g.KMT[c.q2];
@@ -909,16 +920,18 @@
   kp.USTAR[c.q2] = ustar;
   kp.BFSFC[c.q2] = bfsfc;
   if (kp.lshort_wave) { kp.BO[c.q2] = bo; kp.BOSOL[c.q2] = bosol; }
+  });
 }
 
 struct KppBlRaw { double visc, vd1, vd2, db; };
 template <bool PBC = false, bool SAME = false, bool SPARSE = false, bool XS = false>
-__global__ void __launch_bounds__(POP_COL_THREADS)
+__global__ void __launch_bounds__(POP_COL_THREADS, 3)
 k_kpp_blmix(DevGrid g, StepParams sp, KppDev kp, const double *__restrict__ DBLOC, const double *__restrict__ STF1,
             const double *__restrict__ STF2, double *__restrict__ VISC, double *__restrict__ VDC1, double *__restrict__ VDC2,
             double *__restrict__ SRC1, double *__restrict__ SRC2, double *__restrict__ HBLT_OUT) {
+  col_tiles(g, [&](int slot, int nslots) {
   Col c;
-  if (!col_setup(g, c, false)) return;
+  if (!col_setup(g, c, false, slot, nslots)) return;
   const int km = g.km, nxb = g.nxb;
   const long long n2 = g.n2;
   const int kmt = g.KMT[c.q2];
@@ -1104,14 +1117,16 @@
     else { SRC1[o] = stf1 / dzk * (flux1_prev - fl1); SRC2[o] = stf2 / dzk * (flux2_prev - fl2); if (XS) kp.SRCX[o] = flux2_prev - fl2; }
     flux1_prev = fl1; flux2_prev = fl2;
   }
+  });
 }
 
 #define POP_VVC_KC 8
-__global__ void __launch_bounds__(POP_COL_THREADS)
+__global__ void __launch_bounds__(POP_COL_THREADS, 8)
 k_kpp_hmxl(DevGrid g, KppDev kp, const double *__restrict__ T, const double *__restrict__ S, const double *__restrict__ DBSFC,
            double *__restrict__ HMXL, double *__restrict__ HMXL_DR) {
+  col_tiles(g, [&](int slot, int nslots) {
   Col c;
-  if (!col_setup(g, c, false)) return;
+  if (!col_setup(g, c, false, slot, nslots)) return;
   const int km = g.km, kmt = g.KMT[c.q2];
   const long long n2 = g.n2;
   const bool pbc = g.pbc != 0;
@@ -1153,12 +1168,15 @@
     rhok = rkp1;
   }
   HMXL_DR[c.q2] = hdr;
+  });
 }
 
 __global__ void k_kpp_vvc(DevGrid g, const double *__restrict__ VISC, double *__restrict__ VVC, int patch) {
+  const int k0 = blockIdx.y * POP_VVC_KC + 1, b = blockIdx.z;
+  const int nslots = (int)patch_grid_x(g, patch);
+  for (int slot = (int)blockIdx.x; slot < nslots; slot += (int)gridDim.x) {
   int p2;
-  const int k0 = blockIdx.y * POP_VVC_KC + 1, b = blockIdx.z;
-  if (!patch_cell(g, patch, b, p2)) return;
+  if (!patch_cell(g, patch, b, p2, slot)) continue;
   const int i = p2 % g.nxb, j = p2 / g.nxb, nxb = g.nxb;
   const long long q2 = (long long)b * g.n2 + p2;
   const bool in = i < g.nxb - 1 && j < g.nyb - 1;
@@ -1172,10 +1190,11 @@
       v = au0 * VISC[o] + aun * VISC[o + nxb] + aue * VISC[o + 1] + aune * VISC[o + nxb + 1];
     VVC[o] = v;
   }
-}
-
-inline void launch_kpp_vvc(const DevGrid &g, int vp, hipStream_t st, const double *VISC, double *VVC) {
-  hipLaunchKernelGGL(k_kpp_vvc, dim3(patch_grid_x(g, vp), (g.km + POP_VVC_KC - 1) / POP_VVC_KC, g.nblocks), dim3(vp ? 64 * vp : 256), 0, st, g, VISC, VVC, vp);
+  }
+}
+
+inline void launch_kpp_vvc(const DevGrid &g, int vp, hipStream_t st, const double *VISC, double *VVC, unsigned gx = 0) {
+  hipLaunchKernelGGL(k_kpp_vvc, dim3(gx ? gx : patch_grid_x(g, vp), (g.km + POP_VVC_KC - 1) / POP_VVC_KC, g.nblocks), dim3(vp ? 64 * vp : 256), 0, st, g, VISC, VVC, vp);
 }
 
 struct KppHost {
@@ -1343,15 +1362,29 @@
 
 inline const int *mix_kpp_kbl(const MixDev &m) { return m.kpp ? ((const KppHost *)m.kpp)->dev.KBL : nullptr; }
 
+struct KppCap {
+  int waves = 0;
+  int wgs = 0;
+  int *last = nullptr;
+  bool on() const { return waves > 0 || wgs > 0; }
+  unsigned x(unsigned full, int wg_waves, int yz) const {
+    if (!on()) return full;
+    const long long c = wgs > 0 ? wgs : std::max(1LL, (long long)waves / wg_waves / std::max(1, yz));
+    const unsigned n = (unsigned)std::min<long long>(full, c);
+    if (last) *last = (int)n;
+    return n;
+  }
+};
 inline int kpp_vmix_coeffs(const HostModel &h, const Forms &f, const DevGrid &g, const StepParams &sp, const MixDev &m, const MixState &s,
-                           hipStream_t st, std::string &err) {
+                           hipStream_t st, std::string &err, const KppCap &cap = KppCap()) {
   const KppHost &KH = *(const KppHost *)m.kpp;
   KppDev g_kpp = KH.dev;
   g_kpp.SHF_QSW = s.SHF_QSW; g_kpp.FCORT = g.FCORT;
   if (s.KBL) g_kpp.KBL = s.KBL;
   g_kpp.vdc_same = (s.VDC[0] == s.VDC[1]) ? 1 : 0;
   if (KH.tidal_on || KH.bck_on) { g_kpp.bckgrnd_vdc = KH.zero_bck; g_kpp.bckgrnd_vvc = KH.zero_bck; }
-  const dim3 GC(col_grid(g, POP_COL_THREADS), g.nblocks), BC(POP_COL_THREADS);
+  const dim3 GF(col_grid(g, POP_COL_THREADS), g.nblocks), BC(POP_COL_THREADS);
+  const dim3 GC(cap.x(GF.x, 1, g.nblocks), g.nblocks);
   const dim3 G3((g.n2 + 255) / 256, g.km, g.nblocks);
   double *DBLOC = s.S3a, *DBSFC = s.S3b, *WU = s.S3c, *VISC = s.S3d, *RIW = s.E3;
   const dim3 GL(col_grid_x(g.n2, POP_COL_THREADS), g.nblocks), BL(POP_COL_THREADS, 4);
@@ -1394,8 +1427,8 @@
     depth(side);
     hipEventRecord(KH.ev_join, side);
   }
-  if (sel.interior == KPP_INTERIOR_REG) with_value<60, 62>(g.km, [&](auto KM) { hipLaunchKernelGGL(k_kpp_interior_reg<KM.value>, GC, BC, 0, st, g, g_kpp, T0, T1, s.UMIX, s.VMIX, (const double *)DBLOC, VISC, s.VDC[0], s.VDC[1]); });
-  else if (sel.interior == KPP_INTERIOR_GENERIC) with_flags([&](auto PBC) { hipLaunchKernelGGL(k_kpp_interior<PBC.value>, GC, BC, 0, st, g, g_kpp, T0, T1, s.UMIX, s.VMIX, (const double *)DBLOC, RIW, VISC, s.VDC[0], s.VDC[1]); }, g.pbc);
+  if (sel.interior == KPP_INTERIOR_REG) with_value<60, 62>(g.km, [&](auto KM) { hipLaunchKernelGGL(k_kpp_interior_reg<KM.value>, GF, BC, 0, st, g, g_kpp, T0, T1, s.UMIX, s.VMIX, (const double *)DBLOC, VISC, s.VDC[0], s.VDC[1]); });
+  else if (sel.interior == KPP_INTERIOR_GENERIC) with_flags([&](auto PBC) { hipLaunchKernelGGL(k_kpp_interior<PBC.value>, GF, BC, 0, st, g, g_kpp, T0, T1, s.UMIX, s.VMIX, (const double *)DBLOC, RIW, VISC, s.VDC[0], s.VDC[1]); }, g.pbc);
   if (KH.tidal_on) {
     TidalDev td = KH.tidal;
     if (KH.bck_on) { td.B2 = KH.bck.VDC; td.BPR2 = KH.bck.VVC_PR; }
@@ -1406,7 +1439,8 @@
   with_flags([&](auto PBC, auto SAME, auto SPARSE, auto XS) {
     hipLaunchKernelGGL((k_kpp_blmix<PBC.value, SAME.value, SPARSE.value, XS.value>), GC, BC, 0, st, g, sp, g_kpp, (const double *)DBLOC, s.STF[0], s.STF[1], VISC, s.VDC[0], s.VDC[1], s.KPP_SRC[0], s.KPP_SRC[1], s.HBLT);
   }, g.pbc, sel.same, sel.sparse, g_kpp.SRCX != nullptr);
-  launch_kpp_vvc(g, f.del4_tile_rows, st, (const double *)VISC, s.VVC);
+  launch_kpp_vvc(g, f.del4_tile_rows, st, (const double *)VISC, s.VVC,
+                 cap.x(patch_grid_x(g, f.del4_tile_rows), f.del4_tile_rows ? f.del4_tile_rows : 4, ((g.km + POP_VVC_KC - 1) / POP_VVC_KC) * g.nblocks));
   if (h.c.kpp_ml_diagnostics == 1 && s.HMXL && s.HMXL_DR)
     hipLaunchKernelGGL(k_kpp_hmxl, GC, BC, 0, st, g, g_kpp, T0, T1, (const double *)DBSFC, s.HMXL, s.HMXL_DR);
   if (hipGetLastError() != hipSuccess) { err = "KPP kernel launch failed"; return 1; }
diff --git a/pop2-cesm_amd/csrc/kernels_mix.hpp b/pop2-cesm_amd/csrc/kernels_mix.hpp
--- a/pop2-cesm_amd/csrc/kernels_mix.hpp
+++ b/pop2-cesm_amd/csrc/kernels_mix.hpp
@@ -122,14 +122,14 @@
   return 0;
 }
 inline int mix_vmix_coeffs(const HostModel &h, const Forms &f, const DevGrid &g, const StepParams &sp, const MixDev &m, const MixState &s,
-                           hipStream_t st, std::string &err) {
+                           hipStream_t st, std::string &err, const KppCap &cap = KppCap()) {
   const dim3 G3((g.n2 + 255) / 256, g.km, g.nblocks);
   if (h.c.vmix_choice == 2) {
     with_flags([&](auto PBC) { hipLaunchKernelGGL(k_rich_t<PBC.value>, G3, dim3(256), 0, st, g, sp, s, s.S3c); }, g.pbc);
     hipLaunchKernelGGL(k_rich_u, G3, dim3(256), 0, st, g, sp, s, (const double *)s.S3c);
     return 0;
   }
-  if (h.c.vmix_choice == 3) return kpp_vmix_coeffs(h, f, g, sp, m, s, st, err);
+  if (h.c.vmix_choice == 3) return kpp_vmix_coeffs(h, f, g, sp, m, s, st, err, cap);
   err = "unknown vmix_choice";
   return 1;
 }
diff --git a/pop2-cesm_amd/csrc/kernels_passive.hpp b/pop2-cesm_amd/csrc/kernels_passive.hpp
--- a/pop2-cesm_amd/csrc/kernels_passive.hpp
+++ b/pop2-cesm_amd/csrc/kernels_passive.hpp
@@ -7,12 +7,13 @@
 template <bool PBC = false>
 __global__ void __launch_bounds__(256)
 k_kpp_src_passive(DevGrid g, const double *__restrict__ X, KppSrcPassiveArgs a, int np) {
-  const int p2 = blockIdx.x * blockDim.x + threadIdx.x;
   const int k = blockIdx.y + 1, b = blockIdx.z / np, n = blockIdx.z % np;
-  if (p2 >= g.n2) return;
-  const long long q2 = (long long)b * g.n2 + p2, o = (long long)b * g.n3 + (long long)(k - 1) * g.n2 + p2;
-  const double dzk = (PBC && k > 1) ? pbc_dz(g, k, g.KMT[q2], g.DZBC[q2]) : g.dz[k];
-  a.SRC[n][o] = a.STF[n][q2] / dzk * X[o];
+  for (long long p = (long long)blockIdx.x * blockDim.x + threadIdx.x; p < g.n2; p += (long long)gridDim.x * blockDim.x) {
+    const int p2 = (int)p;
+    const long long q2 = (long long)b * g.n2 + p2, o = (long long)b * g.n3 + (long long)(k - 1) * g.n2 + p2;
+    const double dzk = (PBC && k > 1) ? pbc_dz(g, k, g.KMT[q2], g.DZBC[q2]) : g.dz[k];
+    a.SRC[n][o] = a.STF[n][q2] / dzk * X[o];
+  }
 }
 
 struct AvgPassiveArgs { double *TO[2], *TC[2]; const double *TN[2]; const double *PO, *PC, *PN; double dz1, grav; };
diff --git a/pop2-cesm_amd/csrc/kernels_tidal.hpp b/pop2-cesm_amd/csrc/kernels_tidal.hpp
--- a/pop2-cesm_amd/csrc/kernels_tidal.hpp
+++ b/pop2-cesm_amd/csrc/kernels_tidal.hpp
@@ -16,11 +16,12 @@
 
 struct TidalRaw { double db, co, visc, vd1, vd2; };
 template <bool PBC = false, bool HV = false>
-__global__ void __launch_bounds__(POP_COL_THREADS)
+__global__ void __launch_bounds__(POP_COL_THREADS, HV ? 7 : 8)
 k_kpp_tidal(DevGrid g, TidalDev td, int vdc_same, const double *__restrict__ DBLOC, double *__restrict__ VISC,
             double *__restrict__ VDC1, double *__restrict__ VDC2) {
+  col_tiles(g, [&](int slot, int nslots) {
   Col c;
-  if (!col_setup(g, c, false)) return;
+  if (!col_setup(g, c, false, slot, nslots)) return;
   const int km = g.km;
   const long long n2 = g.n2;
   const int kmt = g.KMT[c.q2];
@@ -67,6 +68,7 @@
     if (td.DIFF) { td.DIFF[o] = t; td.N2[o] = N2; td.KV[o] = kv; td.KVM[o] = kvm; }
     cu = nx;
   }
+  });
 }
 
 }
diff --git a/pop2-cesm_amd/csrc/pop_amd.hip b/pop2-cesm_amd/csrc/pop_amd.hip
--- a/pop2-cesm_amd/csrc/pop_amd.hip
+++ b/pop2-cesm_amd/csrc/pop_amd.hip
@@ -178,7 +178,8 @@
   X(kpp_src_full, "POP_KPP_SRC_FULL") X(solver_unfused, "POP_SOLVER_UNFUSED") X(solver_nograph, "POP_SOLVER_NOGRAPH")                   \
   X(solver_presum, "POP_SOLVER_PRESUM") X(solver_distributed, "POP_SOLVER_DISTRIBUTED") X(solver_overlap_off, "POP_SOLVER_OVERLAP_OFF") \
   X(fpcg_b2, "POP_FPCG_B2") X(pcsi_step2, "POP_PCSI_STEP2") X(halo_separate, "POP_HALO_SEPARATE")                                       \
-  X(halo_overlap_off, "POP_HALO_OVERLAP_OFF") X(rccl_overlap, "POP_RCCL_OVERLAP") X(evp_wave, "POP_EVP_WAVE") X(fpcg_a_pair, "POP_FPCG_A_PAIR") X(kpp_sparse, "POP_KPP_SPARSE") X(pbc_generic_thomas, "POP_PBC_GENERIC_THOMAS") X(pbc_generic_kpp, "POP_PBC_GENERIC_KPP") X(state3d_levels, "POP_STATE3D_LEVELS") X(gm_sf_stored, "POP_GM_SF_STORED") X(pcg_persist, "POP_PCG_PERSIST") X(gm_flux_tile, "POP_GM_FLUX_TILE") X(pcsi_two_step, "POP_PCSI_TWO_STEP") X(block_sums_relay, "POP_BLOCK_SUMS_RELAY") X(aniso_side, "POP_ANISO_SIDE") X(submeso_all_levels, "POP_SUBMESO_ALL_LEVELS")
+  X(halo_overlap_off, "POP_HALO_OVERLAP_OFF") X(rccl_overlap, "POP_RCCL_OVERLAP") X(evp_wave, "POP_EVP_WAVE") X(fpcg_a_pair, "POP_FPCG_A_PAIR") X(kpp_sparse, "POP_KPP_SPARSE") X(pbc_generic_thomas, "POP_PBC_GENERIC_THOMAS") X(pbc_generic_kpp, "POP_PBC_GENERIC_KPP") X(state3d_levels, "POP_STATE3D_LEVELS") X(gm_sf_stored, "POP_GM_SF_STORED") X(pcg_persist, "POP_PCG_PERSIST") X(gm_flux_tile, "POP_GM_FLUX_TILE") X(pcsi_two_step, "POP_PCSI_TWO_STEP") X(block_sums_relay, "POP_BLOCK_SUMS_RELAY") X(aniso_side, "POP_ANISO_SIDE") X(submeso_all_levels, "POP_SUBMESO_ALL_LEVELS") \
+  X(kpp_ahead_waves, "POP_KPP_AHEAD_WAVES") X(kpp_ahead_wgs, "POP_KPP_AHEAD_WGS")
 void pop_tuning_init(pop_tuning *t) {
   if (!t) return;
   t->struct_bytes = (int)sizeof(pop_tuning);
@@ -795,6 +796,9 @@
     HIPCHK(c, hipStreamCreateWithFlags(&c->ahead, hipStreamNonBlocking));
     HIPCHK(c, hipEventCreateWithFlags(&c->ev_ahead_fork, hipEventDisableTiming));
     HIPCHK(c, hipEventCreateWithFlags(&c->ev_ahead, hipEventDisableTiming));
+    int dev = 0;
+    HIPCHK(c, hipGetDevice(&dev));
+    HIPCHK(c, hipDeviceGetAttribute(&c->cu_count, hipDeviceAttributeMultiprocessorCount, dev));
   }
   c->oldt = 0; c->curt = 1; c->newt = 2; c->mixt = 1;
   for (int t = 0; t < 3; ++t) {
@@ -863,6 +867,7 @@
   if (n == "leapfrogts") return c->leapfrogts;
   if (n == "land_skip_active") return c->g.skip;
   if (n == "kpp_ahead_used") return c->ahead_swaps;
+  if (n == "kpp_ahead_wgs_last") return c->ahead_wgs_last;
   if (n == "d2t_fused") return c->f.d2t_fuse;
   if (n == "d2u_fused") return c->f.d2u_fuse;
   if (n == "d2t_last_formed") return c->d2t_last_formed;
@@ -1254,7 +1259,9 @@
   HIPCHK(c, hipEventRecord(c->ev_ahead_fork, c->stream));
   HIPCHK(c, hipStreamWaitEvent(c->ahead, c->ev_ahead_fork, 0));
   const MixState ms = kpp_mix_state(c, c->curt, true);
-  if (mix_vmix_coeffs(c->h, c->f, c->g, step_params(c), c->mix, ms, c->ahead, c->err)) return 1;
+  KppCap cap;
+  cap.waves = c->cu_count * 4 * c->f.kpp_ahead_waves; cap.wgs = c->f.kpp_ahead_wgs; cap.last = &c->ahead_wgs_last;
+  if (mix_vmix_coeffs(c->h, c->f, c->g, step_params(c), c->mix, ms, c->ahead, c->err, cap)) return 1;
   HIPCHK(c, hipEventRecord(c->ev_ahead, c->ahead));
   c->ahead_valid = true; c->ahead_slot = c->curt;
   return 0;
diff --git a/pop2-cesm_amd/csrc/pop_ctx.hpp b/pop2-cesm_amd/csrc/pop_ctx.hpp
--- a/pop2-cesm_amd/csrc/pop_ctx.hpp
+++ b/pop2-cesm_amd/csrc/pop_ctx.hpp
@@ -99,6 +99,8 @@
   int *KBL = nullptr, *KBLa = nullptr;
   hipStream_t ahead = nullptr; hipEvent_t ev_ahead_fork = nullptr, ev_ahead = nullptr;
   bool ahead_valid = false; int ahead_slot = -1, ahead_swaps = 0;
+  int cu_count = 0;
+  int ahead_wgs_last = 0;
   double *R = nullptr, *S0 = nullptr, *S1 = nullptr, *Q = nullptr, *Z = nullptr, *AZ = nullptr;
   double *partial = nullptr, *blocksum = nullptr;
   SolverScalars *sc = nullptr;
```

Result: no change. 10.25 SYPD (-0.6%).
